# XiandaGuo/OpenStereo

Measured on NVIDIA H100. Metric: stereo_pairs_per_sec_gwcnet_256x512_d192, higher is better.
Workload: dtype f32

## Files before the change

include/openstereo_b200.h:

```cpp
#ifndef OPENSTEREO_B200_H_
#define OPENSTEREO_B200_H_

#include <stddef.h>
#include <stdint.h>

#ifdef __cplusplus
extern "C" {
#endif

#define OSB_OK 0
#define OSB_EINVAL 1
#define OSB_ECUDA 2
#define OSB_EUNSUPPORTED 3

#define OSB_ACT_NONE 0
#define OSB_ACT_RELU 1
#define OSB_ACT_LEAKY 2
#define OSB_ACT_RELU6 3

typedef void* osb_stream_t;

int osb_abi_version(void);
const char* osb_last_error(void);
uint64_t osb_launch_count(void);
int osb_tc_overflow_count(osb_stream_t stream, int reset, unsigned int* count);
int osb_tc_overflow_poll(osb_stream_t stream, unsigned int* host_pinned);
const unsigned int* osb_tc_overflow_flag(void);
float osb_set_rz_kappa(float kappa);
int osb_set_persistent_grid_cap(int cap);
const char* osb_tc_last_variant(void);
const char* osb_volume_last_variant(void);


int osb_gwc_volume_fwd(const float* ref, const float* tgt, float* out, int B, int C, int H, int W,
                       int D, int G, osb_stream_t stream);

int osb_concat_volume_fwd(const float* ref, const float* tgt, float* out, int B, int C, int H,
                          int W, int D, int mask_left, osb_stream_t stream);

int osb_gwc_concat_volume_fwd(const float* ref_gwc, const float* tgt_gwc, const float* ref_cat,
                              const float* tgt_cat, float* out, int B, int Cg, int Cc, int H, int W,
                              int D, int G, osb_stream_t stream);

int osb_corr_volume_fwd(const float* left, const float* right, float* out, int B, int C, int H,
                        int W, int D, osb_stream_t stream);


int osb_softargmin_fwd(const float* cost, float* out, int B, int D, int H, int W, float alpha,
                       float start, float step, int normalize, osb_stream_t stream);

int osb_upsample_softargmin_fwd(const float* cost, float* out, int B, int Dl, int Hl, int Wl, int D,
                                int H, int W, int align_corners, osb_stream_t stream);

int osb_upsample_softargmin_values_fwd(const float* cost, const float* values, float* out, int B, int Dl, int Hl, int Wl,
                                       int D, int H, int W, int align_corners, osb_stream_t stream);

int osb_epe_partial_fwd(const float* pred, const float* gt, float* out, int B, int HW, float maxdisp,
                        osb_stream_t stream);


int osb_conv3d_k3_bn_act_fwd(const float* x, const float* w_packed, const float* scale,
                             const float* shift, const float* residual, const float* gate, float* y,
                             int B, int Cin, int Cout, int D, int H, int W, int stride, int act,
                             osb_stream_t stream);

int osb_deconv3d_bn_act_fwd(const float* x, const float* w_packed, const float* scale,
                            const float* shift, const float* residual, float* y, int B, int Cin,
                            int Cout, int D, int H, int W, int kernel, int act, osb_stream_t stream);

int osb_conv3d_1x1_bn_act_fwd(const float* x0, const float* x1, int Cin0, const float* w_packed,
                              const float* scale, const float* shift, const float* residual,
                              const float* gate, float* y, int B, int Cin, int Cout, int D, int H,
                              int W, int act, int sigmoid_out, osb_stream_t stream);


int osb_conv3d_tc_supported(int Cin, int Cout, int W, int stride);
#define OSB_TC_MIN_WIDTH 24
int osb_tc_general_width(int W);
int osb_conv3d_tc_kc(int Cin, int Cout, int W, int stride);
int osb_conv3d_k3_tc_fwd(const float* x_ndhwc, const void* w_split, const float* scale, const float* shift,
                         const float* residual, float* y, int B, int Cin, int Cout, int D, int H, int W, int act,
                         int out_ndhwc, int res_ndhwc, osb_stream_t stream);
int osb_conv3d_k3_tc_gate_fwd(const float* x_ndhwc, const void* w_split, const float* scale, const float* shift,
                              const float* residual, const float* gate_nhwc, float* y, int B, int Cin, int Cout, int D, int H, int W,
                              int act, osb_stream_t stream);
int osb_conv3d_k3_tc_ncdhw_fwd(const float* x_ncdhw, const void* w_split, const float* scale, const float* shift,
                               const float* residual, float* y, int B, int Cin, int Cout, int D, int H, int W, int act,
                               int out_ndhwc, int res_ndhwc, osb_stream_t stream);
int osb_conv3d_s2_tc_supported(int Cin, int Cout, int D, int H, int W);
int osb_conv3d_k3_s2_tc_fwd(const float* x_ndhwc, const void* w_split, const float* scale, const float* shift,
                            const float* residual, float* y, int B, int Cin, int Cout, int D, int H, int W, int act,
                            int out_ndhwc, int res_ndhwc, osb_stream_t stream);
int osb_deconv3d_tc_supported(int Cin, int Cout, int W);
int osb_deconv3d_k3_tc_fwd(const float* x_ndhwc, const void* w_split, const float* scale, const float* shift,
                           const float* residual, float* y, int B, int Cin, int Cout, int D, int H, int W, int act,
                           int out_ndhwc, int res_ndhwc, osb_stream_t stream);
int osb_deconv3d_k4_tc_supported(int Cin, int Cout, int W);
int osb_deconv3d_k4_tc_fwd(const float* x_ndhwc, const void* w_split, const float* scale, const float* shift,
                           const float* residual, float* y, int B, int Cin, int Cout, int cout_real, int D, int H, int W, int act,
                           int out_ndhwc, int res_ndhwc, osb_stream_t stream);
int osb_conv3d_k3_tc_cs_fwd(const float* x_ndhwc, const void* w_split, const float* scale, const float* shift, const float* residual,
                            const float* gate_nhwc, float* y, int B, int Cin, int Cout, int D, int H, int W, int act, int ystride,
                            osb_stream_t stream);
int osb_conv3d_k3_s2_tc_cs_fwd(const float* x_ndhwc, const void* w_split, const float* scale, const float* shift, float* y, int B,
                               int Cin, int Cout, int D, int H, int W, int act, int ystride, osb_stream_t stream);
int osb_deconv3d_k4_tc_cs_fwd(const float* x_ndhwc, const void* w_split, const float* scale, const float* shift, float* y, int B,
                              int Cin, int Cout, int D, int H, int W, int act, int ystride, osb_stream_t stream);
int osb_conv1x1_ndhwc_cat_fwd(const float* x0, const float* x1, int C0, int C1, const float* w_packed, const float* scale,
                              const float* shift, float* y, long long voxels, int Cout, int act, osb_stream_t stream);
int osb_conv1x1_ndhwc_fwd(const float* x, const float* w_packed, const float* scale, const float* shift, float* y,
                          long long voxels, int Cin, int Cout, int act, osb_stream_t stream);
int osb_conv3d_k3_c1_ndhwc_fwd(const float* x_ndhwc, const float* w_taps, const float* scale, const float* shift, float* y, int B,
                               int Cin, int D, int H, int W, osb_stream_t stream);
int osb_conv2d_tc_kc(int Cin, int Cout, int W, int dilation);
int osb_conv2d_k3_tc_fwd(const float* x_nhwc, const void* w_split, const float* scale, const float* shift, const float* residual,
                         float* y, int B, int Cin, int Cout, int H, int W, int dilation, int act, int out_nhwc, int res_nhwc,
                         osb_stream_t stream);
int osb_gwc_volume_sum_fwd(const float* ref, const float* tgt, float* out, int B, int C, int H, int W, int D, int G,
                           osb_stream_t stream);
int osb_group_l2_normalize_fwd(const float* x, float* y, int B, int C, int H, int W, int G, float eps, osb_stream_t stream);
int osb_sub_volume_fwd(const float* left, const float* right, float* out, int B, int C, int H, int W, int D, osb_stream_t stream);
int osb_regression_values_fwd(const float* prob, const float* values, float* out, int B, int D, int H, int W, osb_stream_t stream);

int osb_warped_concat_volume_fwd(const float* x, const float* y, const float* disp, float* out, int B, int C, int D, int H, int W,
                                 int mask_left, osb_stream_t stream);
int osb_warped_gwc_concat_volume_fwd(const float* xg, const float* yg, const float* xc, const float* yc, const float* disp,
                                     float* out, int B, int Cg, int G, int Cc, int D, int H, int W, osb_stream_t stream);

int osb_coex_regression_fwd(const float* cost, const float* spx, float* out, int B, int D, int h, int w, int top_k, int spx_is_logits,
                            osb_stream_t stream);
int osb_nearest_resize3d_fwd(const float* x, float* y, int N, int Di, int Hi, int Wi, int Do, int Ho, int Wo, osb_stream_t stream);

int osb_mbv2_block3d_fwd(const float* x, const float* w_exp, const float* scale1, const float* shift1, const float* w_dw,
                         const float* scale2, const float* shift2, const float* w_proj, const float* scale3, const float* shift3,
                         const float* residual, float* y, int B, int Cin, int Chid, int Cout, int D, int H, int W, int stride,
                         int in_layout, int out_layout, osb_stream_t stream);

int osb_gwc_volume_bwd(const float* grad_vol, const float* ref, const float* tgt, float* grad_ref, float* grad_tgt, int B, int C,
                       int H, int W, int D, int G, int reduce_sum, osb_stream_t stream);
int osb_concat_volume_bwd(const float* grad_vol, float* grad_ref, float* grad_tgt, int B, int C, int H, int W, int D, int mask_left,
                          osb_stream_t stream);
int osb_softargmin_bwd(const float* cost, const float* grad_out, float* grad_cost, int B, int D, int H, int W, float alpha,
                       float start, float step, int normalize, osb_stream_t stream);

int osb_dwconv2d_fwd(const float* x, const float* w, const float* scale, const float* shift, const float* residual, float* y, int B,
                     int C, int H, int W, int KH, int KW, int stride, int act, osb_stream_t stream);
int osb_deconv2d_k3s2_fwd(const float* x, const float* w_packed, const float* scale, const float* shift, const float* residual,
                          float* y, int B, int Cin, int Cout, int H, int W, int act, osb_stream_t stream);

int osb_avgpool_pairs_fwd(const float* x, float* y, long long outer, int n, long long inner, osb_stream_t stream);
int osb_geo_lookup_fwd(const float* geo0, const float* geo1, const float* geo2, const float* geo3, const float* corr0,
                       const float* corr1, const float* corr2, const float* corr3, const float* disp, const float* coords,
                       float* out, int B, int C, int D, int H, int W, int W2, int num_levels, int radius, osb_stream_t stream);
int osb_context_upsample_fwd(const float* disp_low, const float* up_weights, float* out, int B, int h, int w, int scale,
                             osb_stream_t stream);
int osb_ncdhw_to_ndhwc(const float* x, float* y, int B, int C, int D, int H, int W, osb_stream_t stream);
int osb_ncdhw_to_ndhwc_pad(const float* x, float* y, int B, int C, int Cpad, int D, int H, int W, osb_stream_t stream);
int osb_feature_att_gate_fwd(const float* feat_nchw, const float* w1_packed, const float* scale1, const float* shift1,
                             const float* w2_packed, const float* scale2, const float* shift2, float* gate_nhwc, int B,
                             int Cf, int Ch, int Cv, int Cpad, int HW, int act1, osb_stream_t stream);

#ifdef __cplusplus
}
#endif
#endif
```

openstereo_b200/_lib.py:

```python
import ctypes
import os

_PKG = os.path.dirname(os.path.abspath(__file__))
LIB_PATH = os.path.join(_PKG, "lib", "libopenstereo_b200.so")

_f32p = ctypes.c_void_p
_i = ctypes.c_int
_f = ctypes.c_float
_s = ctypes.c_void_p

SIGNATURES = {
    "osb_gwc_volume_fwd": [_f32p, _f32p, _f32p, _i, _i, _i, _i, _i, _i, _s],
    "osb_concat_volume_fwd": [_f32p, _f32p, _f32p, _i, _i, _i, _i, _i, _i, _s],
    "osb_gwc_concat_volume_fwd": [_f32p, _f32p, _f32p, _f32p, _f32p, _i, _i, _i, _i, _i, _i, _i, _s],
    "osb_corr_volume_fwd": [_f32p, _f32p, _f32p, _i, _i, _i, _i, _i, _s],
    "osb_softargmin_fwd": [_f32p, _f32p, _i, _i, _i, _i, _f, _f, _f, _i, _s],
    "osb_upsample_softargmin_fwd": [_f32p, _f32p, _i, _i, _i, _i, _i, _i, _i, _i, _s],
    "osb_epe_partial_fwd": [_f32p, _f32p, _f32p, _i, _i, _f, _s],
    "osb_conv3d_k3_bn_act_fwd": [_f32p] * 7 + [_i] * 8 + [_s],
    "osb_deconv3d_bn_act_fwd": [_f32p] * 6 + [_i] * 8 + [_s],
    "osb_conv3d_1x1_bn_act_fwd": [_f32p, _f32p, _i] + [_f32p] * 6 + [_i] * 8 + [_s],
    "osb_conv3d_tc_supported": [_i, _i, _i, _i],
    "osb_conv3d_tc_kc": [_i, _i, _i, _i],
    "osb_tc_general_width": [_i],
    "osb_conv3d_s2_tc_supported": [_i, _i, _i, _i, _i],
    "osb_deconv3d_tc_supported": [_i, _i, _i],
    "osb_deconv3d_k3_tc_fwd": [_f32p] * 6 + [_i] * 9 + [_s],
    "osb_conv3d_k3_s2_tc_fwd": [_f32p] * 6 + [_i] * 9 + [_s],
    "osb_conv3d_k3_tc_fwd": [_f32p] * 6 + [_i] * 9 + [_s],
    "osb_conv3d_k3_tc_ncdhw_fwd": [_f32p] * 6 + [_i] * 9 + [_s],
    "osb_conv3d_k3_tc_gate_fwd": [_f32p] * 7 + [_i] * 7 + [_s],
    "osb_deconv3d_k4_tc_supported": [_i, _i, _i],
    "osb_conv3d_k3_tc_cs_fwd": [_f32p] * 7 + [_i] * 8 + [_s],
    "osb_conv3d_k3_s2_tc_cs_fwd": [_f32p] * 5 + [_i] * 8 + [_s],
    "osb_deconv3d_k4_tc_cs_fwd": [_f32p] * 5 + [_i] * 8 + [_s],
    "osb_deconv3d_k4_tc_fwd": [_f32p] * 6 + [_i] * 10 + [_s],
    "osb_conv1x1_ndhwc_cat_fwd": [_f32p, _f32p, _i, _i, _f32p, _f32p, _f32p, _f32p, ctypes.c_longlong, _i, _i, _s],
    "osb_feature_att_gate_fwd": [_f32p] * 8 + [_i] * 7 + [_s],
    "osb_ncdhw_to_ndhwc_pad": [_f32p, _f32p, _i, _i, _i, _i, _i, _i, _s],
    "osb_conv1x1_ndhwc_fwd": [_f32p] * 5 + [ctypes.c_longlong, _i, _i, _i, _s],
    "osb_conv3d_k3_c1_ndhwc_fwd": [_f32p] * 5 + [_i] * 5 + [_s],
    "osb_avgpool_pairs_fwd": [_f32p, _f32p, ctypes.c_longlong, _i, ctypes.c_longlong, _s],
    "osb_geo_lookup_fwd": [_f32p] * 11 + [_i] * 8 + [_s],
    "osb_context_upsample_fwd": [_f32p] * 3 + [_i] * 4 + [_s],
    "osb_conv2d_tc_kc": [_i] * 4,
    "osb_conv2d_k3_tc_fwd": [_f32p] * 6 + [_i] * 9 + [_s],
    "osb_ncdhw_to_ndhwc": [_f32p, _f32p, _i, _i, _i, _i, _i, _s],
    "osb_gwc_volume_sum_fwd": [_f32p, _f32p, _f32p, _i, _i, _i, _i, _i, _i, _s],
    "osb_group_l2_normalize_fwd": [_f32p, _f32p, _i, _i, _i, _i, _i, _f, _s],
    "osb_sub_volume_fwd": [_f32p, _f32p, _f32p, _i, _i, _i, _i, _i, _s],
    "osb_regression_values_fwd": [_f32p, _f32p, _f32p, _i, _i, _i, _i, _s],
    "osb_gwc_volume_bwd": [_f32p] * 5 + [_i] * 7 + [_s],
    "osb_concat_volume_bwd": [_f32p] * 3 + [_i] * 6 + [_s],
    "osb_softargmin_bwd": [_f32p] * 3 + [_i] * 4 + [_f, _f, _f, _i, _s],
    "osb_dwconv2d_fwd": [_f32p] * 6 + [_i] * 8 + [_s],
    "osb_deconv2d_k3s2_fwd": [_f32p] * 6 + [_i] * 6 + [_s],
    "osb_upsample_softargmin_values_fwd": [_f32p] * 3 + [_i] * 8 + [_s],
    "osb_warped_concat_volume_fwd": [_f32p] * 4 + [_i] * 6 + [_s],
    "osb_warped_gwc_concat_volume_fwd": [_f32p] * 6 + [_i] * 7 + [_s],
    "osb_coex_regression_fwd": [_f32p] * 3 + [_i] * 6 + [_s],
    "osb_nearest_resize3d_fwd": [_f32p] * 2 + [_i] * 7 + [_s],
    "osb_mbv2_block3d_fwd": [_f32p] * 12 + [_i] * 10 + [_s],
}


class NativeLibraryError(RuntimeError):
    pass


def _load():
    if not os.path.exists(LIB_PATH):
        raise NativeLibraryError(
            "%s not found: build it with `python -m openstereo_b200.build` (there is no CPU/PyTorch fallback)"
            % LIB_PATH)
    lib = ctypes.CDLL(LIB_PATH)
    lib.osb_abi_version.restype = ctypes.c_int
    lib.osb_last_error.restype = ctypes.c_char_p
    lib.osb_launch_count.restype = ctypes.c_uint64
    lib.osb_tc_overflow_count.argtypes = [ctypes.c_void_p, ctypes.c_int, ctypes.POINTER(ctypes.c_uint)]
    lib.osb_tc_overflow_count.restype = ctypes.c_int
    lib.osb_tc_overflow_poll.argtypes = [ctypes.c_void_p, ctypes.c_void_p]
    lib.osb_tc_overflow_poll.restype = ctypes.c_int
    lib.osb_tc_overflow_flag.argtypes = []
    lib.osb_tc_overflow_flag.restype = ctypes.c_void_p
    lib.osb_set_rz_kappa.argtypes = [ctypes.c_float]
    lib.osb_set_rz_kappa.restype = ctypes.c_float
    lib.osb_set_persistent_grid_cap.argtypes = [ctypes.c_int]
    lib.osb_set_persistent_grid_cap.restype = ctypes.c_int
    lib.osb_tc_last_variant.argtypes = []
    lib.osb_tc_last_variant.restype = ctypes.c_char_p
    lib.osb_volume_last_variant.argtypes = []
    lib.osb_volume_last_variant.restype = ctypes.c_char_p
    for name, argtypes in SIGNATURES.items():
        try:
            fn = getattr(lib, name)
        except AttributeError as exc:
            raise NativeLibraryError("%s does not export %s" % (LIB_PATH, name)) from exc
        fn.argtypes = argtypes
        fn.restype = ctypes.c_int
    return lib


lib = _load()

_ERRORS = {1: ValueError, 2: RuntimeError, 3: NotImplementedError}


def call(name, *args):
    if len(args) != len(SIGNATURES[name]):
        raise TypeError("%s takes %d arguments (%d given)" % (name, len(SIGNATURES[name]), len(args)))
    rc = getattr(lib, name)(*args)
    if rc != 0:
        msg = (lib.osb_last_error() or b"").decode("utf-8", "replace")
# ... 6 lines not shown
```

openstereo_b200/aggregation.py:

```python
import torch

from . import ops
from .ops import ACT_LEAKY, ACT_NONE, ACT_RELU, ACT_RELU6


class _Packed:
    __slots__ = ("w", "scale", "shift", "stride", "kernel", "transposed", "cin", "cout", "_w5", "_tc")

    def __init__(self, conv, bn=None):
        self._tc = {}
        self._w5 = conv.weight.detach() if conv.weight.dim() == 5 else None
        self.cin, self.cout = (conv.in_channels, conv.out_channels)
        self.transposed = isinstance(conv, (torch.nn.ConvTranspose3d, torch.nn.ConvTranspose2d))
        self.kernel = int(conv.kernel_size[0])
        self.stride = int(conv.stride[0])
        self._validate(conv)
        wt = conv.weight
        if wt.dim() == 4:
            wt = wt.unsqueeze(2)
        if self.transposed:
            self.w = ops.pack_deconv_weight(wt)
        else:
            self.w = ops.pack_conv_weight(wt)
        if self.kernel == 1:
            self.w = self.w.reshape(self.w.shape[0], self.w.shape[2]).contiguous()
        self.scale, self.shift = (None, None)
        if bn is not None:
            if bn.training:
                raise RuntimeError("BatchNorm folding is only valid in eval mode (call model.eval())")
            self.scale, self.shift = ops.fold_bn(bn)
        if getattr(conv, "bias", None) is not None:
            bias = conv.bias.detach().float()
            self.shift = bias.contiguous() if self.shift is None else (self.shift + bias * self.scale).contiguous()


def _packed_validate(self, conv):
    ks, st = tuple(conv.kernel_size), tuple(conv.stride)
    ok = len(set(ks)) == 1 and len(set(st)) == 1 and tuple(conv.dilation) == (1,) * len(ks) and conv.groups == 1
    if self.transposed:
        op = tuple(conv.output_padding)
        ok = ok and ((ks[0] == 3 and st[0] == 2 and tuple(conv.padding) == (1,) * len(ks) and op == (1,) * len(ks))
                     or (ks[0] == 4 and st[0] == 2 and tuple(conv.padding) == (1,) * len(ks) and op == (0,) * len(ks)))
    else:
        ok = ok and ks[0] in (1, 3) and st[0] in (1, 2) and tuple(conv.padding) == (ks[0] // 2,) * len(ks)
        ok = ok and getattr(conv, "padding_mode", "zeros") == "zeros"
    if not ok:
        raise NotImplementedError("openstereo_b200: no kernel for %r (supported: Conv k1/k3, stride 1/2, padding k//2, dilation 1, "
                                  "groups 1; ConvTranspose k3 s2 p1 op1 or k4 s2 p1)" % (conv,))


_Packed._validate = _packed_validate


def _conv(layer, x, act=ACT_NONE, residual=None, gate=None):
    if layer.kernel == 1:
        return ops.conv3d_1x1(x, layer.w, layer.scale, layer.shift, residual, gate, act)
    return ops.conv3d_k3(x, layer.w, layer.scale, layer.shift, residual, gate, layer.stride, act)


USE_TENSOR_CORES = True


def _tc_weight(layer, width):
    if not USE_TENSOR_CORES or layer.transposed or layer.kernel != 3 or layer.stride != 1 or layer._w5 is None:
        return None
    kc = ops.conv3d_tc_kc(layer.cin, layer.cout, width)
    if not kc:
        return None
    if kc not in layer._tc:
        layer._tc[kc] = ops.pack_tc_weight(layer._w5, kc, pad_cout_to=16 if layer.cout < 16 else None)
    return layer._tc[kc]


def _tc_ok(layer, width):
    return _tc_weight(layer, width) is not None


def _conv_tc(layer, x_ndhwc, act=ACT_NONE, residual=None, out_ndhwc=True, res_ndhwc=True, in_ncdhw=False):
    wt = _tc_weight(layer, x_ndhwc.shape[4] if in_ncdhw else x_ndhwc.shape[3])
    return ops.conv3d_k3_tc(x_ndhwc, wt, layer.scale, layer.shift, residual, act, out_ndhwc, res_ndhwc, in_ncdhw)


def _stem_in(layer, volume, act):
    if ops.conv3d_tc_kc(layer.cin, layer.cout, volume.shape[-1]) == 32:
        return _conv_tc(layer, volume, act, in_ncdhw=True)
    return _conv_tc(layer, ops.to_ndhwc(volume), act)


def _conv_auto(layer, x, act=ACT_NONE, residual=None):
    if layer.stride == 1 and _tc_ok(layer, x.shape[-1]):
        return _conv_tc(layer, ops.to_ndhwc(x), act, residual, out_ndhwc=False, res_ndhwc=False)
    if (USE_TENSOR_CORES and layer.stride == 2 and layer.kernel == 3 and not layer.transposed and layer._w5 is not None
            and ops.conv3d_s2_tc_supported(layer.cin, layer.cout, x.shape[2], x.shape[3], x.shape[4])):
        if "s2" not in layer._tc:
            layer._tc["s2"] = ops.pack_tc_weight(layer._w5, 16, kw_order=(1, 0, 2))
        return ops.conv3d_k3_s2_tc(ops.to_ndhwc(x), layer._tc["s2"], layer.scale, layer.shift, residual, act)
    return _conv(layer, x, act, residual)


def _deconv(layer, x, act=ACT_NONE, residual=None):
    if (USE_TENSOR_CORES and layer.transposed and layer.kernel == 3 and layer._w5 is not None
            and ops.deconv3d_tc_supported(layer.cin, layer.cout, x.shape[-1])):
        if "dc" not in layer._tc:
            layer._tc["dc"] = ops.pack_tc_deconv_weight(layer._w5)
        return ops.deconv3d_k3_tc(ops.to_ndhwc(x), layer._tc["dc"], layer.scale, layer.shift, residual, act)
    return ops.deconv3d(x, layer.w, layer.scale, layer.shift, residual, layer.kernel, act)


def _versions(module):
    return tuple(p._version for p in module.parameters()) + tuple(b._version for b in module.buffers())


class _Engine:

    def __init__(self, module):
        self.module = module
        self._stamp = None

    def _watch(self, device):
        if USE_TENSOR_CORES:
            mon = ops.TcOverflowMonitor.get(device)
            mon.check()
            return mon
        return None

    def _ensure(self, device):
        stamp = (str(device), _versions(self.module), tuple(p.data_ptr() for p in self.module.parameters()))
        if stamp != self._stamp:
            if self.module.training:
                raise RuntimeError("openstereo_b200 engines run inference only: call model.eval()")
            with torch.no_grad():
                self._pack()
            self._stamp = stamp

    @staticmethod
    def _check(x):
        if not x.is_cuda:
            raise RuntimeError("openstereo_b200: not implemented on the CPU (no fallback); move the model to CUDA")
        return x.detach().float().contiguous()


class _GwcHourglass:
    def __init__(self, m):
        self.conv1, self.conv2 = _Packed(m.conv1[0][0], m.conv1[0][1]), _Packed(m.conv2[0][0], m.conv2[0][1])
        self.conv3, self.conv4 = _Packed(m.conv3[0][0], m.conv3[0][1]), _Packed(m.conv4[0][0], m.conv4[0][1])
        self.conv5, self.conv6 = _Packed(m.conv5[0], m.conv5[1]), _Packed(m.conv6[0], m.conv6[1])
        self.redir1, self.redir2 = _Packed(m.redir1[0], m.redir1[1]), _Packed(m.redir2[0], m.redir2[1])

    def __call__(self, x):
        c1 = _conv_auto(self.conv1, x, ACT_RELU)
        c2 = _conv_auto(self.conv2, c1, ACT_RELU)
        c3 = _conv_auto(self.conv3, c2, ACT_RELU)
        c4 = _conv_auto(self.conv4, c3, ACT_RELU)
        c5 = _deconv(self.conv5, c4, ACT_RELU, residual=_conv(self.redir2, c2))
        return _deconv(self.conv6, c5, ACT_RELU, residual=_conv(self.redir1, x))


def _hg_channels_last_ok(hg, x_shape_ndhwc):
    if not USE_TENSOR_CORES:
        return False
    b, d, h, w, c = x_shape_ndhwc
    if d % 4 or h % 4 or w % 4:
        return False
    return (ops.conv3d_s2_tc_supported(hg.conv1.cin, hg.conv1.cout, d, h, w) and _tc_ok(hg.conv2, w // 2)
            and ops.conv3d_s2_tc_supported(hg.conv3.cin, hg.conv3.cout, d // 2, h // 2, w // 2) and _tc_ok(hg.conv4, w // 4)
            and ops.deconv3d_tc_supported(hg.conv5.cin, hg.conv5.cout, w // 4)
            and ops.deconv3d_tc_supported(hg.conv6.cin, hg.conv6.cout, w // 2)
            and (hg.redir1.cin, hg.redir1.cout) in ((32, 32), (64, 64)) and (hg.redir2.cin, hg.redir2.cout) in ((32, 32), (64, 64)))


def _s2_weight(layer):
    if "s2" not in layer._tc:
        layer._tc["s2"] = ops.pack_tc_weight(layer._w5, 16, kw_order=(1, 0, 2))
    return layer._tc["s2"]


def _dc_weight(layer):
    if "dc" not in layer._tc:
        layer._tc["dc"] = ops.pack_tc_deconv_weight(layer._w5)
    return layer._tc["dc"]


def _gwc_hourglass_channels_last(hg, x):
    c1 = ops.conv3d_k3_s2_tc(x, _s2_weight(hg.conv1), hg.conv1.scale, hg.conv1.shift, None, ACT_RELU, out_ndhwc=True)
    c2 = _conv_tc(hg.conv2, c1, ACT_RELU)
    c3 = ops.conv3d_k3_s2_tc(c2, _s2_weight(hg.conv3), hg.conv3.scale, hg.conv3.shift, None, ACT_RELU, out_ndhwc=True)
    c4 = _conv_tc(hg.conv4, c3, ACT_RELU)
    r2 = ops.conv1x1_ndhwc(c2, hg.redir2.w, hg.redir2.scale, hg.redir2.shift)
    c5 = ops.deconv3d_k3_tc(c4, _dc_weight(hg.conv5), hg.conv5.scale, hg.conv5.shift, r2, ACT_RELU, out_ndhwc=True, res_ndhwc=True)
    r1 = ops.conv1x1_ndhwc(x, hg.redir1.w, hg.redir1.scale, hg.redir1.shift)
    return ops.deconv3d_k3_tc(c5, _dc_weight(hg.conv6), hg.conv6.scale, hg.conv6.shift, r1, ACT_RELU, out_ndhwc=True, res_ndhwc=True)


def _classif3_channels_last(classif3, out):
    head0, cls = classif3
    width = out.shape[3]
    if _tc_ok(cls, width):
        return _conv_tc(cls, _conv_tc(head0, out, ACT_RELU), ACT_NONE, out_ndhwc=False, res_ndhwc=False)
    if cls.cin == 32 and cls.cout == 1 and cls._w5 is not None and cls.stride == 1:
        if "c1" not in cls._tc:
            cls._tc["c1"] = ops.pack_c1_weight(cls._w5)
        head = _conv_tc(head0, out, ACT_RELU)
        return ops.conv3d_k3_c1_ndhwc(head, cls._tc["c1"], cls.scale, cls.shift)
    head = _conv_tc(head0, out, ACT_RELU, out_ndhwc=False)
    return _conv(cls, head)


class GwcAggregation(_Engine):

    def _pack(self):
        m = self.module
        self.dres0 = [_Packed(m.dres0[0][0], m.dres0[0][1]), _Packed(m.dres0[2][0], m.dres0[2][1])]
        self.dres1 = [_Packed(m.dres1[0][0], m.dres1[0][1]), _Packed(m.dres1[2][0], m.dres1[2][1])]
        self.hg = [_GwcHourglass(m.dres2), _GwcHourglass(m.dres3), _GwcHourglass(m.dres4)]
        self.classif3 = [_Packed(m.classif3[0][0], m.classif3[0][1]), _Packed(m.classif3[2])]

    def logits(self, volume):
        volume = self._check(volume)
        self._ensure(volume.device)
        width = volume.shape[-1]
        stem_tc = all(_tc_ok(l, width) for l in (self.dres0[0], self.dres0[1], self.dres1[0], self.dres1[1]))
        b, _, dd, hh, ww = volume.shape
        if stem_tc and _tc_ok(self.classif3[0], width) and all(_hg_channels_last_ok(hg, (b, dd, hh, ww, 32)) for hg in self.hg):
            c = _conv_tc(self.dres0[1], _stem_in(self.dres0[0], volume, ACT_RELU), ACT_RELU)
            out = _conv_tc(self.dres1[1], _conv_tc(self.dres1[0], c, ACT_RELU), ACT_NONE, residual=c)
            for hg in self.hg:
                out = _gwc_hourglass_channels_last(hg, out)
            return _classif3_channels_last(self.classif3, out)
        if stem_tc:
            c = _conv_tc(self.dres0[1], _stem_in(self.dres0[0], volume, ACT_RELU), ACT_RELU)
            cost0 = _conv_tc(self.dres1[1], _conv_tc(self.dres1[0], c, ACT_RELU), ACT_NONE, residual=c, out_ndhwc=False)
        else:
            c = _conv(self.dres0[1], _conv(self.dres0[0], volume, ACT_RELU), ACT_RELU)
            cost0 = _conv(self.dres1[1], _conv(self.dres1[0], c, ACT_RELU), ACT_NONE, residual=c)
        out = cost0
        for hg in self.hg:
            out = hg(out)
        if _tc_ok(self.classif3[0], width):
            head = _conv_tc(self.classif3[0], ops.to_ndhwc(out), ACT_RELU, out_ndhwc=False)
        else:
            head = _conv(self.classif3[0], out, ACT_RELU)
        return _conv(self.classif3[1], head)

    def __call__(self, volume, h, w):
        mon = self._watch(volume.device)
        out = ops.upsample_softargmin(self.logits(volume), self.module.maxdisp, h, w, align_corners=False)
        if mon is not None:
            mon.poll()
        return out


class CascadeAggregation(GwcAggregation):

    def __call__(self, cost, fine_d, fine_h, fine_w, disp_range_samples):
        mon = self._watch(cost.device)
        assert tuple(disp_range_samples.shape[1:]) == (fine_d, fine_h, fine_w)
        out = ops.upsample_softargmin_values(self.logits(cost), disp_range_samples, align_corners=False)
        if mon is not None:
            mon.poll()
        return out


class _PSMHourglass:
    def __init__(self, m):
        self.conv1, self.conv2 = _Packed(m.conv1[0], m.conv1[1]), _Packed(m.conv2[0], m.conv2[1])
        self.conv3, self.conv4 = _Packed(m.conv3[0], m.conv3[1]), _Packed(m.conv4[0], m.conv4[1])
        self.conv5, self.conv6 = _Packed(m.conv5[0], m.conv5[1]), _Packed(m.conv6[0], m.conv6[1])

    def __call__(self, x, presqu, postsqu, skip):
        out = _conv_auto(self.conv1, x, ACT_RELU)
        pre = _conv_auto(self.conv2, out, ACT_RELU, residual=postsqu)
        out = _conv_auto(self.conv4, _conv_auto(self.conv3, pre, ACT_RELU), ACT_RELU)
        post = _deconv(self.conv5, out, ACT_RELU, residual=presqu if presqu is not None else pre)
        return _deconv(self.conv6, post, ACT_NONE, residual=skip), pre, post


def _psm_hg_channels_last_ok(hg, shape_ndhwc):
    if not USE_TENSOR_CORES:
        return False
    b, d, h, w, c = shape_ndhwc
    if d % 4 or h % 4 or w % 4 or any(l._w5 is None for l in (hg.conv1, hg.conv2, hg.conv3, hg.conv4, hg.conv5, hg.conv6)):
        return False
    return (ops.conv3d_s2_tc_supported(hg.conv1.cin, hg.conv1.cout, d, h, w) and _tc_ok(hg.conv2, w // 2)
            and ops.conv3d_s2_tc_supported(hg.conv3.cin, hg.conv3.cout, d // 2, h // 2, w // 2) and _tc_ok(hg.conv4, w // 4)
            and hg.conv5.kernel == 3 and hg.conv6.kernel == 3
            and ops.deconv3d_tc_supported(hg.conv5.cin, hg.conv5.cout, w // 4)
            and ops.deconv3d_tc_supported(hg.conv6.cin, hg.conv6.cout, w // 2))


def _psm_hourglass_channels_last(hg, x, presqu, postsqu, skip):
    out = ops.conv3d_k3_s2_tc(x, _s2_weight(hg.conv1), hg.conv1.scale, hg.conv1.shift, None, ACT_RELU, out_ndhwc=True)
    pre = _conv_tc(hg.conv2, out, ACT_RELU, residual=postsqu)
    out = ops.conv3d_k3_s2_tc(pre, _s2_weight(hg.conv3), hg.conv3.scale, hg.conv3.shift, None, ACT_RELU, out_ndhwc=True)
    out = _conv_tc(hg.conv4, out, ACT_RELU)
    post = ops.deconv3d_k3_tc(out, _dc_weight(hg.conv5), hg.conv5.scale, hg.conv5.shift, presqu if presqu is not None else pre, ACT_RELU,
                              out_ndhwc=True, res_ndhwc=True)
    out = ops.deconv3d_k3_tc(post, _dc_weight(hg.conv6), hg.conv6.scale, hg.conv6.shift, skip, ACT_NONE, out_ndhwc=True, res_ndhwc=True)
    return out, pre, post


class PSMAggregation(_Engine):

    def _pack(self):
        m = self.module
        self.dres0 = [_Packed(m.dres0[0][0], m.dres0[0][1]), _Packed(m.dres0[1][0], m.dres0[1][1])]
        self.dres1 = [_Packed(m.dres1[0][0], m.dres1[0][1]), _Packed(m.dres1[1][0], m.dres1[1][1])]
        self.hg = [_PSMHourglass(m.dres2), _PSMHourglass(m.dres3), _PSMHourglass(m.dres4)]
        self.heads = [[_Packed(c[0][0], c[0][1]), _Packed(c[1])] for c in (m.classif1, m.classif2, m.classif3)]
# ... 577 lines not shown
```

openstereo_b200/csrc/api.cu:

```cuda
#include <atomic>
#include <cstdarg>
#include <cstring>

#include "common.cuh"

namespace osb {

static thread_local char g_error[512] = "";
static std::atomic<uint64_t> g_launches{0};

void set_error(const char* fmt, ...) {
  va_list ap;
  va_start(ap, fmt);
  vsnprintf(g_error, sizeof(g_error), fmt, ap);
  va_end(ap);
}

static std::atomic<float> g_rz_kappa{1.57e-8f};
float rz_kappa() { return g_rz_kappa.load(std::memory_order_relaxed); }

static std::atomic<int> g_grid_cap{0};
long long cap_persistent_grid(long long grid) {
  const int cap = g_grid_cap.load(std::memory_order_relaxed);
  return (cap > 0 && grid > cap) ? cap : grid;
// ... 18 lines not shown
  unsigned int* fresh = nullptr;
  if (cudaMalloc(&fresh, sizeof(unsigned int)) != cudaSuccess || cudaMemset(fresh, 0, sizeof(unsigned int)) != cudaSuccess) {
    set_error("tc_overflow_flag: %s", cudaGetErrorString(cudaGetLastError()));
    return nullptr;
  }
  unsigned int* expected = nullptr;
  if (!g_overflow[dev].compare_exchange_strong(expected, fresh, std::memory_order_acq_rel)) {
    (void)cudaFree(fresh);
    return expected;
  }
  return fresh;
}

int device_index() {
  int dev = 0;
  if (cudaGetDevice(&dev) != cudaSuccess) {
    (void)cudaGetLastError();
    return 0;
  }
  return dev;
}

int sm_count() {
  static std::atomic<int> cache[64];
  const int dev = device_index();
  int n = cache[dev & 63].load(std::memory_order_relaxed);
  if (n > 0) return n;
  if (cudaDeviceGetAttribute(&n, cudaDevAttrMultiProcessorCount, dev) != cudaSuccess || n <= 0) {
    (void)cudaGetLastError();
    n = 132;
  }
  cache[dev & 63].store(n, std::memory_order_relaxed);
  return n;
}

void count_launch(int n) { g_launches.fetch_add((uint64_t)n, std::memory_order_relaxed); }

int check_launch(const char* what) {
  cudaError_t e = cudaGetLastError();
  if (e == cudaSuccess) return OSB_OK;
  set_error("%s: launch failed: %s", what, cudaGetErrorString(e));
  return OSB_ECUDA;
}

typedef CUresult (*EncodeTiledFn)(CUtensorMap*, CUtensorMapDataType, cuuint32_t, void*, const cuuint64_t*,
                                  const cuuint64_t*, const cuuint32_t*, const cuuint32_t*, CUtensorMapInterleave,
                                  CUtensorMapSwizzle, CUtensorMapL2promotion, CUtensorMapFloatOOBfill);

static EncodeTiledFn encode_fn() {
  static EncodeTiledFn fn = [] {
    void* p = nullptr;
    cudaDriverEntryPointQueryResult q;
    cudaError_t e = cudaGetDriverEntryPoint("cuTensorMapEncodeTiled", &p, cudaEnableDefault, &q);
    if (e != cudaSuccess || q != cudaDriverEntryPointSuccess) {
      (void)cudaGetLastError();
      return (EncodeTiledFn) nullptr;
    }
    return reinterpret_cast<EncodeTiledFn>(p);
  }();
  return fn;
}

bool make_tensor_map_3d(CUtensorMap* out, const void* base, uint64_t d0, uint64_t d1, uint64_t d2, uint64_t stride1_bytes,
                        uint64_t stride2_bytes, uint32_t box0, uint32_t box1, uint32_t box2) {
  EncodeTiledFn fn = encode_fn();
  if (!fn) {
    set_error("cuTensorMapEncodeTiled not available from the driver");
    return false;
  }
  const cuuint64_t dims[3] = {d0, d1, d2};
  const cuuint64_t strides[2] = {stride1_bytes, stride2_bytes};
  const cuuint32_t box[3] = {box0, box1, box2};
  const cuuint32_t elem[3] = {1, 1, 1};
  CUresult r = fn(out, CU_TENSOR_MAP_DATA_TYPE_FLOAT32, 3, const_cast<void*>(base), dims, strides, box, elem,
                  CU_TENSOR_MAP_INTERLEAVE_NONE, CU_TENSOR_MAP_SWIZZLE_NONE, CU_TENSOR_MAP_L2_PROMOTION_L2_128B,
                  CU_TENSOR_MAP_FLOAT_OOB_FILL_NONE);
  if (r != CUDA_SUCCESS) {
    set_error("cuTensorMapEncodeTiled failed with CUresult %d", (int)r);
    return false;
  }
  return true;
}

}

extern "C" {
int osb_abi_version(void) { return 1; }
const char* osb_last_error(void) { return osb::g_error; }
uint64_t osb_launch_count(void) { return osb::g_launches.load(std::memory_order_relaxed); }
float osb_set_rz_kappa(float kappa) {
  const float old = osb::g_rz_kappa.load(std::memory_order_relaxed);
  if (kappa >= 0.f && kappa < 1e-6f) osb::g_rz_kappa.store(kappa, std::memory_order_relaxed);
  return old;
}
int osb_set_persistent_grid_cap(int cap) { return osb::g_grid_cap.exchange(cap > 0 ? cap : 0, std::memory_order_relaxed); }
const char* osb_tc_last_variant(void) { return osb::g_tc_variant; }
int osb_tc_overflow_count(osb_stream_t stream, int reset, unsigned int* count) {
  using namespace osb;
  OSB_REQUIRE(count, "tc_overflow_count: null pointer");
  unsigned int* flag = tc_overflow_flag();
  if (!flag) return OSB_ECUDA;
  cudaStream_t st = (cudaStream_t)stream;
  cudaError_t e = cudaMemcpyAsync(count, flag, sizeof(unsigned int), cudaMemcpyDeviceToHost, st);
  if (e == cudaSuccess && reset) e = cudaMemsetAsync(flag, 0, sizeof(unsigned int), st);
  if (e == cudaSuccess) e = cudaStreamSynchronize(st);
  if (e != cudaSuccess) {
    set_error("tc_overflow_count: %s", cudaGetErrorString(e));
    return OSB_ECUDA;
  }
  return OSB_OK;
}
const unsigned int* osb_tc_overflow_flag(void) { return osb::tc_overflow_flag(); }
int osb_tc_overflow_poll(osb_stream_t stream, unsigned int* host_pinned) {
  using namespace osb;
  OSB_REQUIRE(host_pinned, "tc_overflow_poll: null pointer");
  unsigned int* flag = tc_overflow_flag();
  if (!flag) return OSB_ECUDA;
  cudaError_t e = cudaMemcpyAsync(host_pinned, flag, sizeof(unsigned int), cudaMemcpyDeviceToHost, (cudaStream_t)stream);
  if (e != cudaSuccess) {
    set_error("tc_overflow_poll: %s", cudaGetErrorString(e));
    return OSB_ECUDA;
  }
  return OSB_OK;
}
}
```

openstereo_b200/csrc/common.cuh:

```cuda
#pragma once
#include <cuda.h>
#include <cuda_runtime.h>
#include <stdint.h>
#include <stdio.h>

#include <string>

#include "../../include/openstereo_b200.h"

namespace osb {

void set_error(const char* fmt, ...);
void count_launch(int n = 1);
int check_launch(const char* what);
int device_index();
int sm_count();
long long cap_persistent_grid(long long grid);
std::string tc_variant_name(const char* fmt, ...);
void set_tc_variant(const char* name);
struct PerDeviceFlag {
  bool done[64] = {};
  bool& here() { return done[device_index() & 63]; }
};

#define OSB_REQUIRE(cond, ...)          \
  do {                                  \
    if (!(cond)) {                      \
      ::osb::set_error(__VA_ARGS__);    \
      return OSB_EINVAL;                \
    }                                   \
  } while (0)

__device__ __forceinline__ uint32_t smem_u32(const void* p) {
  return static_cast<uint32_t>(__cvta_generic_to_shared(p));
}

__device__ __forceinline__ void mbar_init(uint64_t* bar, uint32_t count) {
  asm volatile("mbarrier.init.shared::cta.b64 [%0], %1;" ::"r"(smem_u32(bar)), "r"(count));
}
__device__ __forceinline__ void fence_mbar_init() {
  asm volatile("fence.mbarrier_init.release.cluster;" ::: "memory");
}
__device__ __forceinline__ void fence_proxy_async() {
  asm volatile("fence.proxy.async.shared::cta;" ::: "memory");
}
__device__ __forceinline__ void mbar_arrive_expect_tx(uint64_t* bar, uint32_t bytes) {
  asm volatile("mbarrier.arrive.expect_tx.shared::cta.b64 _, [%0], %1;" ::"r"(smem_u32(bar)), "r"(bytes)
               : "memory");
}
__device__ __forceinline__ void mbar_wait(uint64_t* bar, uint32_t parity) {
  asm volatile(
      "{\n"
      ".reg .pred p;\n"
      "WAIT_LOOP:\n"
      "mbarrier.try_wait.parity.shared::cta.b64 p, [%0], %1;\n"
      "@p bra DONE;\n"
      "bra WAIT_LOOP;\n"
      "DONE:\n"
      "}\n" ::"r"(smem_u32(bar)),
      "r"(parity)
      : "memory");
}
__device__ __forceinline__ void tma_load_3d(void* smem_dst, const CUtensorMap* map, uint64_t* bar, int c0,
                                            int c1, int c2) {
  asm volatile(
      "cp.async.bulk.tensor.3d.shared::cluster.global.mbarrier::complete_tx::bytes [%0], [%1, {%3, %4, %5}], [%2];"
      ::"r"(smem_u32(smem_dst)),
      "l"(reinterpret_cast<uint64_t>(map)), "r"(smem_u32(bar)), "r"(c0), "r"(c1), "r"(c2)
      : "memory");
}
__device__ __forceinline__ void tma_prefetch_desc(const CUtensorMap* map) {
  asm volatile("prefetch.tensormap [%0];" ::"l"(reinterpret_cast<uint64_t>(map)) : "memory");
}

__device__ __forceinline__ void st_cs_f4(float* p, float4 v) { __stcs(reinterpret_cast<float4*>(p), v); }

bool make_tensor_map_3d(CUtensorMap* out, const void* base, uint64_t d0, uint64_t d1, uint64_t d2, uint64_t stride1_bytes,
                        uint64_t stride2_bytes, uint32_t box0, uint32_t box1, uint32_t box2);

}
```

openstereo_b200/csrc/conv3d_tc.cu:

```cuda
#include <type_traits>

#include "tc_common.cuh"

namespace osb {

constexpr int TC_W = 128;
constexpr int TC_KC = 32;
constexpr int TC_TILES = TC_WGS;
constexpr int TC_ROWS = TC_TILES + 2;
constexpr int TC_STAGES = 4;
constexpr int TC_RAW = 2;
constexpr int TC_ROW_BYTES = TC_W * TC_KC * 4;

struct TcParams {
  const float* x;
  const void* w;
  const float* scale;
  const float* shift;
  const float* residual;
  float* y;
  int B, D, H, Cin, Cout;
  int act;
  float kappa;
  unsigned int* overflow;
  int out_ndhwc, res_ndhwc;
  int bulk_rows;
  int in_ncdhw;
  int items, hblocks;
};

template <int COUT>
struct TcCfg {
  static constexpr int N3 = 3 * COUT;
  static constexpr int B_SLICE = N3 * TC_KC * 4;
  static constexpr int XCHG_FLOATS = 2 * frag_xchg_floats<COUT, 1>();
  static constexpr int A_OFF = 0;
  static constexpr int B_OFF = A_OFF + TC_STAGES * TC_ROW_BYTES;
  static constexpr int RAW_OFF = B_OFF + TC_BSLOTS * 3 * B_SLICE;
  static constexpr int BAR_OFF = RAW_OFF + TC_RAW * TC_ROW_BYTES;
  static constexpr size_t SMEM = 1024 + (size_t)BAR_OFF + 256 + TC_WGS * XCHG_FLOATS * 4 + 4 * TC_WGS * FRAG_TP_FLOATS * 4 + 2 * COUT * 4;
  static_assert(B_SLICE % 1024 == 0, "weight slices must stay 1024-byte aligned");
  static_assert(SMEM <= 232448, "shared memory budget of one CTA exceeded");
};

template <int COUT>
__global__ void __launch_bounds__(TC_WG_THREADS, 1) conv3d_tc_kernel(const TcParams p) {
  using C = TcCfg<COUT>;
  constexpr int N3 = C::N3;
  constexpr int B_SLICE = C::B_SLICE;
  extern __shared__ __align__(1024) uint8_t smem_raw[];
  uint8_t* smem = smem_raw + ((1024u - (smem_u32(smem_raw) & 1023u)) & 1023u);
  uint8_t* a_buf = smem + C::A_OFF;
  uint8_t* b_buf = smem + C::B_OFF;
  uint8_t* raw_buf = smem + C::RAW_OFF;
  uint64_t* bars = reinterpret_cast<uint64_t*>(smem + C::BAR_OFF);
  uint64_t* a_ready = bars;
  uint64_t* a_empty = a_ready + TC_STAGES;
  uint64_t* b_full = a_empty + TC_STAGES;
  uint64_t* b_empty = b_full + TC_BSLOTS * 3;
  uint64_t* raw_full = b_empty + TC_BSLOTS * 3;
  uint64_t* raw_empty = raw_full + TC_RAW;
  float* xchg = reinterpret_cast<float*>(smem + C::BAR_OFF + 256);
  float* tiles = xchg + TC_WGS * C::XCHG_FLOATS;
  float* s_scale = tiles + 4 * TC_WGS * FRAG_TP_FLOATS;
  float* s_shift = s_scale + COUT;

  const int warp = threadIdx.x >> 5, lane = threadIdx.x & 31;
  const int nchunk = p.Cin / TC_KC;

  if (threadIdx.x == 0) {
    for (int s = 0; s < TC_STAGES; ++s) {
      mbar_init(&a_ready[s], 128);
      mbar_init(&a_empty[s], 4 * TC_WGS);
    }
    for (int k = 0; k < TC_BSLOTS * 3; ++k) {
      mbar_init(&b_full[k], 1);
      mbar_init(&b_empty[k], 4 * TC_WGS);
    }
    for (int k = 0; k < TC_RAW; ++k) {
      mbar_init(&raw_full[k], 1);
      mbar_init(&raw_empty[k], 128);
    }
    fence_mbar_init();
  }
  for (int c = threadIdx.x; c < COUT; c += blockDim.x) {
    s_scale[c] = p.scale ? p.scale[c] : 1.f;
    s_shift[c] = p.shift ? p.shift[c] : 0.f;
  }
  __syncthreads();
  struct RowIter {
    int it, kd, ch, r;
  };
  auto advance = [&](RowIter& s) {
    for (;;) {
      if (s.it >= p.items) return false;
      if (++s.r < TC_ROWS) return true;
      s.r = -1;
      if (++s.ch < nchunk) continue;
      s.ch = 0;
      const int d = (s.it / p.hblocks) % p.D;
      for (++s.kd; s.kd < 3; ++s.kd) {
        const int din = d + s.kd - 1;
        if (din >= 0 && din < p.D) break;
      }
      if (s.kd < 3) continue;
      s.it += gridDim.x;
      if (s.it >= p.items) return false;
      const int d2 = (s.it / p.hblocks) % p.D;
      s.kd = (d2 == 0) ? 1 : 0;
    }
  };
  if (warp < 4 * TC_WGS) {
    setmaxnreg_inc<TC_CONSUMER_REGS>();
    const int wg = warp >> 2;
    xchg += wg * C::XCHG_FLOATS;
    const int bar_xchg = 1 + wg;
    constexpr uint32_t LO = TcK<TC_KC>::LO_OFF;
    constexpr uint32_t A_HALF = 64 * TC_KC * 4 / 16;
    const uint64_t dbase = desc_sw128_base();
    const uint32_t b16 = (smem_u32(b_buf) & 0x3FFFF) >> 4;
    const int q = warp & 3;
    uint32_t rowc = 0, phc = 0, exc = 0;
    for (int it = blockIdx.x; it < p.items; it += gridDim.x) {
      const int d = (it / p.hblocks) % p.D;
      const int b = it / (p.hblocks * p.D);
      const int h = (it % p.hblocks) * TC_TILES + wg;
      if (h < p.H && p.residual && p.res_ndhwc)
        asm volatile("prefetch.global.L2 [%0];" ::"l"(p.residual + ((((size_t)b * p.D + d) * p.H + h) * TC_W + q * 32 + lane) * COUT));
      float acc[2][N3 / 2];
      uint32_t accum = 0;
      for (int kd = 0; kd < 3; ++kd) {
        const int din = d + kd - 1;
        if (din < 0 || din >= p.D) continue;
        for (int ch = 0; ch < nchunk; ++ch, ++phc) {
          const uint32_t bslot = (phc & 1) * 3;
#pragma unroll
          for (int r = 0; r < TC_ROWS; ++r) {
            const uint32_t s = rowc % TC_STAGES, par = (rowc / TC_STAGES) & 1;
            mbar_wait(&a_ready[s], par);
            const int kh = r - wg;
            if (kh >= 0 && kh < 3) {
              mbar_wait(&b_full[bslot + kh], (phc >> 1) & 1);
              const uint64_t da0 = dbase | (uint64_t)((smem_u32(a_buf + s * TC_ROW_BYTES) & 0x3FFFF) >> 4);
              const uint64_t db0 = dbase | (uint64_t)(b16 + (bslot + kh) * (B_SLICE / 16));
              wg_fence();
#pragma unroll
              for (int ks = 0; ks < TcK<TC_KC>::KSTEPS; ++ks)
                wg_mma_split<N3>(acc, da0 + 2 * ks, A_HALF, db0 + 2 * ks, LO, ks > 0 ? 1u : accum);
              wg_commit();
              wg_wait_all();
              accum = 1;
              wg_release(&b_empty[bslot + kh], lane);
            }
            wg_release(&a_empty[s], lane);
            ++rowc;
          }
        }
      }
      if (h >= p.H) continue;
      const float corr = 1.f + p.kappa * (float)(((d > 0) + 1 + (d + 1 < p.D)) * nchunk * 3 * TcK<TC_KC>::KSTEPS * 3);
      frag_unshift<COUT, 1, TC_W>(acc, xchg + (exc & 1) * (C::XCHG_FLOATS / 2), q, lane, corr, bar_xchg);
      ++exc;
      const size_t row0 = (((size_t)b * p.D + d) * p.H + h) * TC_W;
      const size_t plane = (size_t)p.D * p.H * TC_W;
      const size_t ncdhw0 = (size_t)b * p.Cout * plane + ((size_t)d * p.H + h) * TC_W;
      auto rows = [&](int m, ptrdiff_t& yo, ptrdiff_t& ro, ptrdiff_t& go) {
        yo = p.out_ndhwc ? (ptrdiff_t)(row0 + m) * COUT : (ptrdiff_t)(ncdhw0 + m);
        ro = p.res_ndhwc ? (ptrdiff_t)(row0 + m) * COUT : (ptrdiff_t)(ncdhw0 + m);
        go = 0;
        return true;
      };
      frag_epilogue<COUT>(acc, lane, q, tiles + warp * FRAG_TP_FLOATS, s_scale, s_shift, p.act, p.y, p.out_ndhwc ? 1 : plane, p.residual, p.res_ndhwc ? 1 : plane,
                          nullptr, rows, COUT == 32 ? 32 : p.Cout);
    }
  }
  else if (warp < 4 * TC_WGS + 4) {
    setmaxnreg_dec<TC_LOADER_REGS>();
    const int lt = threadIdx.x - 4 * TC_WGS * 32;
    const int vsel = lt >> 3, c16 = lt & 7;
    const int vcol = ((vsel & 1) << 2) | ((vsel >> 1) & 3) | (vsel & 8);
    float amax = 0.f;
    auto run = [&](auto in_ncdhw) {
      constexpr bool NCDHW = decltype(in_ncdhw)::value;
      const size_t row_stride = (size_t)TC_W * p.Cin;
      auto load_row = [&](const RowIter& s, float4 (&v)[8]) {
        const int hb = s.it % p.hblocks;
        const int d = (s.it / p.hblocks) % p.D;
        const int b = s.it / (p.hblocks * p.D);
        const int hin = hb * TC_TILES - 1 + s.r, din = d + s.kd - 1;
        if (hin >= 0 && hin < p.H && NCDHW) {
          const size_t plane = (size_t)p.D * p.H * TC_W;
          const float* src = p.x + (((size_t)b * p.Cin + s.ch * TC_KC) * p.D + din) * p.H * TC_W + (size_t)hin * TC_W + lt;
#pragma unroll
          for (int j = 0; j < 8; ++j, src += 4 * plane)
            v[j] = make_float4(__ldg(src), __ldg(src + plane), __ldg(src + 2 * plane), __ldg(src + 3 * plane));
          const bool swap = (lt >> 3) & 1;
#pragma unroll
          for (int j = 0; j < 8; j += 2) {
            const float4 e = v[j], o = v[j + 1];
            v[j] = swap ? o : e;
            v[j + 1] = swap ? e : o;
          }
        } else if (hin >= 0 && hin < p.H) {
          const float* src = p.x + (((size_t)b * p.D + din) * p.H + hin) * row_stride + s.ch * TC_KC + c16 * 4 + vcol * p.Cin;
#pragma unroll
          for (int j = 0; j < 8; ++j) v[j] = __ldg(reinterpret_cast<const float4*>(src + 16 * j * p.Cin));
        } else {
#pragma unroll
          for (int j = 0; j < 8; ++j) v[j] = make_float4(0.f, 0.f, 0.f, 0.f);
        }
      };
      uint32_t rowc = 0;
      auto store_row = [&](const float4 (&v)[8]) {
        const uint32_t s = rowc % TC_STAGES, par = (rowc / TC_STAGES) & 1;
        mbar_wait_relaxed(&a_empty[s], par ^ 1);
        uint8_t* tile = a_buf + s * TC_ROW_BYTES;
        if (NCDHW) {
#pragma unroll
          for (int j = 0; j < 8; ++j) stage_f16_split<TC_KC>(tile, lt, j ^ ((lt >> 3) & 1), v[j], amax);
        } else {
#pragma unroll
          for (int j = 0; j < 8; ++j) stage_f16_split<TC_KC>(tile, vcol + 16 * j, c16, v[j], amax);
        }
        fence_proxy_async();
        mbar_arrive(&a_ready[s]);
        ++rowc;
      };
      RowIter ld{(int)blockIdx.x, 0, 0, -1};
      if (ld.it < p.items) ld.kd = (((ld.it / p.hblocks) % p.D) == 0) ? 1 : 0;
      if (p.bulk_rows) {
        uint32_t rawc = 0;
        while (advance(ld)) {
          const int hb = ld.it % p.hblocks;
          const int hin = hb * TC_TILES - 1 + ld.r;
          const uint32_t slot = rawc % TC_RAW, par = (rawc / TC_RAW) & 1;
          mbar_wait_relaxed(&raw_full[slot], par);
          float4 v[8];
          if (hin >= 0 && hin < p.H && NCDHW) {
            const float* src = reinterpret_cast<const float*>(raw_buf + slot * TC_ROW_BYTES) + lt;
#pragma unroll
            for (int j = 0; j < 8; ++j) {
              const float* q = src + 4 * (j ^ ((lt >> 3) & 1)) * TC_W;
              v[j] = make_float4(q[0], q[TC_W], q[2 * TC_W], q[3 * TC_W]);
            }
          } else if (hin >= 0 && hin < p.H) {
            const float* src = reinterpret_cast<const float*>(raw_buf + slot * TC_ROW_BYTES) + c16 * 4;
#pragma unroll
            for (int j = 0; j < 8; ++j) v[j] = *reinterpret_cast<const float4*>(src + (vcol + 16 * j) * TC_KC);
          } else {
#pragma unroll
            for (int j = 0; j < 8; ++j) v[j] = make_float4(0.f, 0.f, 0.f, 0.f);
          }
          store_row(v);
          mbar_arrive(&raw_empty[slot]);
          ++rawc;
        }
        tc_report_overflow(p.overflow, amax);
        amax = 0.f;
      }
      float4 va[8], vb[8];
      bool has_a = !p.bulk_rows && advance(ld);
      if (has_a) load_row(ld, va);
      bool has_b = has_a && advance(ld);
      if (has_b) load_row(ld, vb);
      while (has_a) {
        store_row(va);
        has_a = has_b && advance(ld);
        if (has_a) load_row(ld, va);
        if (!has_b) break;
        store_row(vb);
        has_b = has_a && advance(ld);
        if (has_b) load_row(ld, vb);
      }
      tc_report_overflow(p.overflow, amax);
    };
    if (p.in_ncdhw) run(std::true_type{});
    else run(std::false_type{});
  }
  else {
    setmaxnreg_dec<TC_PRODUCER_REGS>();
    if (warp == 4 * TC_WGS + 4 && elect_one()) {
      const uint8_t* wsrc = reinterpret_cast<const uint8_t*>(p.w);
      uint32_t phc = 0;
      for (int it = blockIdx.x; it < p.items; it += gridDim.x) {
        const int d = (it / p.hblocks) % p.D;
        for (int kd = 0; kd < 3; ++kd) {
          const int din = d + kd - 1;
          if (din < 0 || din >= p.D) continue;
          for (int ch = 0; ch < nchunk; ++ch, ++phc) {
            for (int kh = 0; kh < 3; ++kh) {
              const uint32_t slot = (phc & 1) * 3 + kh;
              const size_t slice = ((size_t)kd * nchunk + ch) * 3 + kh;
              mbar_wait_relaxed(&b_empty[slot], ((phc >> 1) & 1) ^ 1);
              mbar_arrive_expect_tx(&b_full[slot], B_SLICE);
              bulk_g2s(b_buf + slot * B_SLICE, wsrc + slice * B_SLICE, B_SLICE, &b_full[slot]);
            }
          }
        }
      }
    }
    else if (warp == 4 * TC_WGS + 5 && p.bulk_rows && elect_one()) {
      RowIter ld{(int)blockIdx.x, 0, 0, -1};
      if (ld.it < p.items) ld.kd = (((ld.it / p.hblocks) % p.D) == 0) ? 1 : 0;
      uint32_t rawc = 0;
      while (advance(ld)) {
        const int hb = ld.it % p.hblocks;
        const int d = (ld.it / p.hblocks) % p.D;
        const int b = ld.it / (p.hblocks * p.D);
        const int hin = hb * TC_TILES - 1 + ld.r, din = d + ld.kd - 1;
        const uint32_t slot = rawc % TC_RAW, par = (rawc / TC_RAW) & 1;
        mbar_wait_relaxed(&raw_empty[slot], par ^ 1);
        if (hin >= 0 && hin < p.H && p.in_ncdhw) {
          const size_t plane = (size_t)p.D * p.H * TC_W;
          const float* src = p.x + (((size_t)b * p.Cin + ld.ch * TC_KC) * p.D + din) * p.H * TC_W + (size_t)hin * TC_W;
          mbar_arrive_expect_tx(&raw_full[slot], TC_ROW_BYTES);
          for (int c = 0; c < TC_KC; ++c)
            bulk_g2s(raw_buf + slot * TC_ROW_BYTES + c * (TC_W * 4), src + c * plane, TC_W * 4, &raw_full[slot]);
        } else if (hin >= 0 && hin < p.H) {
          const float* src = p.x + (((size_t)b * p.D + din) * p.H + hin) * (size_t)(TC_W * TC_KC);
          mbar_arrive_expect_tx(&raw_full[slot], TC_ROW_BYTES);
          bulk_g2s(raw_buf + slot * TC_ROW_BYTES, src, TC_ROW_BYTES, &raw_full[slot]);
        } else {
          mbar_arrive(&raw_full[slot]);
        }
        ++rawc;
      }
    }
    __syncwarp();
  }
}

__global__ void __launch_bounds__(256) ncdhw_to_ndhwc_kernel(const float* __restrict__ x, float* __restrict__ y, int C, int Cp,
                                                             size_t vol) {
  __shared__ float tile[32][33];
  const int b = blockIdx.z;
  const size_t v0 = (size_t)blockIdx.x * 32;
  const int c0 = blockIdx.y * 32;
  const int tx = threadIdx.x & 31, ty = threadIdx.x >> 5;
  for (int i = ty; i < 32; i += 8) {
    const int c = c0 + i;
    const size_t v = v0 + tx;
    tile[i][tx] = (c < C && v < vol) ? __ldg(x + ((size_t)b * C + c) * vol + v) : 0.f;
  }
  __syncthreads();
  for (int i = ty; i < 32; i += 8) {
    const size_t v = v0 + i;
    const int c = c0 + tx;
    if (c < Cp && v < vol) y[((size_t)b * vol + v) * Cp + c] = tile[tx][i];
  }
}

template <int COUT>
int launch_tc(const TcArgs& a, cudaStream_t stream) {
  TcParams p{};
  p.Cout = a.Cout, p.in_ncdhw = a.in_ncdhw;
  p.bulk_rows = a.in_ncdhw || a.Cin == TC_KC;
  p.hblocks = (a.H + TC_TILES - 1) / TC_TILES;
  static const std::string variant = tc_variant_name("tc<%d>", COUT);
  return launch_persistent<conv3d_tc_kernel<COUT>>(a, p, (long long)a.B * a.D * p.hblocks, TcCfg<COUT>::SMEM, variant.c_str(), stream);
}
template int launch_tc<32>(const TcArgs&, cudaStream_t);
template int launch_tc<16>(const TcArgs&, cudaStream_t);

}

extern "C" {

int osb_tc_general_width(int W) { return W >= OSB_TC_MIN_WIDTH ? 1 : 0; }

int osb_conv3d_tc_kc(int Cin, int Cout, int W, int stride) {
  return stride == 1 ? osb::select_conv3d_tc(Cin, Cout, W, 1, false, false).kc : 0;
}

int osb_conv3d_tc_supported(int Cin, int Cout, int W, int stride) { return osb_conv3d_tc_kc(Cin, Cout, W, stride) != 0; }

int osb_ncdhw_to_ndhwc_pad(const float* x, float* y, int B, int C, int Cpad, int D, int H, int W, osb_stream_t stream) {
  using namespace osb;
  OSB_REQUIRE(x && y, "ncdhw_to_ndhwc: null pointer");
  OSB_REQUIRE(B > 0 && C > 0 && Cpad >= C && D > 0 && H > 0 && W > 0 && B <= 65535, "ncdhw_to_ndhwc: bad shape");
  const size_t vol = (size_t)D * H * W;
  dim3 grid((unsigned)((vol + 31) / 32), (Cpad + 31) / 32, B);
  ncdhw_to_ndhwc_kernel<<<grid, 256, 0, (cudaStream_t)stream>>>(x, y, C, Cpad, vol);
  count_launch();
  return check_launch("ncdhw_to_ndhwc_kernel");
}

int osb_ncdhw_to_ndhwc(const float* x, float* y, int B, int C, int D, int H, int W, osb_stream_t stream) {
  return osb_ncdhw_to_ndhwc_pad(x, y, B, C, C, D, H, W, stream);
}

static int conv3d_k3_tc_impl(osb::TcArgs a, int dilation, osb_stream_t stream) {
  using namespace osb;
  const int kc = select_conv3d_tc(a.Cin, a.Cout, a.W, dilation, false, false).kc;
  OSB_REQUIRE(kc, "conv3d_k3_tc: unsupported shape Cin=%d Cout=%d W=%d dilation=%d", a.Cin, a.Cout, a.W, dilation);
  OSB_REQUIRE(!a.in_ncdhw || kc == 32, "conv3d_k3_tc: NCDHW input is served by the W = 128 kernel only");
  OSB_REQUIRE((!a.ystride && !a.gate) || kc == 16, "conv3d_k3_tc: a channel slice or gate needs the 16-channel-chunk kernels");
  OSB_REQUIRE(a.Cout > 16 || (!a.out_ndhwc && (!a.residual || !a.res_ndhwc)), "conv3d_k3_tc: Cout <= 16 writes (and adds) NCDHW tensors only");
  const TcLaunch launch = select_conv3d_tc(a.Cin, a.Cout, a.W, dilation, a.gate != nullptr, a.slice()).launch;
  const int rc = check_tc_args("conv3d_k3_tc", a, launch);
  return rc != OSB_OK ? rc : launch(a, (cudaStream_t)stream);
}

int osb_conv3d_k3_tc_fwd(const float* x_ndhwc, const void* w_split, const float* scale, const float* shift,
                         const float* residual, float* y, int B, int Cin, int Cout, int D, int H, int W, int act,
                         int out_ndhwc, int res_ndhwc, osb_stream_t stream) {
  return conv3d_k3_tc_impl({x_ndhwc, w_split, scale, shift, residual, nullptr, y, B, Cin, Cout, D, H, W, act, out_ndhwc, res_ndhwc, 0, 0,
                            Cout}, 1, stream);
}

int osb_conv3d_k3_tc_gate_fwd(const float* x_ndhwc, const void* w_split, const float* scale, const float* shift,
                              const float* residual, const float* gate_nhwc, float* y, int B, int Cin, int Cout, int D, int H, int W,
                              int act, osb_stream_t stream) {
  OSB_REQUIRE(gate_nhwc, "conv3d_k3_tc_gate: null gate");
  return conv3d_k3_tc_impl({x_ndhwc, w_split, scale, shift, residual, gate_nhwc, y, B, Cin, Cout, D, H, W, act, 1, 1, 0, 0, Cout}, 1,
                           stream);
}

int osb_conv3d_k3_tc_cs_fwd(const float* x_ndhwc, const void* w_split, const float* scale, const float* shift, const float* residual,
                            const float* gate_nhwc, float* y, int B, int Cin, int Cout, int D, int H, int W, int act, int ystride,
                            osb_stream_t stream) {
  return conv3d_k3_tc_impl({x_ndhwc, w_split, scale, shift, residual, gate_nhwc, y, B, Cin, Cout, D, H, W, act, 1, 1, 0, ystride, Cout},
                           1, stream);
}

int osb_conv3d_k3_tc_ncdhw_fwd(const float* x_ncdhw, const void* w_split, const float* scale, const float* shift,
                               const float* residual, float* y, int B, int Cin, int Cout, int D, int H, int W, int act,
                               int out_ndhwc, int res_ndhwc, osb_stream_t stream) {
  return conv3d_k3_tc_impl({x_ncdhw, w_split, scale, shift, residual, nullptr, y, B, Cin, Cout, D, H, W, act, out_ndhwc, res_ndhwc, 1, 0,
                            Cout}, 1, stream);
}

int osb_conv2d_tc_kc(int Cin, int Cout, int W, int dilation) { return osb::select_conv3d_tc(Cin, Cout, W, dilation, false, false).kc; }

int osb_conv2d_k3_tc_fwd(const float* x_nhwc, const void* w_split, const float* scale, const float* shift, const float* residual,
                         float* y, int B, int Cin, int Cout, int H, int W, int dilation, int act, int out_nhwc, int res_nhwc,
                         osb_stream_t stream) {
  return conv3d_k3_tc_impl({x_nhwc, w_split, scale, shift, residual, nullptr, y, B, Cin, Cout, 1, H, W, act, out_nhwc, res_nhwc, 0, 0,
                            Cout}, dilation, stream);
}
}
```

openstereo_b200/csrc/conv3d_tcdc.cu:

```cuda
#include "tc_common.cuh"

namespace osb {

struct TcdcParams {
  const float* x;
  const void* w;
  const float* scale;
  const float* shift;
  const float* residual;
  float* y;
  int B, D, H, Cin;
  int act;
  float kappa;
  unsigned int* overflow;
  int out_ndhwc, res_ndhwc;
  int items, hblocks;
  int Wr, ctiles;
  int ystride;
  int cout_real;
};

template <int COUT, int KC, int W, int TILES, bool GW = false, int KS_ = 3>
struct TcdcCfg {
  static_assert(!GW || W == 128, "general-width tiles are 128-column segments of one input row");
  static_assert(KS_ == 3 || (KS_ == 4 && !GW), "kernel size 3 (any width) or 4 (whole-row tiles)");
  static constexpr int KS = KS_;
  static constexpr int HALO = GW ? 1 : 0;
  static constexpr int CSTEP = 128 - HALO;
  static constexpr int R = 128 / W;
  static constexpr int ROWB = KC * 4;
  static constexpr int UNIT_BYTES = 128 * ROWB;
  static constexpr int N3 = KS_ * COUT;
  static constexpr int G = 32;
  static constexpr int NG = COUT / G;
  static constexpr int NGK = KS_ * G;
  static constexpr int B_SLICE = N3 * ROWB;
  static constexpr int B_SUB = NGK * ROWB;
  static constexpr int SCOLS = KS_ == 3 ? NGK : 2 * G;
  static constexpr int LD = SCOLS + 4;
  static constexpr int NU = KS_ - 1;
  static constexpr int NLW = 4;
  static constexpr int XCHG_FLOATS = 2 * 4 * 2 * 32;
  static constexpr int FIXED_SMEM = 1024 + TC_BSLOTS * KS_ * B_SUB + TC_WGS * 128 * LD * 4 + 1024 + TC_WGS * XCHG_FLOATS * 4 + 3 * COUT * 4;
  static constexpr int STAGES = (232448 - FIXED_SMEM) / UNIT_BYTES < 10 ? (232448 - FIXED_SMEM) / UNIT_BYTES : 10;
  static_assert(STAGES >= NLW, "the ring must hold at least one unit per loader warp");
  static constexpr int HBLK = TILES * R;
  static constexpr int KSTEPS = KC / 16;
  static constexpr int LO = KC / 8;
  static constexpr int A_OFF = 0;
  static constexpr int B_OFF = A_OFF + STAGES * UNIT_BYTES;
  static constexpr int STAGE_OFF = B_OFF + TC_BSLOTS * KS_ * B_SUB;
  static constexpr int BAR_OFF = STAGE_OFF + TC_WGS * 128 * LD * 4;
  static constexpr int THREADS = TC_WG_THREADS;
  static constexpr size_t SMEM = 1024 + (size_t)BAR_OFF + 1024 + TC_WGS * XCHG_FLOATS * 4 + 3 * COUT * 4;
  static_assert(SMEM <= 232448, "shared memory budget of one CTA exceeded");
  static_assert(TILES == 1, "a consumer warpgroup holds one accumulator tile");
  static_assert(COUT % G == 0, "output channels come in groups of 32");
  static_assert(32 * LD >= TP_WARP_FLOATS, "store_ndhwc_chunk32 transposes through the warp's own rows of the staging tile");
  static_assert(B_SUB % 1024 == 0 && UNIT_BYTES % 1024 == 0, "operand tiles must stay 1024-byte aligned");
  static constexpr int kh_of(int u, int t) { return (t - 1 + 2 * u >= 0 && t - 1 + 2 * u < KS_) ? t - 1 + 2 * u : -1; }
};

struct ItemDc {
  int b, od, j0, ct, nkd;
};
__device__ __forceinline__ bool kd_valid(int od, int kd, int D) {
  const int num = od + 1 - kd;
  return !(num & 1) && num >= 0 && (num >> 1) < D;
}
__device__ __forceinline__ bool kh_valid(int ph, int kh) { return ((ph + 1 - kh) & 1) == 0; }
template <class C>
__device__ __forceinline__ ItemDc decode_dc(const TcdcParams& p, int it) {
  ItemDc w;
  w.ct = 0;
  if (C::HALO) {
    w.ct = it % p.ctiles;
    it /= p.ctiles;
  }
  const int Do = 2 * p.D;
  w.od = it % Do;
  it /= Do;
  w.j0 = (it % p.hblocks) * C::HBLK;
  w.b = it / p.hblocks;
  w.nkd = 0;
#pragma unroll
  for (int k = 0; k < C::KS; ++k) w.nkd += kd_valid(w.od, k, p.D) ? 1 : 0;
  return w;
}

template <int N, int GA, int GB, bool ADD>
__device__ __forceinline__ void dc_stage_pair(float* stage, int ld, const float (&acc)[2][N / 2], int wq, int lane) {
#pragma unroll
  for (int h = 0; h < 2; ++h) {
    float* r0 = stage + (64 * h + 16 * wq + (lane >> 2)) * ld + 2 * (lane & 3);
#pragma unroll
    for (int g = 0; g < 2; ++g)
#pragma unroll
      for (int jj = 0; jj < 4; ++jj) {
        const int j = (g ? GB : GA) * 4 + jj;
#pragma unroll
        for (int r = 0; r < 2; ++r) {
          float2* d = reinterpret_cast<float2*>(r0 + 8 * r * ld + 32 * g + 8 * jj);
          float2 v = make_float2(acc[h][4 * j + 2 * r], acc[h][4 * j + 2 * r + 1]);
          if (ADD) {
            const float2 s = *d;
            v = make_float2(s.x + v.x, s.y + v.y);
          }
          *d = v;
        }
      }
  }
}

template <int COUT, int KC, int W, int TILES, bool GW = false, int KS = 3>
__global__ void __launch_bounds__(TcdcCfg<COUT, KC, W, TILES, GW, KS>::THREADS, 1) conv3d_tcdc_kernel(const TcdcParams p) {
  using C = TcdcCfg<COUT, KC, W, TILES, GW, KS>;
  extern __shared__ __align__(1024) uint8_t smem_raw[];
  uint8_t* smem = smem_raw + ((1024u - (smem_u32(smem_raw) & 1023u)) & 1023u);
  uint8_t* a_buf = smem + C::A_OFF;
  uint8_t* b_buf = smem + C::B_OFF;
  float* stage = reinterpret_cast<float*>(smem + C::STAGE_OFF);
  uint64_t* bars = reinterpret_cast<uint64_t*>(smem + C::BAR_OFF);
  uint64_t* a_ready = bars;
  uint64_t* a_empty = a_ready + C::STAGES;
  uint64_t* b_full = a_empty + C::STAGES;
  uint64_t* b_empty = b_full + TC_BSLOTS * KS;
  float* xchg = reinterpret_cast<float*>(smem + C::BAR_OFF + 1024);
  float* s_scale = xchg + TC_WGS * C::XCHG_FLOATS;
  float* s_shift = s_scale + COUT;
  float* zeros = s_shift + COUT;

  const int warp = threadIdx.x >> 5, lane = threadIdx.x & 31;
  const int nchunk = p.Cin / KC;
  const int Wp = GW ? p.Wr : W;
  const int YS = (W < 32 && p.ystride) ? p.ystride : COUT;

  if (threadIdx.x == 0) {
    for (int s = 0; s < C::STAGES; ++s) {
      mbar_init(&a_ready[s], 32);
      mbar_init(&a_empty[s], 4 * TC_WGS);
    }
    for (int k = 0; k < TC_BSLOTS * KS; ++k) {
      mbar_init(&b_full[k], 1);
      mbar_init(&b_empty[k], 4 * TC_WGS);
    }
    fence_mbar_init();
  }
  for (int c = threadIdx.x; c < COUT; c += blockDim.x) {
    s_scale[c] = p.scale ? p.scale[c] : 1.f;
    s_shift[c] = p.shift ? p.shift[c] : 0.f;
    zeros[c] = 0.f;
  }
  __syncthreads();

  if (warp < 4 * TC_WGS) {
    setmaxnreg_inc<TC_CONSUMER_REGS>();
    const int wg = warp >> 2;
    stage += wg * 128 * C::LD;
    xchg += wg * C::XCHG_FLOATS;
    const int bar_stage = 1 + 2 * wg, bar_xchg = 2 + 2 * wg;
    const uint64_t dbase = (KC == 32) ? desc_sw128_base() : desc_sw64_base();
    constexpr uint32_t A_HALF = 64 * C::ROWB / 16;
    const uint32_t b16 = (smem_u32(b_buf) & 0x3FFFF) >> 4;
    const int q = warp & 3;
    const int m = q * 32 + lane;
    const int rr = m / W, wcol = m % W;
    const bool has_right_q = (((q + 1) * 32) % W) != 0;
    const bool has_left_q = ((q * 32) % W) != 0;
    const int Do = 2 * p.D, Ho = 2 * p.H;
    const int Wo = 2 * Wp;
    uint32_t unitc = 0, phc = 0, exc = 0;
    for (int it = blockIdx.x; it < p.items; it += gridDim.x) {
      const int cg = (it % C::NG) * C::G;
      const ItemDc w = decode_dc<C>(p, it / C::NG);
      float ev[32], od_[32];
      float acc[2][C::NGK / 2];
      uint32_t accum = 0;
      for (int kd = 0; kd < KS; ++kd) {
        if (!kd_valid(w.od, kd, p.D)) continue;
        for (int ch = 0; ch < nchunk; ++ch, ++phc) {
          const uint32_t bset = (phc & 1) * KS, bpar = (phc >> 1) & 1;
#pragma unroll
          for (int kh = 0; kh < KS; ++kh) {
            if (kh_valid(wg, kh)) continue;
            mbar_wait(&b_full[bset + kh], bpar);
            wg_release(&b_empty[bset + kh], lane);
          }
#pragma unroll
          for (int u = 0; u < C::NU; ++u) {
            const uint32_t slot = unitc % C::STAGES, par = (unitc / C::STAGES) & 1;
            mbar_wait(&a_ready[slot], par);
            const int kh = C::kh_of(u, wg);
            if (kh >= 0) {
              mbar_wait(&b_full[bset + kh], bpar);
              const uint64_t da0 = dbase | (uint64_t)((smem_u32(a_buf + slot * C::UNIT_BYTES) & 0x3FFFF) >> 4);
              const uint64_t db0 = dbase | (uint64_t)(b16 + ((bset + kh) * C::B_SUB) / 16);
              wg_fence();
#pragma unroll
              for (int ks = 0; ks < C::KSTEPS; ++ks)
                wg_mma_split<C::NGK>(acc, da0 + 2 * ks, A_HALF, db0 + 2 * ks, C::LO, ks > 0 ? 1u : accum);
              wg_commit();
              wg_wait_all();
              accum = 1;
              wg_release(&b_empty[bset + kh], lane);
            }
            wg_release(&a_empty[slot], lane);
            ++unitc;
          }
        }
      }
      const int j = w.j0 + rr;
      const bool live = j < p.H;
      const int oh = 2 * j + wg;
      const int col = GW ? w.ct * C::CSTEP + m : wcol;
      const bool cvalid = !GW || (m < C::CSTEP && col < Wp);
      const uint32_t vmask = GW ? __ballot_sync(0xffffffffu, cvalid) : 0xffffffffu;
      const size_t vox = (((size_t)w.b * Do + w.od) * Ho + oh) * Wo + 2 * col;
      if (live && cvalid && p.residual && p.res_ndhwc) {
        const float* rp = p.residual + vox * YS;
#pragma unroll
        for (int k = 0; k < 2 * COUT; k += 32) asm volatile("prefetch.global.L2 [%0];" ::"l"(rp + k));
      }
      const float corr = 1.f + p.kappa * (float)(w.nkd * (KS == 4 ? 2 : wg + 1) * nchunk * C::KSTEPS * 3);
      float* srow = stage + m * C::LD;
      float* xb = xchg + (exc & 1) * (4 * 2 * 32);
      ++exc;
      named_bar_sync(bar_stage, 128);
      if constexpr (KS == 3) {
        wg_stage<C::NGK>(stage, C::LD, acc, q, lane);
        named_bar_sync(bar_stage, 128);
        if (lane == 0) {
#pragma unroll
          for (int i = 0; i < 32; i += 4)
            *reinterpret_cast<float4*>(xb + (q * 2) * 32 + i) = *reinterpret_cast<const float4*>(srow + 2 * C::G + i);
        }
        named_bar_sync(bar_xchg, 128);
        const float* xr = has_right_q ? xb + ((q + 1) * 2) * 32 : zeros;
#pragma unroll
        for (int i0 = 0; i0 < 32; i0 += 4) {
          const float4 r4 = *reinterpret_cast<const float4*>(xr + i0);
          const float4 e4 = *reinterpret_cast<const float4*>(srow + i0);
          const float4 p24 = *reinterpret_cast<const float4*>(srow + C::G + i0);
          const float4 p04 = *reinterpret_cast<const float4*>(srow + 2 * C::G + i0);
          const float re[4] = {r4.x, r4.y, r4.z, r4.w};
          const float e[4] = {e4.x, e4.y, e4.z, e4.w}, p2[4] = {p24.x, p24.y, p24.z, p24.w}, p0[4] = {p04.x, p04.y, p04.z, p04.w};
#pragma unroll
          for (int k = 0; k < 4; ++k) {
            const int i = i0 + k;
            float right = __shfl_down_sync(0xffffffffu, p0[k], 1);
            right = (lane == 31) ? re[k] : right;
            if (W < 32) right = (wcol == W - 1) ? 0.f : right;
            ev[i] = e[k] * corr;
            od_[i] = (p2[k] + right) * corr;
          }
        }
      } else {
        dc_stage_pair<C::NGK, 1, 3, false>(stage, C::LD, acc, q, lane);
        named_bar_sync(bar_stage, 128);
        if (lane == 31) {
#pragma unroll
          for (int i = 0; i < 32; i += 4)
            *reinterpret_cast<float4*>(xb + (q * 2 + 1) * 32 + i) = *reinterpret_cast<const float4*>(srow + i);
        }
        if (lane == 0) {
#pragma unroll
          for (int i = 0; i < 32; i += 4)
            *reinterpret_cast<float4*>(xb + (q * 2) * 32 + i) = *reinterpret_cast<const float4*>(srow + C::G + i);
        }
        named_bar_sync(bar_xchg, 128);
        const float* xl = has_left_q ? xb + ((q - 1) * 2 + 1) * 32 : zeros;
        const float* xr = has_right_q ? xb + ((q + 1) * 2) * 32 : zeros;
#pragma unroll
        for (int i0 = 0; i0 < 32; i0 += 4) {
          const float4 l4 = *reinterpret_cast<const float4*>(xl + i0);
          const float4 r4 = *reinterpret_cast<const float4*>(xr + i0);
          const float4 p34 = *reinterpret_cast<const float4*>(srow + i0);
          const float4 p04 = *reinterpret_cast<const float4*>(srow + C::G + i0);
          const float le[4] = {l4.x, l4.y, l4.z, l4.w}, re[4] = {r4.x, r4.y, r4.z, r4.w};
          const float p3[4] = {p34.x, p34.y, p34.z, p34.w}, p0[4] = {p04.x, p04.y, p04.z, p04.w};
          float e[4], o[4];
#pragma unroll
          for (int k = 0; k < 4; ++k) {
            const float left = __shfl_up_sync(0xffffffffu, p3[k], 1);
// ... 231 lines not shown
```

openstereo_b200/csrc/conv3d_tcg.cu:

```cuda
#include "tc_common.cuh"

namespace osb {

struct TcgParams {
  const float* x;
  const void* w;
  const float* scale;
  const float* shift;
  const float* residual;
  const float* gate;
  float* y;
  int B, D, H, Cin;
  int act;
  float kappa;
  unsigned int* overflow;
  int out_ndhwc, res_ndhwc;
  int items, hblocks;
  int Wr, ctiles;
  int ystride;
};

template <int COUT, int KC, int W, int TILES, int DIL = 1, bool GW = false>
struct TcgCfg {
  static_assert(!GW || W == 128, "general-width tiles are 128-column segments of one image row");
  static constexpr int HALO = GW ? DIL : 0;
  static constexpr int CSTEP = 128 - 2 * HALO;
  static_assert(DIL == 1 || (W == 128 && DIL == 2 && COUT >= 64), "dilation 2 is instantiated for full-width rows only");
  static constexpr int R = 128 / W;
  static constexpr int ROWB = KC * 4;
  static constexpr int UNIT_BYTES = 128 * ROWB;
  static constexpr int N3 = 3 * COUT;
  static constexpr int G = 32;
  static constexpr int NG = COUT / G;
  static constexpr int NG3 = 3 * G;
  static constexpr int B_SLICE = N3 * ROWB;
  static constexpr int B_SUB = NG3 * ROWB;
  static constexpr int NT = TC_WGS * TILES;
  static constexpr int TS = R * DIL;
  static constexpr int HSPAN = NT * TS;
  __host__ __device__ static constexpr int row0(int hb) { return (hb / DIL) * HSPAN + (hb % DIL) * R; }
  __host__ static int hblocks(int H) { return DIL * ((H + HSPAN - 1) / HSPAN); }
  static constexpr int NLW = 4;
  static constexpr int XCHG_FLOATS = 2 * frag_xchg_floats<G, DIL>();
  static constexpr int FIXED_SMEM = 1024 + TC_BSLOTS * 3 * B_SUB + 1024 + TC_WGS * XCHG_FLOATS * 4 + 4 * TC_WGS * FRAG_TP_FLOATS * 4 +
                                    2 * COUT * 4;
  static constexpr int STAGES = (232448 - FIXED_SMEM) / UNIT_BYTES < 10 ? (232448 - FIXED_SMEM) / UNIT_BYTES : 10;
  static_assert(STAGES >= NLW, "the ring must hold at least one unit per loader warp");
  static constexpr int S_FIRST = -DIL;
  static constexpr int S_LAST = (NT - 1) * TS + DIL;
  static constexpr int KSTEPS = KC / 16;
  static constexpr int LO = KC / 8;
  static constexpr int A_OFF = 0;
  static constexpr int B_OFF = A_OFF + STAGES * UNIT_BYTES;
  static constexpr int BAR_OFF = B_OFF + TC_BSLOTS * 3 * B_SUB;
  static constexpr int THREADS = TC_WG_THREADS;
  static constexpr size_t SMEM = 1024 + (size_t)BAR_OFF + 1024 + TC_WGS * XCHG_FLOATS * 4 + 4 * TC_WGS * FRAG_TP_FLOATS * 4 + 2 * COUT * 4;
  static_assert(SMEM <= 232448, "shared memory budget of one CTA exceeded");
  static_assert(TILES == 1, "a consumer warpgroup holds one accumulator tile");
  static_assert(DIL == 1 || R == 1, "interleaved row blocks assume one image row per tile");
  static_assert(COUT % G == 0, "output channels come in groups of 32");
  static_assert(B_SUB % 1024 == 0 && UNIT_BYTES % 1024 == 0, "operand tiles must stay 1024-byte aligned");
  static constexpr int tile_of(int s, int kh) {
    const int num = s - (kh - 1) * DIL;
    return (num >= 0 && num % TS == 0 && num / TS < NT) ? num / TS : -1;
  }
  static constexpr bool used(int s) { return tile_of(s, 0) >= 0 || tile_of(s, 1) >= 0 || tile_of(s, 2) >= 0; }
  static constexpr int units_per_phase() {
    int n = 0;
    for (int s = S_FIRST; s <= S_LAST; ++s) n += used(s) ? 1 : 0;
    return n;
  }
  static constexpr int NU = units_per_phase();
  static constexpr int unit_s(int j) {
    int k = 0;
    for (int s = S_FIRST; s <= S_LAST; ++s)
      if (used(s)) {
        if (k == j) return s;
        ++k;
      }
    return S_LAST;
  }
};

template <int COUT, int KC, int W, int TILES, int DIL = 1, bool GW = false, bool GATE = false>
__global__ void __launch_bounds__(TcgCfg<COUT, KC, W, TILES, DIL, GW>::THREADS, 1) conv3d_tcg_kernel(const TcgParams p) {
  using C = TcgCfg<COUT, KC, W, TILES, DIL, GW>;
  extern __shared__ __align__(1024) uint8_t smem_raw[];
  uint8_t* smem = reinterpret_cast<uint8_t*>((reinterpret_cast<uintptr_t>(smem_raw) + 1023) & ~static_cast<uintptr_t>(1023));
  uint8_t* a_buf = smem + C::A_OFF;
  uint8_t* b_buf = smem + C::B_OFF;
  uint64_t* bars = reinterpret_cast<uint64_t*>(smem + C::BAR_OFF);
  uint64_t* a_ready = bars;
  uint64_t* a_empty = a_ready + C::STAGES;
  uint64_t* b_full = a_empty + C::STAGES;
  uint64_t* b_empty = b_full + TC_BSLOTS * 3;
  float* xchg = reinterpret_cast<float*>(smem + C::BAR_OFF + 1024);
  float* tiles = xchg + TC_WGS * C::XCHG_FLOATS;
  float* s_scale = tiles + 4 * TC_WGS * FRAG_TP_FLOATS;
  float* s_shift = s_scale + COUT;

  const int warp = threadIdx.x >> 5, lane = threadIdx.x & 31;
  const int nchunk = p.Cin / KC;
  const int Wp = GW ? p.Wr : W;
  const int YS = (W < 32 && p.ystride) ? p.ystride : COUT;
  const int ctiles = GW ? p.ctiles : 1;

  if (threadIdx.x == 0) {
    for (int s = 0; s < C::STAGES; ++s) {
      mbar_init(&a_ready[s], 32);
      mbar_init(&a_empty[s], 4 * TC_WGS);
    }
    for (int k = 0; k < TC_BSLOTS * 3; ++k) {
      mbar_init(&b_full[k], 1);
      mbar_init(&b_empty[k], 4 * TC_WGS);
    }
    fence_mbar_init();
  }
  for (int c = threadIdx.x; c < COUT; c += blockDim.x) {
    s_scale[c] = p.scale ? p.scale[c] : 1.f;
    s_shift[c] = p.shift ? p.shift[c] : 0.f;
  }
  __syncthreads();

  if (warp < 4 * TC_WGS) {
    setmaxnreg_inc<TC_CONSUMER_REGS>();
    const int wg = warp >> 2;
    xchg += wg * C::XCHG_FLOATS;
    const int bar_xchg = 1 + wg;
    const uint64_t dbase = (KC == 32) ? desc_sw128_base() : desc_sw64_base();
    constexpr uint32_t A_HALF = 64 * C::ROWB / 16;
    const uint32_t b16 = (smem_u32(b_buf) & 0x3FFFF) >> 4;
    const int q = warp & 3;
    uint32_t unitc = 0, phc = 0, exc = 0;
    for (int it = blockIdx.x; it < p.items; it += gridDim.x) {
      const int cg = (it % C::NG) * C::G;
      const int it0 = it / C::NG;
      const int ct = it0 % ctiles;
      const int hb = (it0 / ctiles) % p.hblocks;
      const int d = (it0 / (ctiles * p.hblocks)) % p.D;
      const int b = it0 / (ctiles * p.hblocks * p.D);
      auto tile_row = [&](int m, int& h, int& col) {
        h = C::row0(hb) + wg * C::TS + m / W;
        col = GW ? ct * C::CSTEP - C::HALO + m : m % W;
        return h < p.H && (!GW || (m >= C::HALO && m < 128 - C::HALO && col < Wp));
      };
      {
        int h, col;
        if (tile_row(q * 32 + lane, h, col)) {
          const ptrdiff_t vox = (((ptrdiff_t)b * p.D + d) * p.H + h) * Wp + col;
          if (p.residual && p.res_ndhwc) asm volatile("prefetch.global.L2 [%0];" ::"l"(p.residual + vox * YS + cg));
          if (GATE && p.gate) asm volatile("prefetch.global.L2 [%0];" ::"l"(p.gate + (((ptrdiff_t)b * p.H + h) * Wp + col) * YS + cg));
        }
      }
      float acc[2][C::NG3 / 2];
      uint32_t accum = 0;
      for (int kd = 0; kd < 3; ++kd) {
        const int din = d + kd - 1;
        if (din < 0 || din >= p.D) continue;
        for (int ch = 0; ch < nchunk; ++ch, ++phc) {
#pragma unroll
          for (int s = C::S_FIRST; s <= C::S_LAST; ++s) {
            if (!C::used(s)) continue;
            const uint32_t slot = unitc % C::STAGES, par = (unitc / C::STAGES) & 1;
            mbar_wait(&a_ready[slot], par);
            const uint64_t da0 = dbase | (uint64_t)((smem_u32(a_buf + slot * C::UNIT_BYTES) & 0x3FFFF) >> 4);
#pragma unroll
            for (int kh = 0; kh < 3; ++kh) {
              if (C::tile_of(s, kh) != wg) continue;
              const uint32_t bslot = (phc & 1) * 3 + kh;
              mbar_wait(&b_full[bslot], (phc >> 1) & 1);
              const uint64_t db0 = dbase | (uint64_t)(b16 + (bslot * C::B_SUB) / 16);
              wg_fence();
#pragma unroll
              for (int ks = 0; ks < C::KSTEPS; ++ks)
                wg_mma_split<C::NG3>(acc, da0 + 2 * ks, A_HALF, db0 + 2 * ks, C::LO, ks > 0 ? 1u : accum);
              wg_commit();
              wg_wait_all();
              accum = 1;
              wg_release(&b_empty[bslot], lane);
            }
            wg_release(&a_empty[slot], lane);
            ++unitc;
          }
        }
      }
      const float corr = 1.f + p.kappa * (float)(((d > 0) + 1 + (d + 1 < p.D)) * nchunk * 3 * C::KSTEPS * 3);
      frag_unshift<C::G, DIL, W>(acc, xchg + (exc & 1) * (C::XCHG_FLOATS / 2), q, lane, corr, bar_xchg);
      ++exc;
      const size_t plane = (size_t)p.D * p.H * Wp;
      auto rows = [&](int m, ptrdiff_t& yo, ptrdiff_t& ro, ptrdiff_t& go) {
        int h, col;
        const bool ok = tile_row(m, h, col);
        const ptrdiff_t vox = (((ptrdiff_t)b * p.D + d) * p.H + h) * Wp + col;
        const ptrdiff_t ncdhw = (ptrdiff_t)b * COUT * plane + ((ptrdiff_t)d * p.H + h) * Wp + col;
        yo = p.out_ndhwc ? vox * YS : ncdhw;
        ro = p.res_ndhwc ? vox * YS : ncdhw;
        go = (((ptrdiff_t)b * p.H + h) * Wp + col) * YS;
        return ok;
      };
      frag_epilogue<C::G>(acc, lane, q, tiles + warp * FRAG_TP_FLOATS, s_scale + cg, s_shift + cg, p.act, p.y + (p.out_ndhwc ? (size_t)cg : cg * plane),
                          p.out_ndhwc ? 1 : plane, p.residual ? p.residual + (p.res_ndhwc ? (size_t)cg : cg * plane) : nullptr,
                          p.res_ndhwc ? 1 : plane, (GATE && p.gate) ? p.gate + cg : nullptr, rows, C::G);
    }
  }
  else if (warp < 4 * TC_WGS + C::NLW) {
    setmaxnreg_dec<TC_LOADER_REGS>();
    const int lw = warp - 4 * TC_WGS;
    static_assert(KC == 16, "lane_voxel / unit-row mapping below is written for 64-byte operand rows");
    constexpr int CPR = KC / 4;
    constexpr int VPL = 32 / CPR;
    constexpr int NLD = 128 / VPL;
    static_assert(W % VPL == 0, "a load instruction must not straddle image rows");
    const int v0 = lane_voxel<KC>(lane), c = lane % CPR;
    float amax = 0.f;
    uint32_t ubase = 0;
    int first = lw;
    auto fill = [&](const float* base, size_t rstride, size_t cstride, int h_first, int h_step, uint32_t u, int col0) {
      float4 v[NLD];
#pragma unroll
      for (int j = 0; j < NLD; ++j) {
        const int hin = h_first + h_step * ((VPL * j) / W);
        const size_t off = (size_t)((VPL * j) / W) * rstride + (size_t)((VPL * j) % W) * cstride;
        bool ok = hin >= 0 && hin < p.H;
        if (GW) ok = ok && (unsigned)(col0 + VPL * j) < (unsigned)Wp;
        v[j] = ok ? __ldg(reinterpret_cast<const float4*>(base + (ptrdiff_t)off)) : make_float4(0.f, 0.f, 0.f, 0.f);
      }
      const uint32_t slot = u % C::STAGES, ph = (u / C::STAGES) & 1;
      mbar_wait_relaxed(&a_empty[slot], ph ^ 1);
      uint8_t* tile = a_buf + slot * C::UNIT_BYTES;
#pragma unroll
      for (int j = 0; j < NLD; ++j) stage_f16_split<KC>(tile, v0 + VPL * j, c, v[j], amax);
      fence_proxy_async();
      mbar_arrive(&a_ready[slot]);
    };
    for (int it = blockIdx.x; it < p.items; it += gridDim.x) {
      const int it0 = it / C::NG;
      const int ct = it0 % ctiles;
      const int hb = (it0 / ctiles) % p.hblocks;
      const int d = (it0 / (ctiles * p.hblocks)) % p.D;
      const int b = it0 / (ctiles * p.hblocks * p.D);
      const int h0 = C::row0(hb);
      const int col0 = ct * C::CSTEP - C::HALO + v0;
      for (int kd = 0; kd < 3; ++kd) {
        const int din = d + kd - 1;
        if (din < 0 || din >= p.D) continue;
        const float* plane = p.x + ((size_t)b * p.D + din) * p.H * (size_t)Wp * p.Cin;
        for (int ch = 0; ch < nchunk; ++ch) {
#pragma unroll 1
          for (int j = first; j < C::NU; j += C::NLW) {
            const int s = C::unit_s(j);
            const float* base = plane + ((ptrdiff_t)(h0 + s) * Wp + col0) * p.Cin + ch * KC + c * 4;
            fill(base, (size_t)Wp * p.Cin, (size_t)p.Cin, h0 + s, 1, ubase + j, col0);
          }
          ubase += C::NU;
          first = (first + C::NLW - C::NU % C::NLW) % C::NLW;
        }
      }
    }
// ... 80 lines not shown
```

openstereo_b200/csrc/conv3d_tcs2.cu:

```cuda
#include "tc_common.cuh"

namespace osb {

struct Tcs2Params {
  const float* x;
  const void* w;
  const float* scale;
  const float* shift;
  const float* residual;
  float* y;
  int B, D, H, Cin;
  int act;
  float kappa;
  unsigned int* overflow;
  int out_ndhwc, res_ndhwc;
  int items, hblocks;
  int Wr, ctiles;
  int ystride;
};

template <int COUT, int KC, int W, int TILES, bool GW = false>
struct Tcs2Cfg {
  static_assert(!GW || W == 128, "general-width tiles are 128-column segments of one output row");
  static constexpr int HALO = GW ? 1 : 0;
  static constexpr int CSTEP = 128 - HALO;
  static constexpr int R = 128 / W;
  static constexpr int ROWB = KC * 4;
  static constexpr int UNIT_BYTES = 128 * ROWB;
  static constexpr int N3 = 3 * COUT;
  static constexpr int G = 32;
  static constexpr int NG = COUT / G;
  static constexpr int NP = (NG + TC_WGS - 1) / TC_WGS;
  static constexpr int B_SLICE = N3 * ROWB;
  static constexpr int B_SUB = 3 * G * ROWB;
  static constexpr int B_SLOT = TC_WGS * B_SUB;
  static constexpr int PC = 16;
  static constexpr int NPASS = G / PC;
  static constexpr int LD = 3 * PC + 4;
  static constexpr int XCHG_FLOATS = 2 * 4 * PC;
  static constexpr int NLW = 4;
  static constexpr int FIXED_SMEM = 1024 + TC_BSLOTS * 3 * B_SLOT + TC_WGS * 128 * LD * 4 + 1024 + TC_WGS * XCHG_FLOATS * 4 + 3 * COUT * 4;
  static constexpr int STAGES = (232448 - FIXED_SMEM) / UNIT_BYTES < 10 ? (232448 - FIXED_SMEM) / UNIT_BYTES : 10;
  static_assert(STAGES >= NLW, "the ring must hold at least one unit per loader warp");
  static constexpr int NU = TILES * 3 * 2;
  static constexpr int HBLK = TILES * R;
  static constexpr int KSTEPS = KC / 16;
  static constexpr int LO = KC / 8;
  static constexpr int A_OFF = 0;
  static constexpr int B_OFF = A_OFF + STAGES * UNIT_BYTES;
  static constexpr int STAGE_OFF = B_OFF + TC_BSLOTS * 3 * B_SLOT;
  static constexpr int BAR_OFF = STAGE_OFF + TC_WGS * 128 * LD * 4;
  static constexpr int THREADS = TC_WG_THREADS;
  static constexpr size_t SMEM = 1024 + (size_t)BAR_OFF + 1024 + TC_WGS * XCHG_FLOATS * 4 + 3 * COUT * 4;
  static_assert(SMEM <= 232448, "shared memory budget of one CTA exceeded");
  static_assert(TILES == 1, "a consumer warpgroup holds one accumulator tile");
  static_assert(COUT % G == 0, "output channels come in groups of 32");
  static_assert(32 * LD >= TP_WARP_FLOATS, "store_ndhwc_chunk32 transposes through the warp's own rows of the staging tile");
  static_assert(B_SUB % 1024 == 0 && UNIT_BYTES % 1024 == 0, "operand tiles must stay 1024-byte aligned");
};

template <int N>
__device__ __forceinline__ void s2_stage16(float* stage, int ld, const float (&acc)[2][N / 2], int c0, int dst, int wq, int lane) {
#pragma unroll
  for (int h = 0; h < 2; ++h) {
    float* r0 = stage + (64 * h + 16 * wq + (lane >> 2)) * ld + 2 * (lane & 3) + dst;
#pragma unroll
    for (int jj = 0; jj < 2; ++jj) {
      const int j = c0 / 8 + jj;
      *reinterpret_cast<float2*>(r0 + 8 * jj) = make_float2(acc[h][4 * j], acc[h][4 * j + 1]);
      *reinterpret_cast<float2*>(r0 + 8 * ld + 8 * jj) = make_float2(acc[h][4 * j + 2], acc[h][4 * j + 3]);
    }
  }
}

template <int COUT, int KC, int W, int TILES, bool GW = false>
__global__ void __launch_bounds__(Tcs2Cfg<COUT, KC, W, TILES, GW>::THREADS, 1) conv3d_tcs2_kernel(const Tcs2Params p) {
  using C = Tcs2Cfg<COUT, KC, W, TILES, GW>;
  extern __shared__ __align__(1024) uint8_t smem_raw[];
  uint8_t* smem = smem_raw + ((1024u - (smem_u32(smem_raw) & 1023u)) & 1023u);
  uint8_t* a_buf = smem + C::A_OFF;
  uint8_t* b_buf = smem + C::B_OFF;
  float* stage = reinterpret_cast<float*>(smem + C::STAGE_OFF);
  uint64_t* bars = reinterpret_cast<uint64_t*>(smem + C::BAR_OFF);
  uint64_t* a_ready = bars;
  uint64_t* a_empty = a_ready + C::STAGES;
  uint64_t* b_full = a_empty + C::STAGES;
  uint64_t* b_empty = b_full + TC_BSLOTS * 3;
  float* xchg = reinterpret_cast<float*>(smem + C::BAR_OFF + 1024);
  float* s_scale = xchg + TC_WGS * C::XCHG_FLOATS;
  float* s_shift = s_scale + COUT;
  float* zeros = s_shift + COUT;

  const int warp = threadIdx.x >> 5, lane = threadIdx.x & 31;
  const int nchunk = p.Cin / KC;
  const int Wp = GW ? p.Wr : W;
  const int YS = (W < 32 && p.ystride) ? p.ystride : COUT;
  const int ctiles = GW ? p.ctiles : 1;

  if (threadIdx.x == 0) {
    for (int s = 0; s < C::STAGES; ++s) {
      mbar_init(&a_ready[s], 32);
      mbar_init(&a_empty[s], 4 * TC_WGS);
    }
    for (int k = 0; k < TC_BSLOTS * 3; ++k) {
      mbar_init(&b_full[k], 1);
      mbar_init(&b_empty[k], 4 * TC_WGS);
    }
    fence_mbar_init();
  }
  for (int c = threadIdx.x; c < COUT; c += blockDim.x) {
    s_scale[c] = p.scale ? p.scale[c] : 1.f;
    s_shift[c] = p.shift ? p.shift[c] : 0.f;
    zeros[c] = 0.f;
  }
  __syncthreads();

  if (warp < 4 * TC_WGS) {
    setmaxnreg_inc<TC_CONSUMER_REGS>();
    const int wg = warp >> 2;
    stage += wg * 128 * C::LD;
    xchg += wg * C::XCHG_FLOATS;
    const int bar_stage = 1 + 2 * wg, bar_xchg = 2 + 2 * wg;
    const uint64_t dbase = (KC == 32) ? desc_sw128_base() : desc_sw64_base();
    constexpr uint32_t A_HALF = 64 * C::ROWB / 16;
    const uint32_t b16 = (smem_u32(b_buf) & 0x3FFFF) >> 4;
    const int Do = p.D / 2, Ho = p.H / 2;
    const int q = warp & 3;
    const int m = q * 32 + lane;
    const int rr = m / W, wcol = m % W;
    const bool has_left_q = ((q * 32) % W) != 0;
    uint32_t unitc = 0, phc = 0, exc = 0;
    for (int it = blockIdx.x; it < p.items; it += gridDim.x) {
      const int g = (it % C::NP) * TC_WGS + wg;
      const bool has_group = g < C::NG;
      const int cg = g * C::G;
      const int it0 = it / C::NP;
      const int ct = it0 % ctiles;
      const int hb = (it0 / ctiles) % p.hblocks;
      const int d = (it0 / (ctiles * p.hblocks)) % Do;
      const int b = it0 / (ctiles * p.hblocks * Do);
      float acc_e[2][C::G / 2], acc_o[2][C::G];
      uint32_t accum_e = 0, accum_o = 0;
      for (int kd = 0; kd < 3; ++kd) {
        const int din = 2 * d + kd - 1;
        if (din < 0 || din >= p.D) continue;
        for (int ch = 0; ch < nchunk; ++ch, ++phc) {
#pragma unroll
          for (int kh = 0; kh < 3; ++kh) {
            const uint32_t bslot = (phc & 1) * 3 + kh;
#pragma unroll
            for (int par = 0; par < 2; ++par) {
              const uint32_t slot = unitc % C::STAGES, ph = (unitc / C::STAGES) & 1;
              mbar_wait(&a_ready[slot], ph);
              if (par == 0) mbar_wait(&b_full[bslot], (phc >> 1) & 1);
              if (has_group) {
                const uint64_t da0 = dbase | (uint64_t)((smem_u32(a_buf + slot * C::UNIT_BYTES) & 0x3FFFF) >> 4);
                const uint64_t db0 = dbase | (uint64_t)(b16 + (bslot * C::B_SLOT + wg * C::B_SUB + (par ? C::G * C::ROWB : 0)) / 16);
                wg_fence();
#pragma unroll
                for (int ks = 0; ks < C::KSTEPS; ++ks) {
                  if (par == 0) wg_mma_split<C::G>(acc_e, da0 + 2 * ks, A_HALF, db0 + 2 * ks, C::LO, ks > 0 ? 1u : accum_e);
                  else wg_mma_split<2 * C::G>(acc_o, da0 + 2 * ks, A_HALF, db0 + 2 * ks, C::LO, ks > 0 ? 1u : accum_o);
                }
                wg_commit();
                wg_wait_all();
                if (par == 0) accum_e = 1;
                else accum_o = 1;
              }
              wg_release(&a_empty[slot], lane);
              if (par == 1) wg_release(&b_empty[bslot], lane);
              ++unitc;
            }
          }
        }
      }
      if (!has_group) continue;
      const int h = hb * C::HBLK + rr;
      const bool live = h < Ho;
      const int col = GW ? ct * C::CSTEP - C::HALO + m : wcol;
      const bool cvalid = !GW || (m >= C::HALO && col < Wp);
      const uint32_t vmask = GW ? __ballot_sync(0xffffffffu, cvalid) : 0xffffffffu;
      const float corr = 1.f + p.kappa * (float)(((d > 0) + 1 + (2 * d + 1 < p.D)) * nchunk * 3 * C::KSTEPS * 3);
      const ptrdiff_t vox = (((ptrdiff_t)b * Do + d) * Ho + h) * Wp + col;
      const size_t plane = (size_t)Do * Ho * Wp;
      const ptrdiff_t ncdhw0 = (ptrdiff_t)b * COUT * plane + ((ptrdiff_t)d * Ho + h) * Wp + col;
      float out[32];
#pragma unroll
      for (int pass = 0; pass < C::NPASS; ++pass) {
        named_bar_sync(bar_stage, 128);
        s2_stage16<C::G>(stage, C::LD, acc_e, pass * C::PC, 0, q, lane);
        s2_stage16<2 * C::G>(stage, C::LD, acc_o, pass * C::PC, C::PC, q, lane);
        s2_stage16<2 * C::G>(stage, C::LD, acc_o, C::G + pass * C::PC, 2 * C::PC, q, lane);
        named_bar_sync(bar_stage, 128);
        const float* srow = stage + m * C::LD;
        float* xb = xchg + (exc & 1) * (4 * C::PC);
        ++exc;
        if (lane == 31) {
#pragma unroll
          for (int i = 0; i < C::PC; i += 4)
            *reinterpret_cast<float4*>(xb + q * C::PC + i) = *reinterpret_cast<const float4*>(srow + C::PC + i);
        }
        named_bar_sync(bar_xchg, 128);
        const float* xl = has_left_q ? xb + (q - 1) * C::PC : zeros;
#pragma unroll
        for (int i0 = 0; i0 < C::PC; i0 += 4) {
          const float4 l4 = *reinterpret_cast<const float4*>(xl + i0);
          const float4 p14 = *reinterpret_cast<const float4*>(srow + i0);
          const float4 p04 = *reinterpret_cast<const float4*>(srow + C::PC + i0);
          const float4 p24 = *reinterpret_cast<const float4*>(srow + 2 * C::PC + i0);
          const float le[4] = {l4.x, l4.y, l4.z, l4.w};
          const float p0[4] = {p04.x, p04.y, p04.z, p04.w}, p1[4] = {p14.x, p14.y, p14.z, p14.w}, p2[4] = {p24.x, p24.y, p24.z, p24.w};
#pragma unroll
          for (int k = 0; k < 4; ++k) {
            float left = __shfl_up_sync(0xffffffffu, p0[k], 1);
            left = (lane == 0) ? le[k] : left;
            if (W < 32) left = (wcol == 0) ? 0.f : left;
            out[pass * C::PC + i0 + k] = ((left + p1[k]) + p2[k]) * corr;
          }
        }
      }
      const uint32_t vm = (W < 32) ? __ballot_sync(0xffffffffu, live) : (live ? vmask : 0u);
      if (vm && p.out_ndhwc && (!p.residual || p.res_ndhwc)) {
        store_ndhwc_chunk32(stage + q * 32 * C::LD, lane, out, p.y + (vox - lane) * YS + cg,
                            p.residual ? p.residual + (vox - lane) * YS + cg : nullptr, YS, s_scale + cg, s_shift + cg, p.act, vm);
      } else if (live && cvalid) {
#pragma unroll
        for (int i = 0; i < 32; ++i) out[i] = fmaf(out[i], s_scale[cg + i], s_shift[cg + i]);
        if (p.residual) {
          if (p.res_ndhwc) {
            const float4* rp = reinterpret_cast<const float4*>(p.residual + vox * YS + cg);
#pragma unroll
            for (int i = 0; i < 8; ++i) {
              const float4 rv = __ldg(rp + i);
              out[4 * i] += rv.x, out[4 * i + 1] += rv.y, out[4 * i + 2] += rv.z, out[4 * i + 3] += rv.w;
            }
          } else {
#pragma unroll
            for (int i = 0; i < 32; ++i) out[i] += __ldg(p.residual + ncdhw0 + (size_t)(cg + i) * plane);
          }
        }
        if (p.act == OSB_ACT_RELU) {
#pragma unroll
          for (int i = 0; i < 32; ++i) out[i] = fmaxf(out[i], 0.f);
        } else if (p.act == OSB_ACT_LEAKY) {
#pragma unroll
// ... 162 lines not shown
```

openstereo_b200/csrc/tc_common.cuh:

```cuda
#pragma once
#include "common.cuh"

namespace osb {

__device__ __forceinline__ void mbar_wait_relaxed(uint64_t* bar, uint32_t parity) {
  uint32_t done;
  for (;;) {
    asm volatile(
        "{\n.reg .pred p;\nmbarrier.try_wait.parity.shared::cta.b64 p, [%1], %2;\nselp.u32 %0, 1, 0, p;\n}\n"
        : "=r"(done)
        : "r"(smem_u32(bar)), "r"(parity)
        : "memory");
    if (done) return;
    __nanosleep(64);
  }
}
__device__ __forceinline__ void mbar_arrive(uint64_t* bar) {
  asm volatile("mbarrier.arrive.shared::cta.b64 _, [%0];" ::"r"(smem_u32(bar)) : "memory");
}
__device__ __forceinline__ uint64_t desc_sw128_base() {
  uint64_t d = 0;
  d |= (uint64_t)1 << 16;
  d |= (uint64_t)(1024 >> 4) << 32;
  d |= (uint64_t)1 << 62;
  return d;
}
__device__ __forceinline__ uint64_t desc_sw64_base() {
  uint64_t d = 0;
  d |= (uint64_t)1 << 16;
  d |= (uint64_t)(512 >> 4) << 32;
  d |= (uint64_t)2 << 62;
  return d;
}

template <int N>
__device__ __forceinline__ void wgmma_f16(float (&d)[N / 2], uint64_t da, uint64_t db, uint32_t accumulate);
template <>
__device__ __forceinline__ void wgmma_f16<32>(float (&d)[16], uint64_t da, uint64_t db, uint32_t accumulate) {
  asm volatile(
      "{\n.reg .pred p;\nsetp.ne.b32 p, %18, 0;\n"
      "wgmma.mma_async.sync.aligned.m64n32k16.f32.f16.f16 {%0, %1, %2, %3, %4, %5, %6, %7, %8, %9, %10, %11, %12, %13, %14, %15}, %16, %17, p, 1, 1, 0, 0;\n}\n"
      : "+f"(d[0]), "+f"(d[1]), "+f"(d[2]), "+f"(d[3]), "+f"(d[4]), "+f"(d[5]), "+f"(d[6]), "+f"(d[7]), "+f"(d[8]), "+f"(d[9]), "+f"(d[10]), "+f"(d[11]), "+f"(d[12]), "+f"(d[13]), "+f"(d[14]), "+f"(d[15])
      : "l"(da), "l"(db), "r"(accumulate)
      : "memory");
}

template <>
__device__ __forceinline__ void wgmma_f16<48>(float (&d)[24], uint64_t da, uint64_t db, uint32_t accumulate) {
  asm volatile(
      "{\n.reg .pred p;\nsetp.ne.b32 p, %26, 0;\n"
      "wgmma.mma_async.sync.aligned.m64n48k16.f32.f16.f16 {%0, %1, %2, %3, %4, %5, %6, %7, %8, %9, %10, %11, %12, %13, %14, %15, %16, %17, %18, %19, %20, %21, %22, %23}, %24, %25, p, 1, 1, 0, 0;\n}\n"
      : "+f"(d[0]), "+f"(d[1]), "+f"(d[2]), "+f"(d[3]), "+f"(d[4]), "+f"(d[5]), "+f"(d[6]), "+f"(d[7]), "+f"(d[8]), "+f"(d[9]), "+f"(d[10]), "+f"(d[11]), "+f"(d[12]), "+f"(d[13]), "+f"(d[14]), "+f"(d[15]), "+f"(d[16]), "+f"(d[17]), "+f"(d[18]), "+f"(d[19]), "+f"(d[20]), "+f"(d[21]), "+f"(d[22]), "+f"(d[23])
      : "l"(da), "l"(db), "r"(accumulate)
      : "memory");
}

template <>
__device__ __forceinline__ void wgmma_f16<64>(float (&d)[32], uint64_t da, uint64_t db, uint32_t accumulate) {
  asm volatile(
      "{\n.reg .pred p;\nsetp.ne.b32 p, %34, 0;\n"
      "wgmma.mma_async.sync.aligned.m64n64k16.f32.f16.f16 {%0, %1, %2, %3, %4, %5, %6, %7, %8, %9, %10, %11, %12, %13, %14, %15, %16, %17, %18, %19, %20, %21, %22, %23, %24, %25, %26, %27, %28, %29, %30, %31}, %32, %33, p, 1, 1, 0, 0;\n}\n"
      : "+f"(d[0]), "+f"(d[1]), "+f"(d[2]), "+f"(d[3]), "+f"(d[4]), "+f"(d[5]), "+f"(d[6]), "+f"(d[7]), "+f"(d[8]), "+f"(d[9]), "+f"(d[10]), "+f"(d[11]), "+f"(d[12]), "+f"(d[13]), "+f"(d[14]), "+f"(d[15]), "+f"(d[16]), "+f"(d[17]), "+f"(d[18]), "+f"(d[19]), "+f"(d[20]), "+f"(d[21]), "+f"(d[22]), "+f"(d[23]), "+f"(d[24]), "+f"(d[25]), "+f"(d[26]), "+f"(d[27]), "+f"(d[28]), "+f"(d[29]), "+f"(d[30]), "+f"(d[31])
      : "l"(da), "l"(db), "r"(accumulate)
      : "memory");
}

template <>
__device__ __forceinline__ void wgmma_f16<96>(float (&d)[48], uint64_t da, uint64_t db, uint32_t accumulate) {
  asm volatile(
      "{\n.reg .pred p;\nsetp.ne.b32 p, %50, 0;\n"
      "wgmma.mma_async.sync.aligned.m64n96k16.f32.f16.f16 {%0, %1, %2, %3, %4, %5, %6, %7, %8, %9, %10, %11, %12, %13, %14, %15, %16, %17, %18, %19, %20, %21, %22, %23, %24, %25, %26, %27, %28, %29, %30, %31, %32, %33, %34, %35, %36, %37, %38, %39, %40, %41, %42, %43, %44, %45, %46, %47}, %48, %49, p, 1, 1, 0, 0;\n}\n"
      : "+f"(d[0]), "+f"(d[1]), "+f"(d[2]), "+f"(d[3]), "+f"(d[4]), "+f"(d[5]), "+f"(d[6]), "+f"(d[7]), "+f"(d[8]), "+f"(d[9]), "+f"(d[10]), "+f"(d[11]), "+f"(d[12]), "+f"(d[13]), "+f"(d[14]), "+f"(d[15]), "+f"(d[16]), "+f"(d[17]), "+f"(d[18]), "+f"(d[19]), "+f"(d[20]), "+f"(d[21]), "+f"(d[22]), "+f"(d[23]), "+f"(d[24]), "+f"(d[25]), "+f"(d[26]), "+f"(d[27]), "+f"(d[28]), "+f"(d[29]), "+f"(d[30]), "+f"(d[31]), "+f"(d[32]), "+f"(d[33]), "+f"(d[34]), "+f"(d[35]), "+f"(d[36]), "+f"(d[37]), "+f"(d[38]), "+f"(d[39]), "+f"(d[40]), "+f"(d[41]), "+f"(d[42]), "+f"(d[43]), "+f"(d[44]), "+f"(d[45]), "+f"(d[46]), "+f"(d[47])
      : "l"(da), "l"(db), "r"(accumulate)
      : "memory");
}

template <>
__device__ __forceinline__ void wgmma_f16<128>(float (&d)[64], uint64_t da, uint64_t db, uint32_t accumulate) {
  asm volatile(
      "{\n.reg .pred p;\nsetp.ne.b32 p, %66, 0;\n"
      "wgmma.mma_async.sync.aligned.m64n128k16.f32.f16.f16 {%0, %1, %2, %3, %4, %5, %6, %7, %8, %9, %10, %11, %12, %13, %14, %15, %16, %17, %18, %19, %20, %21, %22, %23, %24, %25, %26, %27, %28, %29, %30, %31, %32, %33, %34, %35, %36, %37, %38, %39, %40, %41, %42, %43, %44, %45, %46, %47, %48, %49, %50, %51, %52, %53, %54, %55, %56, %57, %58, %59, %60, %61, %62, %63}, %64, %65, p, 1, 1, 0, 0;\n}\n"
      : "+f"(d[0]), "+f"(d[1]), "+f"(d[2]), "+f"(d[3]), "+f"(d[4]), "+f"(d[5]), "+f"(d[6]), "+f"(d[7]), "+f"(d[8]), "+f"(d[9]), "+f"(d[10]), "+f"(d[11]), "+f"(d[12]), "+f"(d[13]), "+f"(d[14]), "+f"(d[15]), "+f"(d[16]), "+f"(d[17]), "+f"(d[18]), "+f"(d[19]), "+f"(d[20]), "+f"(d[21]), "+f"(d[22]), "+f"(d[23]), "+f"(d[24]), "+f"(d[25]), "+f"(d[26]), "+f"(d[27]), "+f"(d[28]), "+f"(d[29]), "+f"(d[30]), "+f"(d[31]), "+f"(d[32]), "+f"(d[33]), "+f"(d[34]), "+f"(d[35]), "+f"(d[36]), "+f"(d[37]), "+f"(d[38]), "+f"(d[39]), "+f"(d[40]), "+f"(d[41]), "+f"(d[42]), "+f"(d[43]), "+f"(d[44]), "+f"(d[45]), "+f"(d[46]), "+f"(d[47]), "+f"(d[48]), "+f"(d[49]), "+f"(d[50]), "+f"(d[51]), "+f"(d[52]), "+f"(d[53]), "+f"(d[54]), "+f"(d[55]), "+f"(d[56]), "+f"(d[57]), "+f"(d[58]), "+f"(d[59]), "+f"(d[60]), "+f"(d[61]), "+f"(d[62]), "+f"(d[63])
      : "l"(da), "l"(db), "r"(accumulate)
      : "memory");
}

__device__ __forceinline__ void wg_fence() { asm volatile("wgmma.fence.sync.aligned;" ::: "memory"); }
__device__ __forceinline__ void wg_commit() { asm volatile("wgmma.commit_group.sync.aligned;" ::: "memory"); }
__device__ __forceinline__ void wg_wait_all() { asm volatile("wgmma.wait_group.sync.aligned 0;" ::: "memory"); }

template <int N>
__device__ __forceinline__ void wg_mma_split(float (&acc)[2][N / 2], uint64_t da, uint32_t a_half, uint64_t db, uint32_t lo,
                                             uint32_t accumulate) {
#pragma unroll
  for (int h = 0; h < 2; ++h) {
    wgmma_f16<N>(acc[h], da + h * a_half + lo, db, accumulate);
    wgmma_f16<N>(acc[h], da + h * a_half, db + lo, 1);
    wgmma_f16<N>(acc[h], da + h * a_half, db, 1);
  }
}
__device__ __forceinline__ void wg_release(uint64_t* bar, int lane) {
  if (lane == 0) mbar_arrive(bar);
}
template <int N>
__device__ __forceinline__ void wg_stage(float* stage, int ld, const float (&acc)[2][N / 2], int wq, int lane) {
#pragma unroll
  for (int h = 0; h < 2; ++h) {
    float* r0 = stage + (64 * h + 16 * wq + (lane >> 2)) * ld + 2 * (lane & 3);
#pragma unroll
    for (int j = 0; j < N / 8; ++j) {
      *reinterpret_cast<float2*>(r0 + 8 * j) = make_float2(acc[h][4 * j], acc[h][4 * j + 1]);
      *reinterpret_cast<float2*>(r0 + 8 * ld + 8 * j) = make_float2(acc[h][4 * j + 2], acc[h][4 * j + 3]);
    }
  }
}
__device__ __forceinline__ void stage_ld16(const float* row, uint32_t* r) {
#pragma unroll
  for (int i = 0; i < 4; ++i) {
    const float4 v = reinterpret_cast<const float4*>(row)[i];
    r[4 * i] = __float_as_uint(v.x), r[4 * i + 1] = __float_as_uint(v.y), r[4 * i + 2] = __float_as_uint(v.z), r[4 * i + 3] = __float_as_uint(v.w);
  }
}

__device__ __forceinline__ void bulk_g2s(void* smem_dst, const void* gsrc, uint32_t bytes, uint64_t* bar) {
  asm volatile("cp.async.bulk.shared::cluster.global.mbarrier::complete_tx::bytes [%0], [%1], %2, [%3];" ::"r"(smem_u32(smem_dst)),
               "l"(gsrc), "r"(bytes), "r"(smem_u32(bar))
               : "memory");
}
__device__ __forceinline__ void cp_async16(void* smem_dst, const void* gsrc, bool valid) {
  const uint32_t n = valid ? 16u : 0u;
  asm volatile("cp.async.ca.shared.global [%0], [%1], 16, %2;" ::"r"(smem_u32(smem_dst)), "l"(gsrc), "r"(n) : "memory");
}
__device__ __forceinline__ void cp_async_commit() { asm volatile("cp.async.commit_group;" ::: "memory"); }
template <int N>
__device__ __forceinline__ void cp_async_wait() {
  asm volatile("cp.async.wait_group %0;" ::"n"(N) : "memory");
}
constexpr int TC_BSLOTS = 2;
__device__ __forceinline__ void named_bar_sync(int id, int threads) {
  asm volatile("bar.sync %0, %1;" ::"r"(id), "r"(threads) : "memory");
}
__device__ __forceinline__ void named_bar_arrive(int id, int threads) {
  asm volatile("bar.arrive %0, %1;" ::"r"(id), "r"(threads) : "memory");
}
constexpr int TC_WGS = 2;
constexpr int TC_CONSUMER_REGS = 184;
constexpr int TC_LOADER_REGS = 112;
constexpr int TC_PRODUCER_REGS = 32;
constexpr int TC_WG_THREADS = 512;
template <int N>
__device__ __forceinline__ void setmaxnreg_inc() {
  asm volatile("setmaxnreg.inc.sync.aligned.u32 %0;" ::"n"(N));
}
template <int N>
__device__ __forceinline__ void setmaxnreg_dec() {
  asm volatile("setmaxnreg.dec.sync.aligned.u32 %0;" ::"n"(N));
}
__device__ __forceinline__ bool elect_one() {
  uint32_t pred;
  asm volatile("{\n.reg .pred p;\nelect.sync _|p, 0xffffffff;\nselp.u32 %0, 1, 0, p;\n}\n" : "=r"(pred));
  return pred != 0;
}
constexpr float TC_ACT_SCALE = 16.f;
constexpr float TC_F16_MAX = 65504.f;
__device__ __forceinline__ uint32_t cvt_f16x2_sat(float a, float b) {
  uint32_t r;
  asm("cvt.rn.satfinite.f16x2.f32 %0, %1, %2;" : "=r"(r) : "f"(b), "f"(a));
  return r;
}
__device__ __forceinline__ float2 f16x2_to_float2(uint32_t h) {
  float2 f;
  asm("{\n.reg .b16 l, u;\nmov.b32 {l, u}, %2;\ncvt.f32.f16 %0, l;\ncvt.f32.f16 %1, u;\n}\n" : "=f"(f.x), "=f"(f.y) : "r"(h));
  return f;
}
__device__ __forceinline__ void f16_split4(const float4 v, uint2& hi, uint2& lo, float& amax) {
  const float x0 = v.x * TC_ACT_SCALE, x1 = v.y * TC_ACT_SCALE, x2 = v.z * TC_ACT_SCALE, x3 = v.w * TC_ACT_SCALE;
  amax = fmaxf(amax, fmaxf(fmaxf(fabsf(x0), fabsf(x1)), fmaxf(fabsf(x2), fabsf(x3))));
  hi.x = cvt_f16x2_sat(x0, x1);
  hi.y = cvt_f16x2_sat(x2, x3);
  const float2 h01 = f16x2_to_float2(hi.x), h23 = f16x2_to_float2(hi.y);
  lo.x = cvt_f16x2_sat(x0 - h01.x, x1 - h01.y);
  lo.y = cvt_f16x2_sat(x2 - h23.x, x3 - h23.y);
}
unsigned int* tc_overflow_flag();
__device__ __forceinline__ void tc_report_overflow(unsigned int* flag, float amax) {
  if (amax > TC_F16_MAX) atomicAdd(flag, 1u);
}

float rz_kappa();


template <int KC>
__device__ __forceinline__ int swz_offset(int row, int c) {
  if constexpr (KC == 32) return row * 128 + ((c ^ (row & 7)) << 4);
  else return row * 64 + ((c ^ ((row >> 1) & 3)) << 4);
}


template <int KC>
__device__ __forceinline__ void stage_f16_split(uint8_t* tile, int row, int q, const float4 v, float& amax) {
  uint2 hi, lo;
  f16_split4(v, hi, lo, amax);
  const int sub = (q & 1) << 3;
  *reinterpret_cast<uint2*>(tile + swz_offset<KC>(row, q >> 1) + sub) = hi;
  *reinterpret_cast<uint2*>(tile + swz_offset<KC>(row, KC / 8 + (q >> 1)) + sub) = lo;
}
template <int KC>
__device__ __forceinline__ int lane_voxel(int lane) {
  if constexpr (KC == 32) return (((lane >> 3) & 1) << 2) | (lane >> 4);
  else return ((lane >> 2) & 1) | (((lane >> 3) & 1) << 2) | ((lane >> 4) << 1);
}
template <int KC>
struct TcK {
  static constexpr int KSTEPS = KC / 16;
  static constexpr int LO_OFF = KC / 8;
};

template <int G, int DIL>
constexpr int frag_xchg_floats() { return 8 * 2 * DIL * G; }
template <int G, int DIL, int W>
__device__ __forceinline__ void frag_unshift(float (&acc)[2][3 * G / 2], float* xb, int wq, int lane, float corr, int bar) {
  constexpr int SIDE = DIL * G;
  const int l4 = lane >> 2, c0 = 2 * (lane & 3);
#pragma unroll
  for (int h = 0; h < 2; ++h) {
    float* grp = xb + (4 * h + wq) * 2 * SIDE;
    if (l4 >= 8 - DIL) {
#pragma unroll
      for (int j = 0; j < G / 8; ++j)
        *reinterpret_cast<float2*>(grp + (l4 - 8 + DIL) * G + 8 * j + c0) = make_float2(acc[h][4 * j + 2], acc[h][4 * j + 3]);
    }
    if (l4 < DIL) {
#pragma unroll
      for (int j = 0; j < G / 8; ++j)
        *reinterpret_cast<float2*>(grp + SIDE + l4 * G + 8 * j + c0) =
            make_float2(acc[h][4 * (j + G / 4)], acc[h][4 * (j + G / 4) + 1]);
    }
  }
  named_bar_sync(bar, 128);
  const int src_l = (lane - 4 * DIL) & 31, src_r = (lane + 4 * DIL) & 31;
  const bool wrap_l = l4 >= 8 - DIL, wrap_r = l4 < DIL;
#pragma unroll
  for (int h = 0; h < 2; ++h) {
    const int g = 4 * h + wq;
    const float* xl = xb + (g > 0 ? g - 1 : 0) * 2 * SIDE + (l4 < DIL ? l4 : 0) * G + c0;
    const float* xr = xb + (g < 7 ? g + 1 : 7) * 2 * SIDE + SIDE + (l4 >= 8 - DIL ? l4 - 8 + DIL : 0) * G + c0;
    const int mlo = (64 * h + 16 * wq + l4) % W, mhi = (64 * h + 16 * wq + 8 + l4) % W;
#pragma unroll
    for (int j = 0; j < G / 8; ++j) {
      const float2 sl = *reinterpret_cast<const float2*>(xl + 8 * j);
      const float2 sr = *reinterpret_cast<const float2*>(xr + 8 * j);
#pragma unroll
      for (int c2 = 0; c2 < 2; ++c2) {
        const float p0lo = acc[h][4 * j + c2], p0hi = acc[h][4 * j + 2 + c2];
        const float p2lo = acc[h][4 * (j + G / 4) + c2], p2hi = acc[h][4 * (j + G / 4) + 2 + c2];
        float llo = __shfl_sync(0xffffffffu, p0lo, src_l);
        float lhi = __shfl_sync(0xffffffffu, wrap_l ? p0lo : p0hi, src_l);
        float rlo = __shfl_sync(0xffffffffu, wrap_r ? p2hi : p2lo, src_r);
        float rhi = __shfl_sync(0xffffffffu, p2hi, src_r);
        llo = (l4 < DIL) ? (c2 ? sl.y : sl.x) : llo;
        rhi = (l4 >= 8 - DIL) ? (c2 ? sr.y : sr.x) : rhi;
        llo = (mlo < DIL) ? 0.f : llo;
        lhi = (mhi < DIL) ? 0.f : lhi;
        rlo = (mlo >= W - DIL) ? 0.f : rlo;
        rhi = (mhi >= W - DIL) ? 0.f : rhi;
        float& olo = acc[h][4 * (j + G / 8) + c2];
        float& ohi = acc[h][4 * (j + G / 8) + 2 + c2];
        olo = ((llo + olo) + rlo) * corr;
        ohi = ((lhi + ohi) + rhi) * corr;
      }
    }
  }
}
constexpr int FRAG_TP_STRIDE = 40;
constexpr int FRAG_TP_FLOATS = 16 * FRAG_TP_STRIDE;
template <int G, class Rows>
__device__ __forceinline__ void frag_epilogue(const float (&acc)[2][3 * G / 2], int lane, int wq, float* tbuf, const float* sc,
                                              const float* sh, int act, float* y, size_t ycs, const float* res, size_t rcs,
                                              const float* gate, Rows rows, int nch) {
  const int c0 = 2 * (lane & 3), l4 = lane >> 2;
  if constexpr (G == 32) {
    if (ycs == 1 && (!res || rcs == 1)) {
      const int c4 = 4 * (lane & 7), sub = lane >> 3;
      const float4 a = *reinterpret_cast<const float4*>(sc + c4);
      const float4 b = *reinterpret_cast<const float4*>(sh + c4);
#pragma unroll
      for (int h = 0; h < 2; ++h) {
        __syncwarp();
#pragma unroll
        for (int j = 0; j < 4; ++j)
#pragma unroll
          for (int rh = 0; rh < 2; ++rh)
            *reinterpret_cast<float2*>(tbuf + (8 * rh + l4) * FRAG_TP_STRIDE + 8 * j + c0) =
                make_float2(acc[h][4 * (j + 4) + 2 * rh], acc[h][4 * (j + 4) + 2 * rh + 1]);
        __syncwarp();
        float4 o[4];
        ptrdiff_t yo[4], ro[4], go[4];
        bool ok[4];
#pragma unroll
        for (int i = 0; i < 4; ++i) {
          ok[i] = rows(64 * h + 16 * wq + 4 * i + sub, yo[i], ro[i], go[i]);
          o[i] = *reinterpret_cast<const float4*>(tbuf + (4 * i + sub) * FRAG_TP_STRIDE + c4);
          o[i].x = fmaf(o[i].x, a.x, b.x), o[i].y = fmaf(o[i].y, a.y, b.y), o[i].z = fmaf(o[i].z, a.z, b.z), o[i].w = fmaf(o[i].w, a.w, b.w);
        }
        if (res) {
          float4 r[4];
#pragma unroll
          for (int i = 0; i < 4; ++i) r[i] = ok[i] ? __ldg(reinterpret_cast<const float4*>(res + ro[i] + c4)) : make_float4(0.f, 0.f, 0.f, 0.f);
#pragma unroll
          for (int i = 0; i < 4; ++i) o[i].x += r[i].x, o[i].y += r[i].y, o[i].z += r[i].z, o[i].w += r[i].w;
        }
        if (act == OSB_ACT_RELU) {
#pragma unroll
          for (int i = 0; i < 4; ++i) o[i].x = fmaxf(o[i].x, 0.f), o[i].y = fmaxf(o[i].y, 0.f), o[i].z = fmaxf(o[i].z, 0.f), o[i].w = fmaxf(o[i].w, 0.f);
        } else if (act == OSB_ACT_LEAKY) {
#pragma unroll
          for (int i = 0; i < 4; ++i) {
            o[i].x = o[i].x > 0.f ? o[i].x : 0.01f * o[i].x, o[i].y = o[i].y > 0.f ? o[i].y : 0.01f * o[i].y;
            o[i].z = o[i].z > 0.f ? o[i].z : 0.01f * o[i].z, o[i].w = o[i].w > 0.f ? o[i].w : 0.01f * o[i].w;
          }
        }
        if (gate) {
          float4 g[4];
#pragma unroll
          for (int i = 0; i < 4; ++i) g[i] = ok[i] ? __ldg(reinterpret_cast<const float4*>(gate + go[i] + c4)) : make_float4(1.f, 1.f, 1.f, 1.f);
#pragma unroll
          for (int i = 0; i < 4; ++i) o[i].x *= g[i].x, o[i].y *= g[i].y, o[i].z *= g[i].z, o[i].w *= g[i].w;
        }
#pragma unroll
        for (int i = 0; i < 4; ++i)
          if (ok[i]) *reinterpret_cast<float4*>(y + yo[i] + c4) = o[i];
      }
      return;
    }
  }
#pragma unroll
  for (int h = 0; h < 2; ++h) {
    float2 rv[G / 8][2], gv[G / 8][2];
#pragma unroll
    for (int j = 0; j < G / 8; ++j)
#pragma unroll
      for (int rh = 0; rh < 2; ++rh) {
        const int c = 8 * j + c0;
        ptrdiff_t yo, ro, go;
        const bool live = rows(64 * h + 16 * wq + l4 + 8 * rh, yo, ro, go);
        rv[j][rh] = make_float2(0.f, 0.f);
        gv[j][rh] = make_float2(1.f, 1.f);
        if (res) {
          if (rcs == 1) {
            if (live) rv[j][rh] = __ldg(reinterpret_cast<const float2*>(res + ro + c));
          } else {
            if (live && c < nch) rv[j][rh].x = __ldg(res + ro + (size_t)c * rcs);
            if (live && c + 1 < nch) rv[j][rh].y = __ldg(res + ro + (size_t)(c + 1) * rcs);
          }
        }
        if (gate && live) gv[j][rh] = __ldg(reinterpret_cast<const float2*>(gate + go + c));
      }
#pragma unroll
    for (int j = 0; j < G / 8; ++j) {
      const int c = 8 * j + c0;
      const float2 a = *reinterpret_cast<const float2*>(sc + c);
      const float2 b = *reinterpret_cast<const float2*>(sh + c);
#pragma unroll
      for (int rh = 0; rh < 2; ++rh) {
        ptrdiff_t yo, ro, go;
        const bool live = rows(64 * h + 16 * wq + l4 + 8 * rh, yo, ro, go);
        float v0 = fmaf(acc[h][4 * (j + G / 8) + 2 * rh], a.x, b.x);
        float v1 = fmaf(acc[h][4 * (j + G / 8) + 2 * rh + 1], a.y, b.y);
        if (res) v0 += rv[j][rh].x, v1 += rv[j][rh].y;
        if (act == OSB_ACT_RELU) {
          v0 = fmaxf(v0, 0.f), v1 = fmaxf(v1, 0.f);
        } else if (act == OSB_ACT_LEAKY) {
          v0 = v0 > 0.f ? v0 : 0.01f * v0, v1 = v1 > 0.f ? v1 : 0.01f * v1;
        }
        if (gate) v0 *= gv[j][rh].x, v1 *= gv[j][rh].y;
        if (!live) continue;
        if (ycs == 1) {
          *reinterpret_cast<float2*>(y + yo + c) = make_float2(v0, v1);
        } else {
          if (c < nch) y[yo + (size_t)c * ycs] = v0;
          if (c + 1 < nch) y[yo + (size_t)(c + 1) * ycs] = v1;
        }
      }
    }
  }
}

constexpr int TP_STRIDE = 36;
constexpr int TP_WARP_FLOATS = 32 * TP_STRIDE;

__device__ __forceinline__ void store_ndhwc_chunk32(float* tbuf, int lane, const float (&sum)[32], float* y0, const float* res0,
                                                    size_t vstride, const float* sc, const float* sh, int act,
                                                    uint32_t vmask = 0xffffffffu, const float* gate0 = nullptr) {
  const int c4 = 4 * (lane & 7), sub = lane >> 3;
  __syncwarp();
  float4* row = reinterpret_cast<float4*>(tbuf + lane * TP_STRIDE);
#pragma unroll
  for (int i = 0; i < 8; ++i) row[i] = make_float4(sum[4 * i], sum[4 * i + 1], sum[4 * i + 2], sum[4 * i + 3]);
  __syncwarp();
  const float4 a = *reinterpret_cast<const float4*>(sc + c4);
  const float4 b = *reinterpret_cast<const float4*>(sh + c4);
  float4 o[8];
#pragma unroll
  for (int j = 0; j < 8; ++j) {
    o[j] = *reinterpret_cast<const float4*>(tbuf + (4 * j + sub) * TP_STRIDE + c4);
    o[j].x = fmaf(o[j].x, a.x, b.x), o[j].y = fmaf(o[j].y, a.y, b.y), o[j].z = fmaf(o[j].z, a.z, b.z), o[j].w = fmaf(o[j].w, a.w, b.w);
  }
  if (res0) {
    float4 r[8];
#pragma unroll
    for (int j = 0; j < 8; ++j)
      r[j] = ((vmask >> (4 * j + sub)) & 1u) ? __ldg(reinterpret_cast<const float4*>(res0 + (size_t)(4 * j + sub) * vstride + c4))
                                             : make_float4(0.f, 0.f, 0.f, 0.f);
#pragma unroll
    for (int j = 0; j < 8; ++j) o[j].x += r[j].x, o[j].y += r[j].y, o[j].z += r[j].z, o[j].w += r[j].w;
  }
  if (act == OSB_ACT_RELU) {
#pragma unroll
    for (int j = 0; j < 8; ++j) o[j].x = fmaxf(o[j].x, 0.f), o[j].y = fmaxf(o[j].y, 0.f), o[j].z = fmaxf(o[j].z, 0.f), o[j].w = fmaxf(o[j].w, 0.f);
  } else if (act == OSB_ACT_LEAKY) {
#pragma unroll
    for (int j = 0; j < 8; ++j) {
      o[j].x = o[j].x > 0.f ? o[j].x : 0.01f * o[j].x, o[j].y = o[j].y > 0.f ? o[j].y : 0.01f * o[j].y;
      o[j].z = o[j].z > 0.f ? o[j].z : 0.01f * o[j].z, o[j].w = o[j].w > 0.f ? o[j].w : 0.01f * o[j].w;
    }
  }
  if (gate0) {
#pragma unroll
    for (int j = 0; j < 8; ++j) {
      if (!((vmask >> (4 * j + sub)) & 1u)) continue;
      const float4 g = __ldg(reinterpret_cast<const float4*>(gate0 + (size_t)(4 * j + sub) * vstride + c4));
      o[j].x *= g.x, o[j].y *= g.y, o[j].z *= g.z, o[j].w *= g.w;
    }
  }
#pragma unroll
  for (int j = 0; j < 8; ++j)
    if ((vmask >> (4 * j + sub)) & 1u) *reinterpret_cast<float4*>(y0 + (size_t)(4 * j + sub) * vstride + c4) = o[j];
}

struct TcArgs {
  const float* x;
  const void* w;
  const float* scale;
  const float* shift;
  const float* residual;
  const float* gate;
  float* y;
  int B, Cin, Cout, D, H, W;
  int act, out_ndhwc, res_ndhwc;
  int in_ncdhw;
  int ystride;
  int cout_real;
  float kappa;
  unsigned int* overflow;
  bool slice() const { return ystride != 0 && ystride != Cout; }
};
using TcLaunch = int (*)(const TcArgs&, cudaStream_t);

inline int check_tc_args(const char* what, TcArgs& a, TcLaunch launch) {
  auto aligned = [](const void* p) { return (reinterpret_cast<uintptr_t>(p) & 15) == 0; };
  OSB_REQUIRE(a.x && a.w && a.y, "%s: null pointer", what);
  OSB_REQUIRE(a.B > 0 && a.D > 0 && a.H > 0, "%s: empty shape", what);
  OSB_REQUIRE(a.act >= 0 && a.act <= 2, "%s: unknown activation %d", what, a.act);
  OSB_REQUIRE(aligned(a.x) && aligned(a.w) && aligned(a.y) && aligned(a.residual) && aligned(a.gate),
              "%s: pointers must be 16-byte aligned", what);
  const bool channels_last = a.out_ndhwc && (!a.residual || a.res_ndhwc);
  OSB_REQUIRE(a.ystride == 0 || (a.ystride >= a.Cout && a.ystride % 4 == 0 && channels_last),
              "%s: a channel slice (ystride %d) needs channels-last tensors", what, a.ystride);
  OSB_REQUIRE(!a.gate || channels_last, "%s: the gate operand needs a channels-last output (and residual)", what);
  OSB_REQUIRE(a.cout_real == a.Cout || (a.cout_real >= 1 && a.cout_real < a.Cout && !a.out_ndhwc && (!a.residual || !a.res_ndhwc)),
              "%s: only NCDHW tensors may hold fewer (%d) channels than the packed %d", what, a.cout_real, a.Cout);
  if (!launch) {
    set_error("%s: no instantiation serves Cout=%d W=%d with gate=%d ystride=%d", what, a.Cout, a.W, a.gate != nullptr, a.ystride);
    return OSB_EUNSUPPORTED;
  }
  a.kappa = rz_kappa();
  a.overflow = tc_overflow_flag();
  return a.overflow ? OSB_OK : OSB_ECUDA;
}

template <auto KERNEL, class P>
int launch_persistent(const TcArgs& a, P p, long long items, size_t smem, const char* variant, cudaStream_t stream) {
  OSB_REQUIRE(items < (1ll << 31), "%s: too many work items", variant);
  static PerDeviceFlag configured;
  if (!configured.here()) {
    const cudaError_t e = cudaFuncSetAttribute(KERNEL, cudaFuncAttributeMaxDynamicSharedMemorySize, (int)smem);
    if (e != cudaSuccess) {
      set_error("%s: cannot reserve %zu bytes of shared memory: %s", variant, smem, cudaGetErrorString(e));
      return OSB_ECUDA;
    }
    configured.here() = true;
  }
  p.x = a.x, p.w = a.w, p.scale = a.scale, p.shift = a.shift, p.residual = a.residual, p.y = a.y;
  p.B = a.B, p.D = a.D, p.H = a.H, p.Cin = a.Cin, p.act = a.act, p.out_ndhwc = a.out_ndhwc, p.res_ndhwc = a.res_ndhwc;
  p.kappa = a.kappa, p.overflow = a.overflow;
  p.items = (int)items;
  const int sms = sm_count();
  set_tc_variant(variant);
  KERNEL<<<(int)cap_persistent_grid(p.items < sms ? p.items : sms), TC_WG_THREADS, smem, stream>>>(p);
  count_launch();
  const cudaError_t e = cudaGetLastError();
  if (e != cudaSuccess) {
    cudaFuncAttributes fa{};
    (void)cudaFuncGetAttributes(&fa, KERNEL);
    set_error("%s: launch failed: %s (threads %d, kernel maxThreadsPerBlock %d, regs %d, static smem %zu, dynamic smem %zu, "
              "max dynamic %d)", variant, cudaGetErrorString(e), TC_WG_THREADS, fa.maxThreadsPerBlock, fa.numRegs,
              fa.sharedSizeBytes, smem, fa.maxDynamicSharedSizeBytes);
    return OSB_ECUDA;
  }
  return OSB_OK;
}

struct TcRoute {
  TcLaunch launch;
  int kc;
};
TcRoute select_conv3d_tc(int Cin, int Cout, int W, int dilation, bool gate, bool slice);
template <int COUT>
int launch_tc(const TcArgs& a, cudaStream_t stream);

}
```

openstereo_b200/ops.py:

```python
import math

import torch

from . import _lib

ACT_NONE, ACT_RELU, ACT_LEAKY, ACT_RELU6 = 0, 1, 2, 3
TC_WIDTH = 128
TC_KC = 32


_LAUNCH_DEVICE = [None]


def _stream(t):
    _LAUNCH_DEVICE[0] = t.device.index
    return torch.cuda.current_stream(t.device).cuda_stream


def _same_device(*tensors):
    devs = {t.device for t in tensors if t is not None}
    if len(devs) > 1:
        raise RuntimeError("openstereo_b200: operands live on different devices: %s" % sorted(str(d) for d in devs))


_PROFILE = None


def profile_start():
    global _PROFILE
    _PROFILE = {}


def profile_stop():
    global _PROFILE
    out, _PROFILE = _PROFILE, None
    return out or {}


def _call(name, *args):
    dev = _LAUNCH_DEVICE[0]
    if dev is not None and dev != torch.cuda.current_device():
        with torch.cuda.device(dev):
            return _call_on_current(name, *args)
    return _call_on_current(name, *args)


def _call_on_current(name, *args):
    if _PROFILE is None:
        return _lib.call(name, *args)
    start, stop = torch.cuda.Event(enable_timing=True), torch.cuda.Event(enable_timing=True)
    start.record()
    _lib.call(name, *args)
    stop.record()
    _PROFILE.setdefault(name, []).append((start, stop))


def _prep(t, name):
    if not isinstance(t, torch.Tensor):
        raise TypeError("%s must be a torch.Tensor" % name)
    if not t.is_cuda:
        raise RuntimeError("%s: not implemented on the CPU (openstereo_b200 has no CPU fallback)" % name)
    if t.dtype not in (torch.float32, torch.float16, torch.bfloat16):
        raise TypeError("%s: unsupported dtype %s" % (name, t.dtype))
    return t.detach().float().contiguous(), t.dtype


def _ptr(t):
    return None if t is None else t.data_ptr()


def _recording(*tensors):
    return torch.is_grad_enabled() and any(isinstance(t, torch.Tensor) and t.requires_grad for t in tensors)


def _grad_operands(*tensors):
    for t in tensors:
        if not t.is_cuda:
            raise RuntimeError("openstereo_b200: not implemented on the CPU (openstereo_b200 has no CPU fallback)")
    return [t.float() for t in tensors]


def build_gwc_volume(refimg_fea, targetimg_fea, maxdisp, num_groups):
    if _recording(refimg_fea, targetimg_fea):
        from .autograd import GwcVolumeFn
        assert refimg_fea.dim() == 4 and refimg_fea.shape == targetimg_fea.shape and refimg_fea.shape[1] % num_groups == 0
        r, t = _grad_operands(refimg_fea, targetimg_fea)
        return GwcVolumeFn.apply(r, t, int(maxdisp), int(num_groups), False).to(refimg_fea.dtype)
    ref, dt = _prep(refimg_fea, "refimg_fea")
    tgt, _ = _prep(targetimg_fea, "targetimg_fea")
    assert ref.dim() == 4 and ref.shape == tgt.shape
    _same_device(ref, tgt)
    b, c, h, w = ref.shape
    assert c % num_groups == 0
    out = torch.empty((b, num_groups, maxdisp, h, w), dtype=torch.float32, device=ref.device)
    if out.numel():
        _call("osb_gwc_volume_fwd", ref.data_ptr(), tgt.data_ptr(), out.data_ptr(), b, c, h, w, maxdisp,
                  num_groups, _stream(out))
    return out.to(dt)


def build_concat_volume(refimg_fea, targetimg_fea, maxdisp, mask_left=True):
    if _recording(refimg_fea, targetimg_fea):
        from .autograd import ConcatVolumeFn
        assert refimg_fea.dim() == 4 and refimg_fea.shape == targetimg_fea.shape
        r, t = _grad_operands(refimg_fea, targetimg_fea)
        return ConcatVolumeFn.apply(r, t, int(maxdisp), bool(mask_left)).to(refimg_fea.dtype)
    ref, dt = _prep(refimg_fea, "refimg_fea")
    tgt, _ = _prep(targetimg_fea, "targetimg_fea")
    assert ref.dim() == 4 and ref.shape == tgt.shape
    _same_device(ref, tgt)
    b, c, h, w = ref.shape
    out = torch.empty((b, 2 * c, maxdisp, h, w), dtype=torch.float32, device=ref.device)
    if out.numel():
        _call("osb_concat_volume_fwd", ref.data_ptr(), tgt.data_ptr(), out.data_ptr(), b, c, h, w, maxdisp,
                  1 if mask_left else 0, _stream(out))
    return out.to(dt)


def cat_fms(reference_fm, target_fm, max_disp=192, start_disp=0, dilation=1):
    if start_disp != 0 or dilation != 1:
        raise NotImplementedError("cat_fms: only start_disp=0, dilation=1 (the PSMNet configuration) is accelerated")
    return build_concat_volume(reference_fm, target_fm, max_disp)


def correlation_volume(left_feature, right_feature, max_disp):
    if _recording(left_feature, right_feature):
        from .autograd import GwcVolumeFn
        assert left_feature.dim() == 4 and left_feature.shape == right_feature.shape
        l, r = _grad_operands(left_feature, right_feature)
        return GwcVolumeFn.apply(l, r, int(max_disp), 1, False).squeeze(1).to(left_feature.dtype)
    l, dt = _prep(left_feature, "left_feature")
    r, _ = _prep(right_feature, "right_feature")
    assert l.dim() == 4 and l.shape == r.shape
    _same_device(l, r)
    b, c, h, w = l.shape
    out = torch.empty((b, max_disp, h, w), dtype=torch.float32, device=l.device)
    if out.numel():
# ... 412 lines not shown
            if n:
                tc_overflow_count(self.device, reset=True)
                raise RuntimeError("openstereo_b200: %d loader threads met activations outside the fp16 range of the tensor-core "
                                   "convolutions (|x| >= 4094); the previous result is invalid.  Run those layers with "
                                   "aggregation.USE_TENSOR_CORES = False" % n)


def f16_split(w):
    w = w.contiguous()
    hi = w.to(torch.float16)
    lo = (w - hi.float()).to(torch.float16)
    return hi, lo


class TcWeight:
    __slots__ = ("data", "inv", "kc", "cout", "cout_real", "ksize", "_eff")

    def __init__(self, data, inv, kc, cout, cout_real=None, ksize=3):
        self.data, self.inv, self.kc, self.cout, self._eff = data, inv, kc, cout, None
        self.cout_real = cout if cout_real is None else cout_real
        self.ksize = ksize

    def eff_scale(self, scale):
        key = None if scale is None else (scale.data_ptr(), scale._version)
        if self._eff is None or self._eff[0] != key:
            if scale is not None and scale.numel() < self.inv.numel():
                scale = torch.cat((scale.float(), scale.new_ones(self.inv.numel() - scale.numel()).float()))
            eff = self.inv if scale is None else scale.float() * self.inv
            self._eff = (key, eff.contiguous())
        return self._eff[1]


def pack_tc_weight(weight, kc=None, kw_order=(0, 1, 2), pad_cout_to=None):
    w = weight.detach().float()
    cout_real, cin = w.shape[:2]
    k = int(w.shape[2])
    if pad_cout_to is not None and cout_real < pad_cout_to:
        w = torch.cat((w, w.new_zeros((pad_cout_to - cout_real,) + tuple(w.shape[1:]))), 0)
    cout = w.shape[0]
    kc = TC_KC if kc is None else kc
    assert kc in (16, 32) and cin % kc == 0 and k in (3, 4) and tuple(w.shape[2:]) == (k, k, k) and len(kw_order) == k
    amax = w.abs().amax(dim=(1, 2, 3, 4))
    _, ex = torch.frexp(amax)
    e = torch.where(amax > 0, TC_WEIGHT_TOP_LOG2 - ex, torch.zeros_like(ex)).clamp(-40, 40)
    ws = torch.ldexp(w, e.view(-1, 1, 1, 1, 1))
    hi, lo = f16_split(ws)
    both = torch.stack((hi, lo), 0)
    both = both[..., list(kw_order)]
    both = both.contiguous().view(2, cout, cin // kc, kc, k, k, k)
    both = both.permute(4, 2, 5, 6, 1, 0, 3)
    data = both.reshape(k, cin // kc, k, k * cout, 2 * kc).contiguous()
    cpr = (2 * kc) // 8
    rows = torch.arange(k * cout, device=data.device)
    key = (rows & 7) if kc == 32 else ((rows >> 1) & 3)
    src = torch.arange(cpr, device=data.device).view(1, cpr) ^ key.view(-1, 1)
    data = data.view(k, cin // kc, k, k * cout, cpr, 8)
    data = torch.gather(data, 4, src.view(1, 1, 1, k * cout, cpr, 1).expand(k, cin // kc, k, k * cout, cpr, 8).contiguous())
    data = data.reshape(k, cin // kc, k, k * cout, 2 * kc).contiguous()
    inv = torch.ldexp(torch.ones_like(amax), -(e + TC_ACT_SCALE_LOG2))
    return TcWeight(data, inv.contiguous(), kc, cout, cout_real, ksize=k)


def _tc_args(w_split, cin, kc, scale):
    assert isinstance(w_split, TcWeight) and w_split.kc == kc
    k = w_split.ksize
    assert tuple(w_split.data.shape) == (k, cin // kc, k, k * w_split.cout, 2 * kc) and w_split.data.dtype == torch.float16
    assert w_split.data.is_contiguous() and w_split.data.is_cuda
    return w_split.data.data_ptr(), w_split.eff_scale(scale)


def to_ndhwc(x, pad_to=None):
    assert x.is_cuda and x.dtype == torch.float32 and x.is_contiguous() and x.dim() == 5
    b, c, d, h, w = x.shape
    cp = c if pad_to is None else int(pad_to)
    assert cp >= c
    y = torch.empty((b, d, h, w, cp), dtype=torch.float32, device=x.device)
    if cp == c:
        _call("osb_ncdhw_to_ndhwc", x.data_ptr(), y.data_ptr(), b, c, d, h, w, _stream(y))
    else:
        _call("osb_ncdhw_to_ndhwc_pad", x.data_ptr(), y.data_ptr(), b, c, cp, d, h, w, _stream(y))
    return y


def conv3d_k3_tc(x_ndhwc, w_split, scale=None, shift=None, residual=None, act=ACT_NONE, out_ndhwc=True, res_ndhwc=True,
                 in_ncdhw=False, gate=None):
    assert x_ndhwc.is_cuda and x_ndhwc.dtype == torch.float32 and x_ndhwc.is_contiguous() and x_ndhwc.dim() == 5
    if in_ncdhw:
        b, cin, d, h, w = x_ndhwc.shape
    else:
        b, d, h, w, cin = x_ndhwc.shape
    cout = w_split.cout_real
    kc = conv3d_tc_kc(cin, cout, w)
    assert kc
    wptr, scale = _tc_args(w_split, cin, kc, scale)
    if shift is not None and shift.numel() < w_split.cout:
        shift = torch.cat((shift.float(), shift.new_zeros(w_split.cout - shift.numel()).float()))
    shape = (b, d, h, w, cout) if out_ndhwc else (b, cout, d, h, w)
    y = torch.empty(shape, dtype=torch.float32, device=x_ndhwc.device)
    if residual is not None:
        want = (b, d, h, w, cout) if res_ndhwc else (b, cout, d, h, w)
        assert tuple(residual.shape) == want and residual.is_contiguous()
    assert not in_ncdhw or kc == 32
    if gate is not None:
        assert kc == 16 and out_ndhwc and res_ndhwc and not in_ncdhw
        assert tuple(gate.shape) == (b, h, w, cout) and gate.is_contiguous() and gate.dtype == torch.float32 and gate.is_cuda
        _call("osb_conv3d_k3_tc_gate_fwd", x_ndhwc.data_ptr(), wptr, _ptr(scale), _ptr(shift), _ptr(residual), gate.data_ptr(),
              y.data_ptr(), b, cin, cout, d, h, w, act, _stream(y))
        return y
    _call("osb_conv3d_k3_tc_ncdhw_fwd" if in_ncdhw else "osb_conv3d_k3_tc_fwd", x_ndhwc.data_ptr(), wptr, _ptr(scale), _ptr(shift), _ptr(residual),
          y.data_ptr(), b, cin, cout, d, h, w, act, 1 if out_ndhwc else 0, 1 if res_ndhwc else 0, _stream(y))
    return y


def conv3d_s2_tc_supported(cin, cout, d, h, w):
    return bool(_lib.lib.osb_conv3d_s2_tc_supported(int(cin), int(cout), int(d), int(h), int(w)))


def conv3d_k3_s2_tc(x_ndhwc, w_split, scale=None, shift=None, residual=None, act=ACT_NONE, out_ndhwc=False, res_ndhwc=False):
    assert x_ndhwc.is_cuda and x_ndhwc.dtype == torch.float32 and x_ndhwc.is_contiguous() and x_ndhwc.dim() == 5
    b, d, h, w, cin = x_ndhwc.shape
    cout = w_split.cout
    wptr, scale = _tc_args(w_split, cin, 16, scale)
    do, ho, wo = d // 2, h // 2, w // 2
    shape = (b, do, ho, wo, cout) if out_ndhwc else (b, cout, do, ho, wo)
    y = torch.empty(shape, dtype=torch.float32, device=x_ndhwc.device)
    if residual is not None:
        want = (b, do, ho, wo, cout) if res_ndhwc else (b, cout, do, ho, wo)
        assert tuple(residual.shape) == want and residual.is_contiguous()
    _call("osb_conv3d_k3_s2_tc_fwd", x_ndhwc.data_ptr(), wptr, _ptr(scale), _ptr(shift), _ptr(residual),
          y.data_ptr(), b, cin, cout, d, h, w, act, 1 if out_ndhwc else 0, 1 if res_ndhwc else 0, _stream(y))
    return y


def deconv3d_tc_supported(cin, cout, w):
    return bool(_lib.lib.osb_deconv3d_tc_supported(int(cin), int(cout), int(w)))


def pack_tc_deconv_weight(weight):
    w = weight.detach().float().permute(1, 0, 2, 3, 4).contiguous()
    return pack_tc_weight(w, 16, kw_order=(1, 2, 0) if w.shape[2] == 3 else (1, 3, 2, 0))


def deconv3d_k4_tc_supported(cin, cout, w):
    return bool(_lib.lib.osb_deconv3d_k4_tc_supported(int(cin), int(cout), int(w)))


def deconv3d_k4_tc(x_ndhwc, w_split, scale=None, shift=None, residual=None, act=ACT_NONE, out_ndhwc=True, res_ndhwc=True,
                   cout_real=None):
    assert x_ndhwc.is_cuda and x_ndhwc.dtype == torch.float32 and x_ndhwc.is_contiguous() and x_ndhwc.dim() == 5
    b, d, h, w, cin = x_ndhwc.shape
    cout = w_split.cout
    creal = cout if cout_real is None else int(cout_real)
    assert w_split.ksize == 4 and (out_ndhwc is False or creal == cout)
    wptr, scale = _tc_args(w_split, cin, 16, scale)
    shape = (b, 2 * d, 2 * h, 2 * w, cout) if out_ndhwc else (b, creal, 2 * d, 2 * h, 2 * w)
    y = torch.empty(shape, dtype=torch.float32, device=x_ndhwc.device)
    if residual is not None:
        want = (b, 2 * d, 2 * h, 2 * w, cout) if res_ndhwc else (b, creal, 2 * d, 2 * h, 2 * w)
        assert tuple(residual.shape) == want and residual.is_contiguous()
    _call("osb_deconv3d_k4_tc_fwd", x_ndhwc.data_ptr(), wptr, _ptr(scale), _ptr(shift), _ptr(residual),
          y.data_ptr(), b, cin, cout, creal, d, h, w, act, 1 if out_ndhwc else 0, 1 if res_ndhwc else 0, _stream(y))
    return y


def tc_slice(kind, x_ndhwc, w_split, scale, shift, y, coff, act=ACT_NONE, gate=None):
    assert x_ndhwc.is_cuda and x_ndhwc.dtype == torch.float32 and x_ndhwc.is_contiguous() and x_ndhwc.dim() == 5
    assert y.is_contiguous() and y.dtype == torch.float32 and y.dim() == 5
    b, d, h, w, cin = x_ndhwc.shape
    cout, ctot = w_split.cout, y.shape[-1]
    assert 0 <= coff and coff + cout <= ctot and coff % 4 == 0
    wptr, scale = _tc_args(w_split, cin, 16, scale)
    yp = y.data_ptr() + 4 * coff
    if kind == "s1":
        assert tuple(y.shape[:4]) == (b, d, h, w)
        gp = None
        if gate is not None:
            assert tuple(gate.shape) == (b, h, w, ctot) and gate.is_contiguous()
            gp = gate.data_ptr() + 4 * coff
        _call("osb_conv3d_k3_tc_cs_fwd", x_ndhwc.data_ptr(), wptr, _ptr(scale), _ptr(shift), None, gp, yp, b, cin, cout, d, h, w, act,
              ctot, _stream(y))
    elif kind == "s2":
        assert tuple(y.shape[:4]) == (b, d // 2, h // 2, w // 2) and gate is None
        _call("osb_conv3d_k3_s2_tc_cs_fwd", x_ndhwc.data_ptr(), wptr, _ptr(scale), _ptr(shift), yp, b, cin, cout, d, h, w, act, ctot,
              _stream(y))
# ... 161 lines not shown
```

Before: 284.3.

## Pass pre-split fp16 hi/lo activations between stem convs, loaded via TMA

Adds a split fp16 hi/lo activation layout that the W=128 tensor-core conv kernel can write in its epilogue and read back with a 4D TMA load, replacing the 128-thread loader that converts fp32 to split fp16 for every row. The GwcNet stem and classifier head chains now keep intermediates in this layout. The goal is to avoid the loader-warp conversion work and to move the same number of bytes per voxel without extra conversion passes. In exchange it adds a new tensor map, changes the smem channel chunk ordering and swizzle indexing (vcol, lane_voxel, TcK), and adds overflow reporting on stores, so correctness depends on the reordered layout matching everywhere.

```diff
diff --git a/include/openstereo_b200.h b/include/openstereo_b200.h
--- a/include/openstereo_b200.h
+++ b/include/openstereo_b200.h
@@ -87,6 +87,13 @@
 int osb_conv3d_k3_tc_ncdhw_fwd(const float* x_ncdhw, const void* w_split, const float* scale, const float* shift,
                                const float* residual, float* y, int B, int Cin, int Cout, int D, int H, int W, int act,
                                int out_ndhwc, int res_ndhwc, osb_stream_t stream);
+#define OSB_LAYOUT_NCDHW 0
+#define OSB_LAYOUT_NDHWC 1
+#define OSB_LAYOUT_SPLIT 2
+int osb_ncdhw_to_split(const float* x, float* y_split, int B, int C, int D, int H, int W, osb_stream_t stream);
+int osb_conv3d_k3_tc_split_fwd(const float* x, const void* w_split, const float* scale, const float* shift, const float* residual,
+                               float* y, int B, int Cin, int Cout, int D, int H, int W, int act, int in_layout, int out_layout,
+                               int res_layout, osb_stream_t stream);
 int osb_conv3d_s2_tc_supported(int Cin, int Cout, int D, int H, int W);
 int osb_conv3d_k3_s2_tc_fwd(const float* x_ndhwc, const void* w_split, const float* scale, const float* shift,
                             const float* residual, float* y, int B, int Cin, int Cout, int D, int H, int W, int act,
diff --git a/openstereo_b200/_lib.py b/openstereo_b200/_lib.py
--- a/openstereo_b200/_lib.py
+++ b/openstereo_b200/_lib.py
@@ -29,6 +29,8 @@
     "osb_conv3d_k3_s2_tc_fwd": [_f32p] * 6 + [_i] * 9 + [_s],
     "osb_conv3d_k3_tc_fwd": [_f32p] * 6 + [_i] * 9 + [_s],
     "osb_conv3d_k3_tc_ncdhw_fwd": [_f32p] * 6 + [_i] * 9 + [_s],
+    "osb_conv3d_k3_tc_split_fwd": [_f32p] * 6 + [_i] * 10 + [_s],
+    "osb_ncdhw_to_split": [_f32p, _f32p] + [_i] * 5 + [_s],
     "osb_conv3d_k3_tc_gate_fwd": [_f32p] * 7 + [_i] * 7 + [_s],
     "osb_deconv3d_k4_tc_supported": [_i, _i, _i],
     "osb_conv3d_k3_tc_cs_fwd": [_f32p] * 7 + [_i] * 8 + [_s],
diff --git a/openstereo_b200/aggregation.py b/openstereo_b200/aggregation.py
--- a/openstereo_b200/aggregation.py
+++ b/openstereo_b200/aggregation.py
@@ -76,14 +76,19 @@
     return _tc_weight(layer, width) is not None
 
 
-def _conv_tc(layer, x_ndhwc, act=ACT_NONE, residual=None, out_ndhwc=True, res_ndhwc=True, in_ncdhw=False):
+def _conv_tc(layer, x_ndhwc, act=ACT_NONE, residual=None, out_ndhwc=True, res_ndhwc=True, in_ncdhw=False, out_split=False):
     wt = _tc_weight(layer, x_ndhwc.shape[4] if in_ncdhw else x_ndhwc.shape[3])
-    return ops.conv3d_k3_tc(x_ndhwc, wt, layer.scale, layer.shift, residual, act, out_ndhwc, res_ndhwc, in_ncdhw)
-
-
-def _stem_in(layer, volume, act):
+    return ops.conv3d_k3_tc(x_ndhwc, wt, layer.scale, layer.shift, residual, act, out_ndhwc, res_ndhwc, in_ncdhw,
+                            out_split=out_split)
+
+
+def _split_chain_ok(width, *layers):
+    return USE_TENSOR_CORES and all(ops.conv3d_tc_kc(l.cin, l.cout, width) == 32 for l in layers)
+
+
+def _stem_in(layer, volume, act, out_split=False):
     if ops.conv3d_tc_kc(layer.cin, layer.cout, volume.shape[-1]) == 32:
-        return _conv_tc(layer, volume, act, in_ncdhw=True)
+        return _conv_tc(layer, volume, act, in_ncdhw=True, out_split=out_split)
     return _conv_tc(layer, ops.to_ndhwc(volume), act)
 
 
@@ -196,7 +201,8 @@
     head0, cls = classif3
     width = out.shape[3]
     if _tc_ok(cls, width):
-        return _conv_tc(cls, _conv_tc(head0, out, ACT_RELU), ACT_NONE, out_ndhwc=False, res_ndhwc=False)
+        mid = _conv_tc(head0, out, ACT_RELU, out_split=_split_chain_ok(width, head0, cls))
+        return _conv_tc(cls, mid, ACT_NONE, out_ndhwc=False, res_ndhwc=False)
     if cls.cin == 32 and cls.cout == 1 and cls._w5 is not None and cls.stride == 1:
         if "c1" not in cls._tc:
             cls._tc["c1"] = ops.pack_c1_weight(cls._w5)
@@ -222,8 +228,9 @@
         stem_tc = all(_tc_ok(l, width) for l in (self.dres0[0], self.dres0[1], self.dres1[0], self.dres1[1]))
         b, _, dd, hh, ww = volume.shape
         if stem_tc and _tc_ok(self.classif3[0], width) and all(_hg_channels_last_ok(hg, (b, dd, hh, ww, 32)) for hg in self.hg):
-            c = _conv_tc(self.dres0[1], _stem_in(self.dres0[0], volume, ACT_RELU), ACT_RELU)
-            out = _conv_tc(self.dres1[1], _conv_tc(self.dres1[0], c, ACT_RELU), ACT_NONE, residual=c)
+            split = _split_chain_ok(width, self.dres0[0], self.dres0[1], self.dres1[0], self.dres1[1])
+            c = _conv_tc(self.dres0[1], _stem_in(self.dres0[0], volume, ACT_RELU, out_split=split), ACT_RELU, out_split=split)
+            out = _conv_tc(self.dres1[1], _conv_tc(self.dres1[0], c, ACT_RELU, out_split=split), ACT_NONE, residual=c)
             for hg in self.hg:
                 out = _gwc_hourglass_channels_last(hg, out)
             return _classif3_channels_last(self.classif3, out)
diff --git a/openstereo_b200/csrc/api.cu b/openstereo_b200/csrc/api.cu
--- a/openstereo_b200/csrc/api.cu
+++ b/openstereo_b200/csrc/api.cu
@@ -124,6 +124,27 @@
   return true;
 }
 
+bool make_tensor_map_split(CUtensorMap* out, const void* base, int C, int W, int H, int BD, int kc) {
+  EncodeTiledFn fn = encode_fn();
+  if (!fn) {
+    set_error("cuTensorMapEncodeTiled not available from the driver");
+    return false;
+  }
+  const uint64_t vox = 2ull * C * sizeof(uint16_t);
+  const cuuint64_t dims[4] = {2ull * C, (cuuint64_t)W, (cuuint64_t)H, (cuuint64_t)BD};
+  const cuuint64_t strides[3] = {vox, vox * W, vox * W * H};
+  const cuuint32_t box[4] = {2u * kc, (cuuint32_t)W, 1, 1};
+  const cuuint32_t elem[4] = {1, 1, 1, 1};
+  CUresult r = fn(out, CU_TENSOR_MAP_DATA_TYPE_FLOAT16, 4, const_cast<void*>(base), dims, strides, box, elem,
+                  CU_TENSOR_MAP_INTERLEAVE_NONE, kc == 32 ? CU_TENSOR_MAP_SWIZZLE_128B : CU_TENSOR_MAP_SWIZZLE_64B,
+                  CU_TENSOR_MAP_L2_PROMOTION_L2_128B, CU_TENSOR_MAP_FLOAT_OOB_FILL_NONE);
+  if (r != CUDA_SUCCESS) {
+    set_error("cuTensorMapEncodeTiled (split activations) failed with CUresult %d", (int)r);
+    return false;
+  }
+  return true;
+}
+
 }
 
 extern "C" {
diff --git a/openstereo_b200/csrc/common.cuh b/openstereo_b200/csrc/common.cuh
--- a/openstereo_b200/csrc/common.cuh
+++ b/openstereo_b200/csrc/common.cuh
@@ -69,6 +69,13 @@
       "l"(reinterpret_cast<uint64_t>(map)), "r"(smem_u32(bar)), "r"(c0), "r"(c1), "r"(c2)
       : "memory");
 }
+__device__ __forceinline__ void tma_load_4d(void* smem_dst, const CUtensorMap* map, uint64_t* bar, int c0, int c1, int c2, int c3) {
+  asm volatile(
+      "cp.async.bulk.tensor.4d.shared::cluster.global.mbarrier::complete_tx::bytes [%0], [%1, {%3, %4, %5, %6}], [%2];"
+      ::"r"(smem_u32(smem_dst)),
+      "l"(reinterpret_cast<uint64_t>(map)), "r"(smem_u32(bar)), "r"(c0), "r"(c1), "r"(c2), "r"(c3)
+      : "memory");
+}
 __device__ __forceinline__ void tma_prefetch_desc(const CUtensorMap* map) {
   asm volatile("prefetch.tensormap [%0];" ::"l"(reinterpret_cast<uint64_t>(map)) : "memory");
 }
@@ -77,5 +84,6 @@
 
 bool make_tensor_map_3d(CUtensorMap* out, const void* base, uint64_t d0, uint64_t d1, uint64_t d2, uint64_t stride1_bytes,
                         uint64_t stride2_bytes, uint32_t box0, uint32_t box1, uint32_t box2);
+bool make_tensor_map_split(CUtensorMap* out, const void* base, int C, int W, int H, int BD, int kc);
 
 }
diff --git a/openstereo_b200/csrc/conv3d_tc.cu b/openstereo_b200/csrc/conv3d_tc.cu
--- a/openstereo_b200/csrc/conv3d_tc.cu
+++ b/openstereo_b200/csrc/conv3d_tc.cu
@@ -13,6 +13,7 @@
 constexpr int TC_ROW_BYTES = TC_W * TC_KC * 4;
 
 struct TcParams {
+  CUtensorMap xmap;
   const float* x;
   const void* w;
   const float* scale;
@@ -26,6 +27,7 @@
   int out_ndhwc, res_ndhwc;
   int bulk_rows;
   int in_ncdhw;
+  int in_split, out_split, res_split;
   int items, hblocks;
 };
 
@@ -44,7 +46,7 @@
 };
 
 template <int COUT>
-__global__ void __launch_bounds__(TC_WG_THREADS, 1) conv3d_tc_kernel(const TcParams p) {
+__global__ void __launch_bounds__(TC_WG_THREADS, 1) conv3d_tc_kernel(const __grid_constant__ TcParams p) {
   using C = TcCfg<COUT>;
   constexpr int N3 = C::N3;
   constexpr int B_SLICE = C::B_SLICE;
@@ -70,7 +72,7 @@
 
   if (threadIdx.x == 0) {
     for (int s = 0; s < TC_STAGES; ++s) {
-      mbar_init(&a_ready[s], 128);
+      mbar_init(&a_ready[s], p.in_split ? 1 : 128);
       mbar_init(&a_empty[s], 4 * TC_WGS);
     }
     for (int k = 0; k < TC_BSLOTS * 3; ++k) {
@@ -115,7 +117,6 @@
     const int wg = warp >> 2;
     xchg += wg * C::XCHG_FLOATS;
     const int bar_xchg = 1 + wg;
-    constexpr uint32_t LO = TcK<TC_KC>::LO_OFF;
     constexpr uint32_t A_HALF = 64 * TC_KC * 4 / 16;
     const uint64_t dbase = desc_sw128_base();
     const uint32_t b16 = (smem_u32(b_buf) & 0x3FFFF) >> 4;
@@ -146,7 +147,8 @@
               wg_fence();
 #pragma unroll
               for (int ks = 0; ks < TcK<TC_KC>::KSTEPS; ++ks)
-                wg_mma_split<N3>(acc, da0 + 2 * ks, A_HALF, db0 + 2 * ks, LO, ks > 0 ? 1u : accum);
+                wg_mma_split<N3>(acc, da0 + TcK<TC_KC>::A_KSTEP * ks, A_HALF, TcK<TC_KC>::A_LO, db0 + 2 * ks, TcK<TC_KC>::B_LO,
+                                 ks > 0 ? 1u : accum);
               wg_commit();
               wg_wait_all();
               accum = 1;
@@ -171,14 +173,33 @@
         return true;
       };
       frag_epilogue<COUT>(acc, lane, q, tiles + warp * FRAG_TP_FLOATS, s_scale, s_shift, p.act, p.y, p.out_ndhwc ? 1 : plane, p.residual, p.res_ndhwc ? 1 : plane,
-                          nullptr, rows, COUT == 32 ? 32 : p.Cout);
+                          nullptr, rows, COUT == 32 ? 32 : p.Cout, p.out_split, p.res_split, p.overflow);
     }
   }
   else if (warp < 4 * TC_WGS + 4) {
     setmaxnreg_dec<TC_LOADER_REGS>();
+    if (p.in_split) {
+      if (warp == 4 * TC_WGS && elect_one()) {
+        RowIter ld{(int)blockIdx.x, 0, 0, -1};
+        if (ld.it < p.items) ld.kd = (((ld.it / p.hblocks) % p.D) == 0) ? 1 : 0;
+        uint32_t rowc = 0;
+        while (advance(ld)) {
+          const int hb = ld.it % p.hblocks;
+          const int d = (ld.it / p.hblocks) % p.D;
+          const int b = ld.it / (p.hblocks * p.D);
+          const uint32_t s = rowc % TC_STAGES, par = (rowc / TC_STAGES) & 1;
+          mbar_wait_relaxed(&a_empty[s], par ^ 1);
+          mbar_arrive_expect_tx(&a_ready[s], TC_ROW_BYTES);
+          tma_load_4d(a_buf + s * TC_ROW_BYTES, &p.xmap, &a_ready[s], 2 * TC_KC * ld.ch, 0, hb * TC_TILES - 1 + ld.r, b * p.D + d + ld.kd - 1);
+          ++rowc;
+        }
+      }
+      __syncwarp();
+      return;
+    }
     const int lt = threadIdx.x - 4 * TC_WGS * 32;
     const int vsel = lt >> 3, c16 = lt & 7;
-    const int vcol = ((vsel & 1) << 2) | ((vsel >> 1) & 3) | (vsel & 8);
+    const int vcol = ((vsel & 1) << 1) | ((vsel >> 1) & 1) | (vsel & 12);
     float amax = 0.f;
     auto run = [&](auto in_ncdhw) {
       constexpr bool NCDHW = decltype(in_ncdhw)::value;
@@ -331,12 +352,13 @@
 }
 
 __global__ void __launch_bounds__(256) ncdhw_to_ndhwc_kernel(const float* __restrict__ x, float* __restrict__ y, int C, int Cp,
-                                                             size_t vol) {
+                                                             size_t vol, uint16_t* __restrict__ ys, unsigned int* overflow) {
   __shared__ float tile[32][33];
   const int b = blockIdx.z;
   const size_t v0 = (size_t)blockIdx.x * 32;
   const int c0 = blockIdx.y * 32;
   const int tx = threadIdx.x & 31, ty = threadIdx.x >> 5;
+  float amax = 0.f;
   for (int i = ty; i < 32; i += 8) {
     const int c = c0 + i;
     const size_t v = v0 + tx;
@@ -346,15 +368,28 @@
   for (int i = ty; i < 32; i += 8) {
     const size_t v = v0 + i;
     const int c = c0 + tx;
-    if (c < Cp && v < vol) y[((size_t)b * vol + v) * Cp + c] = tile[tx][i];
-  }
+    if (c >= Cp || v >= vol) continue;
+    if (!ys) {
+      y[((size_t)b * vol + v) * Cp + c] = tile[tx][i];
+      continue;
+    }
+    const float s = tile[tx][i] * TC_ACT_SCALE;
+    const uint32_t hl = cvt_f16x2_sat(s, s - f16x2_to_float2(cvt_f16x2_sat(s, 0.f)).x);
+    uint16_t* vox = ys + ((size_t)b * vol + v) * 2 * Cp;
+    vox[split_index(c)] = (uint16_t)(hl & 0xFFFFu);
+    vox[split_index(c) + SPLIT_GRANULE] = (uint16_t)(hl >> 16);
+    amax = fmaxf(amax, fabsf(s));
+  }
+  if (ys) tc_report_overflow(overflow, amax);
 }
 
 template <int COUT>
 int launch_tc(const TcArgs& a, cudaStream_t stream) {
   TcParams p{};
   p.Cout = a.Cout, p.in_ncdhw = a.in_ncdhw;
-  p.bulk_rows = a.in_ncdhw || a.Cin == TC_KC;
+  p.in_split = a.in_split, p.out_split = a.out_split, p.res_split = a.res_split;
+  p.bulk_rows = !a.in_split && (a.in_ncdhw || a.Cin == TC_KC);
+  if (a.in_split && !make_tensor_map_split(&p.xmap, a.x, a.Cin, TC_W, a.H, a.B * a.D, TC_KC)) return OSB_ECUDA;
   p.hblocks = (a.H + TC_TILES - 1) / TC_TILES;
   static const std::string variant = tc_variant_name("tc<%d>", COUT);
   return launch_persistent<conv3d_tc_kernel<COUT>>(a, p, (long long)a.B * a.D * p.hblocks, TcCfg<COUT>::SMEM, variant.c_str(), stream);
@@ -380,7 +415,21 @@
   OSB_REQUIRE(B > 0 && C > 0 && Cpad >= C && D > 0 && H > 0 && W > 0 && B <= 65535, "ncdhw_to_ndhwc: bad shape");
   const size_t vol = (size_t)D * H * W;
   dim3 grid((unsigned)((vol + 31) / 32), (Cpad + 31) / 32, B);
-  ncdhw_to_ndhwc_kernel<<<grid, 256, 0, (cudaStream_t)stream>>>(x, y, C, Cpad, vol);
+  ncdhw_to_ndhwc_kernel<<<grid, 256, 0, (cudaStream_t)stream>>>(x, y, C, Cpad, vol, nullptr, nullptr);
+  count_launch();
+  return check_launch("ncdhw_to_ndhwc_kernel");
+}
+
+int osb_ncdhw_to_split(const float* x, float* y_split, int B, int C, int D, int H, int W, osb_stream_t stream) {
+  using namespace osb;
+  OSB_REQUIRE(x && y_split, "ncdhw_to_split: null pointer");
+  OSB_REQUIRE(B > 0 && C > 0 && C % SPLIT_GRANULE == 0 && D > 0 && H > 0 && W > 0 && B <= 65535,
+              "ncdhw_to_split: bad shape (C must be a multiple of %d)", SPLIT_GRANULE);
+  unsigned int* flag = tc_overflow_flag();
+  if (!flag) return OSB_ECUDA;
+  const size_t vol = (size_t)D * H * W;
+  dim3 grid((unsigned)((vol + 31) / 32), (C + 31) / 32, B);
+  ncdhw_to_ndhwc_kernel<<<grid, 256, 0, (cudaStream_t)stream>>>(x, nullptr, C, C, vol, reinterpret_cast<uint16_t*>(y_split), flag);
   count_launch();
   return check_launch("ncdhw_to_ndhwc_kernel");
 }
@@ -396,6 +445,12 @@
   OSB_REQUIRE(!a.in_ncdhw || kc == 32, "conv3d_k3_tc: NCDHW input is served by the W = 128 kernel only");
   OSB_REQUIRE((!a.ystride && !a.gate) || kc == 16, "conv3d_k3_tc: a channel slice or gate needs the 16-channel-chunk kernels");
   OSB_REQUIRE(a.Cout > 16 || (!a.out_ndhwc && (!a.residual || !a.res_ndhwc)), "conv3d_k3_tc: Cout <= 16 writes (and adds) NCDHW tensors only");
+  OSB_REQUIRE(!(a.in_split || a.out_split || a.res_split) || (kc == 32 && !a.ystride && !a.gate),
+              "conv3d_k3_tc: split activations are served by the W = 128 kernel only");
+  OSB_REQUIRE(!a.in_split || !a.in_ncdhw, "conv3d_k3_tc: an input is either NCDHW or split");
+  OSB_REQUIRE((!a.out_split || a.out_ndhwc) && (!a.res_split || a.res_ndhwc), "conv3d_k3_tc: split tensors are channels-last");
+  OSB_REQUIRE(!(a.out_split || a.res_split) || (a.out_ndhwc && (!a.residual || a.res_ndhwc)),
+              "conv3d_k3_tc: a split output or residual needs a channels-last output and residual");
   const TcLaunch launch = select_conv3d_tc(a.Cin, a.Cout, a.W, dilation, a.gate != nullptr, a.slice()).launch;
   const int rc = check_tc_args("conv3d_k3_tc", a, launch);
   return rc != OSB_OK ? rc : launch(a, (cudaStream_t)stream);
@@ -430,6 +485,17 @@
                             Cout}, 1, stream);
 }
 
+int osb_conv3d_k3_tc_split_fwd(const float* x, const void* w_split, const float* scale, const float* shift, const float* residual,
+                               float* y, int B, int Cin, int Cout, int D, int H, int W, int act, int in_layout, int out_layout,
+                               int res_layout, osb_stream_t stream) {
+  auto known = [](int l) { return l == OSB_LAYOUT_NCDHW || l == OSB_LAYOUT_NDHWC || l == OSB_LAYOUT_SPLIT; };
+  OSB_REQUIRE(known(in_layout) && known(out_layout) && known(res_layout), "conv3d_k3_tc_split: unknown layout");
+  osb::TcArgs a{x, w_split, scale, shift, residual, nullptr, y, B, Cin, Cout, D, H, W, act, out_layout != OSB_LAYOUT_NCDHW, res_layout != OSB_LAYOUT_NCDHW,
+                in_layout == OSB_LAYOUT_NCDHW, 0, Cout};
+  a.in_split = in_layout == OSB_LAYOUT_SPLIT, a.out_split = out_layout == OSB_LAYOUT_SPLIT, a.res_split = res_layout == OSB_LAYOUT_SPLIT;
+  return conv3d_k3_tc_impl(a, 1, stream);
+}
+
 int osb_conv2d_tc_kc(int Cin, int Cout, int W, int dilation) { return osb::select_conv3d_tc(Cin, Cout, W, dilation, false, false).kc; }
 
 int osb_conv2d_k3_tc_fwd(const float* x_nhwc, const void* w_split, const float* scale, const float* shift, const float* residual,
diff --git a/openstereo_b200/csrc/conv3d_tcdc.cu b/openstereo_b200/csrc/conv3d_tcdc.cu
--- a/openstereo_b200/csrc/conv3d_tcdc.cu
+++ b/openstereo_b200/csrc/conv3d_tcdc.cu
@@ -46,7 +46,6 @@
   static_assert(STAGES >= NLW, "the ring must hold at least one unit per loader warp");
   static constexpr int HBLK = TILES * R;
   static constexpr int KSTEPS = KC / 16;
-  static constexpr int LO = KC / 8;
   static constexpr int A_OFF = 0;
   static constexpr int B_OFF = A_OFF + STAGES * UNIT_BYTES;
   static constexpr int STAGE_OFF = B_OFF + TC_BSLOTS * KS_ * B_SUB;
@@ -198,7 +197,7 @@
               wg_fence();
 #pragma unroll
               for (int ks = 0; ks < C::KSTEPS; ++ks)
-                wg_mma_split<C::NGK>(acc, da0 + 2 * ks, A_HALF, db0 + 2 * ks, C::LO, ks > 0 ? 1u : accum);
+                wg_mma_split<C::NGK>(acc, da0 + TcK<KC>::A_KSTEP * ks, A_HALF, TcK<KC>::A_LO, db0 + 2 * ks, TcK<KC>::B_LO, ks > 0 ? 1u : accum);
               wg_commit();
               wg_wait_all();
               accum = 1;
diff --git a/openstereo_b200/csrc/conv3d_tcg.cu b/openstereo_b200/csrc/conv3d_tcg.cu
--- a/openstereo_b200/csrc/conv3d_tcg.cu
+++ b/openstereo_b200/csrc/conv3d_tcg.cu
@@ -49,7 +49,6 @@
   static constexpr int S_FIRST = -DIL;
   static constexpr int S_LAST = (NT - 1) * TS + DIL;
   static constexpr int KSTEPS = KC / 16;
-  static constexpr int LO = KC / 8;
   static constexpr int A_OFF = 0;
   static constexpr int B_OFF = A_OFF + STAGES * UNIT_BYTES;
   static constexpr int BAR_OFF = B_OFF + TC_BSLOTS * 3 * B_SUB;
@@ -173,7 +172,7 @@
               wg_fence();
 #pragma unroll
               for (int ks = 0; ks < C::KSTEPS; ++ks)
-                wg_mma_split<C::NG3>(acc, da0 + 2 * ks, A_HALF, db0 + 2 * ks, C::LO, ks > 0 ? 1u : accum);
+                wg_mma_split<C::NG3>(acc, da0 + TcK<KC>::A_KSTEP * ks, A_HALF, TcK<KC>::A_LO, db0 + 2 * ks, TcK<KC>::B_LO, ks > 0 ? 1u : accum);
               wg_commit();
               wg_wait_all();
               accum = 1;
diff --git a/openstereo_b200/csrc/conv3d_tcs2.cu b/openstereo_b200/csrc/conv3d_tcs2.cu
--- a/openstereo_b200/csrc/conv3d_tcs2.cu
+++ b/openstereo_b200/csrc/conv3d_tcs2.cu
@@ -45,7 +45,6 @@
   static constexpr int NU = TILES * 3 * 2;
   static constexpr int HBLK = TILES * R;
   static constexpr int KSTEPS = KC / 16;
-  static constexpr int LO = KC / 8;
   static constexpr int A_OFF = 0;
   static constexpr int B_OFF = A_OFF + STAGES * UNIT_BYTES;
   static constexpr int STAGE_OFF = B_OFF + TC_BSLOTS * 3 * B_SLOT;
@@ -159,8 +158,8 @@
                 wg_fence();
 #pragma unroll
                 for (int ks = 0; ks < C::KSTEPS; ++ks) {
-                  if (par == 0) wg_mma_split<C::G>(acc_e, da0 + 2 * ks, A_HALF, db0 + 2 * ks, C::LO, ks > 0 ? 1u : accum_e);
-                  else wg_mma_split<2 * C::G>(acc_o, da0 + 2 * ks, A_HALF, db0 + 2 * ks, C::LO, ks > 0 ? 1u : accum_o);
+                  if (par == 0) wg_mma_split<C::G>(acc_e, da0 + TcK<KC>::A_KSTEP * ks, A_HALF, TcK<KC>::A_LO, db0 + 2 * ks, TcK<KC>::B_LO, ks > 0 ? 1u : accum_e);
+                  else wg_mma_split<2 * C::G>(acc_o, da0 + TcK<KC>::A_KSTEP * ks, A_HALF, TcK<KC>::A_LO, db0 + 2 * ks, TcK<KC>::B_LO, ks > 0 ? 1u : accum_o);
                 }
                 wg_commit();
                 wg_wait_all();
diff --git a/openstereo_b200/csrc/tc_common.cuh b/openstereo_b200/csrc/tc_common.cuh
--- a/openstereo_b200/csrc/tc_common.cuh
+++ b/openstereo_b200/csrc/tc_common.cuh
@@ -90,12 +90,12 @@
 __device__ __forceinline__ void wg_wait_all() { asm volatile("wgmma.wait_group.sync.aligned 0;" ::: "memory"); }
 
 template <int N>
-__device__ __forceinline__ void wg_mma_split(float (&acc)[2][N / 2], uint64_t da, uint32_t a_half, uint64_t db, uint32_t lo,
-                                             uint32_t accumulate) {
+__device__ __forceinline__ void wg_mma_split(float (&acc)[2][N / 2], uint64_t da, uint32_t a_half, uint32_t a_lo, uint64_t db,
+                                             uint32_t b_lo, uint32_t accumulate) {
 #pragma unroll
   for (int h = 0; h < 2; ++h) {
-    wgmma_f16<N>(acc[h], da + h * a_half + lo, db, accumulate);
-    wgmma_f16<N>(acc[h], da + h * a_half, db + lo, 1);
+    wgmma_f16<N>(acc[h], da + h * a_half + a_lo, db, accumulate);
+    wgmma_f16<N>(acc[h], da + h * a_half, db + b_lo, 1);
     wgmma_f16<N>(acc[h], da + h * a_half, db, 1);
   }
 }
@@ -197,23 +197,41 @@
 }
 
 
+constexpr int SPLIT_GRANULE = 16;
+__device__ __forceinline__ int split_index(int c) { return (c / SPLIT_GRANULE) * 2 * SPLIT_GRANULE + c % SPLIT_GRANULE; }
+__device__ __forceinline__ void split_store4(uint16_t* vox, int c, const float4 v, float& amax) {
+  uint2 hi, lo;
+  f16_split4(v, hi, lo, amax);
+  *reinterpret_cast<uint2*>(vox + split_index(c)) = hi;
+  *reinterpret_cast<uint2*>(vox + split_index(c) + SPLIT_GRANULE) = lo;
+}
+__device__ __forceinline__ float4 split_load4(const uint16_t* vox, int c) {
+  const uint2 hi = __ldg(reinterpret_cast<const uint2*>(vox + split_index(c)));
+  const uint2 lo = __ldg(reinterpret_cast<const uint2*>(vox + split_index(c) + SPLIT_GRANULE));
+  const float2 h01 = f16x2_to_float2(hi.x), h23 = f16x2_to_float2(hi.y), l01 = f16x2_to_float2(lo.x), l23 = f16x2_to_float2(lo.y);
+  constexpr float inv = 1.f / TC_ACT_SCALE;
+  return make_float4((h01.x + l01.x) * inv, (h01.y + l01.y) * inv, (h23.x + l23.x) * inv, (h23.y + l23.y) * inv);
+}
+
 template <int KC>
 __device__ __forceinline__ void stage_f16_split(uint8_t* tile, int row, int q, const float4 v, float& amax) {
   uint2 hi, lo;
   f16_split4(v, hi, lo, amax);
-  const int sub = (q & 1) << 3;
-  *reinterpret_cast<uint2*>(tile + swz_offset<KC>(row, q >> 1) + sub) = hi;
-  *reinterpret_cast<uint2*>(tile + swz_offset<KC>(row, KC / 8 + (q >> 1)) + sub) = lo;
+  const int sub = (q & 1) << 3, chunk = 4 * (q >> 2) + ((q >> 1) & 1);
+  *reinterpret_cast<uint2*>(tile + swz_offset<KC>(row, chunk) + sub) = hi;
+  *reinterpret_cast<uint2*>(tile + swz_offset<KC>(row, chunk + 2) + sub) = lo;
 }
 template <int KC>
 __device__ __forceinline__ int lane_voxel(int lane) {
-  if constexpr (KC == 32) return (((lane >> 3) & 1) << 2) | (lane >> 4);
+  if constexpr (KC == 32) return (((lane >> 3) & 1) << 1) | (lane >> 4);
   else return ((lane >> 2) & 1) | (((lane >> 3) & 1) << 2) | ((lane >> 4) << 1);
 }
 template <int KC>
 struct TcK {
   static constexpr int KSTEPS = KC / 16;
-  static constexpr int LO_OFF = KC / 8;
+  static constexpr int A_KSTEP = 4;
+  static constexpr int A_LO = 2;
+  static constexpr int B_LO = KC / 8;
 };
 
 template <int G, int DIL>
@@ -277,13 +295,15 @@
 template <int G, class Rows>
 __device__ __forceinline__ void frag_epilogue(const float (&acc)[2][3 * G / 2], int lane, int wq, float* tbuf, const float* sc,
                                               const float* sh, int act, float* y, size_t ycs, const float* res, size_t rcs,
-                                              const float* gate, Rows rows, int nch) {
+                                              const float* gate, Rows rows, int nch, bool y_split = false, bool res_split = false,
+                                              unsigned int* overflow = nullptr) {
   const int c0 = 2 * (lane & 3), l4 = lane >> 2;
   if constexpr (G == 32) {
     if (ycs == 1 && (!res || rcs == 1)) {
       const int c4 = 4 * (lane & 7), sub = lane >> 3;
       const float4 a = *reinterpret_cast<const float4*>(sc + c4);
       const float4 b = *reinterpret_cast<const float4*>(sh + c4);
+      float amax = 0.f;
 #pragma unroll
       for (int h = 0; h < 2; ++h) {
         __syncwarp();
@@ -306,7 +326,10 @@
         if (res) {
           float4 r[4];
 #pragma unroll
-          for (int i = 0; i < 4; ++i) r[i] = ok[i] ? __ldg(reinterpret_cast<const float4*>(res + ro[i] + c4)) : make_float4(0.f, 0.f, 0.f, 0.f);
+          for (int i = 0; i < 4; ++i)
+            r[i] = !ok[i] ? make_float4(0.f, 0.f, 0.f, 0.f)
+                 : res_split ? split_load4(reinterpret_cast<const uint16_t*>(res + ro[i]), c4)
+                             : __ldg(reinterpret_cast<const float4*>(res + ro[i] + c4));
 #pragma unroll
           for (int i = 0; i < 4; ++i) o[i].x += r[i].x, o[i].y += r[i].y, o[i].z += r[i].z, o[i].w += r[i].w;
         }
@@ -328,9 +351,13 @@
           for (int i = 0; i < 4; ++i) o[i].x *= g[i].x, o[i].y *= g[i].y, o[i].z *= g[i].z, o[i].w *= g[i].w;
         }
 #pragma unroll
-        for (int i = 0; i < 4; ++i)
-          if (ok[i]) *reinterpret_cast<float4*>(y + yo[i] + c4) = o[i];
+        for (int i = 0; i < 4; ++i) {
+          if (!ok[i]) continue;
+          if (y_split) split_store4(reinterpret_cast<uint16_t*>(y + yo[i]), c4, o[i], amax);
+          else *reinterpret_cast<float4*>(y + yo[i] + c4) = o[i];
+        }
       }
+      if (y_split) tc_report_overflow(overflow, amax);
       return;
     }
   }
@@ -453,6 +480,7 @@
   int cout_real;
   float kappa;
   unsigned int* overflow;
+  int in_split = 0, out_split = 0, res_split = 0;
   bool slice() const { return ystride != 0 && ystride != Cout; }
 };
 using TcLaunch = int (*)(const TcArgs&, cudaStream_t);
diff --git a/openstereo_b200/ops.py b/openstereo_b200/ops.py
--- a/openstereo_b200/ops.py
+++ b/openstereo_b200/ops.py
@@ -37,22 +37,22 @@
     return out or {}
 
 
-def _call(name, *args):
+def _call(name, *args, profile_as=None):
     dev = _LAUNCH_DEVICE[0]
     if dev is not None and dev != torch.cuda.current_device():
         with torch.cuda.device(dev):
-            return _call_on_current(name, *args)
-    return _call_on_current(name, *args)
-
-
-def _call_on_current(name, *args):
+            return _call_on_current(name, args, profile_as or name)
+    return _call_on_current(name, args, profile_as or name)
+
+
+def _call_on_current(name, args, key):
     if _PROFILE is None:
         return _lib.call(name, *args)
     start, stop = torch.cuda.Event(enable_timing=True), torch.cuda.Event(enable_timing=True)
     start.record()
     _lib.call(name, *args)
     stop.record()
-    _PROFILE.setdefault(name, []).append((start, stop))
+    _PROFILE.setdefault(key, []).append((start, stop))
 
 
 def _prep(t, name):
@@ -631,24 +631,65 @@
     return y
 
 
+SPLIT_GRANULE = 16
+LAYOUT_NCDHW, LAYOUT_NDHWC, LAYOUT_SPLIT = 0, 1, 2
+
+
+def is_split(t):
+    return t.dtype == torch.float16 and t.dim() == 5
+
+
+def to_split(x):
+    assert x.is_cuda and x.dtype == torch.float32 and x.is_contiguous() and x.dim() == 5
+    b, c, d, h, w = x.shape
+    assert c % SPLIT_GRANULE == 0, "split activations need a multiple of %d channels" % SPLIT_GRANULE
+    y = torch.empty((b, d, h, w, 2 * c), dtype=torch.float16, device=x.device)
+    _call("osb_ncdhw_to_split", x.data_ptr(), y.data_ptr(), b, c, d, h, w, _stream(y))
+    return y
+
+
+def from_split(x_split):
+    assert is_split(x_split) and x_split.shape[4] % (2 * SPLIT_GRANULE) == 0
+    g = x_split.shape[4] // (2 * SPLIT_GRANULE)
+    v = x_split.view(*x_split.shape[:4], g, 2, SPLIT_GRANULE).float()
+    return ((v[..., 0, :] + v[..., 1, :]) * (1.0 / 16)).reshape(*x_split.shape[:4], g * SPLIT_GRANULE).contiguous()
+
+
 def conv3d_k3_tc(x_ndhwc, w_split, scale=None, shift=None, residual=None, act=ACT_NONE, out_ndhwc=True, res_ndhwc=True,
-                 in_ncdhw=False, gate=None):
-    assert x_ndhwc.is_cuda and x_ndhwc.dtype == torch.float32 and x_ndhwc.is_contiguous() and x_ndhwc.dim() == 5
+                 in_ncdhw=False, gate=None, out_split=False):
+    assert x_ndhwc.is_cuda and x_ndhwc.dtype in (torch.float32, torch.float16) and x_ndhwc.is_contiguous() and x_ndhwc.dim() == 5
+    in_split = is_split(x_ndhwc)
+    assert not (in_split and in_ncdhw)
     if in_ncdhw:
         b, cin, d, h, w = x_ndhwc.shape
     else:
         b, d, h, w, cin = x_ndhwc.shape
+        if in_split:
+            cin = w_split.data.shape[1] * w_split.kc
+            if x_ndhwc.shape[4] != 2 * cin:
+                raise ValueError("conv3d_k3_tc: an fp16 input is read as split activations (ops.to_split), 2 * Cin = %d entries per "
+                                 "voxel for this weight; got %d" % (2 * cin, x_ndhwc.shape[4]))
     cout = w_split.cout_real
     kc = conv3d_tc_kc(cin, cout, w)
     assert kc
     wptr, scale = _tc_args(w_split, cin, kc, scale)
     if shift is not None and shift.numel() < w_split.cout:
         shift = torch.cat((shift.float(), shift.new_zeros(w_split.cout - shift.numel()).float()))
+    res_split = residual is not None and is_split(residual)
+    if residual is not None:
+        want = (b, d, h, w, 2 * cout if res_split else cout) if res_ndhwc else (b, cout, d, h, w)
+        assert tuple(residual.shape) == want and residual.is_contiguous() and (res_split or residual.dtype == torch.float32)
+    if in_split or out_split or res_split:
+        assert gate is None and (out_ndhwc or not out_split)
+        shape = (b, d, h, w, 2 * cout if out_split else cout) if out_ndhwc else (b, cout, d, h, w)
+        y = torch.empty(shape, dtype=torch.float16 if out_split else torch.float32, device=x_ndhwc.device)
+        layout = lambda split, ndhwc: LAYOUT_SPLIT if split else (LAYOUT_NDHWC if ndhwc else LAYOUT_NCDHW)
+        _call("osb_conv3d_k3_tc_split_fwd", x_ndhwc.data_ptr(), wptr, _ptr(scale), _ptr(shift), _ptr(residual), y.data_ptr(),
+              b, cin, cout, d, h, w, act, layout(in_split, not in_ncdhw), layout(out_split, out_ndhwc), layout(res_split, res_ndhwc),
+              _stream(y), profile_as="osb_conv3d_k3_tc_ncdhw_fwd" if in_ncdhw else "osb_conv3d_k3_tc_fwd")
+        return y
     shape = (b, d, h, w, cout) if out_ndhwc else (b, cout, d, h, w)
     y = torch.empty(shape, dtype=torch.float32, device=x_ndhwc.device)
-    if residual is not None:
-        want = (b, d, h, w, cout) if res_ndhwc else (b, cout, d, h, w)
-        assert tuple(residual.shape) == want and residual.is_contiguous()
     assert not in_ncdhw or kc == 32
     if gate is not None:
         assert kc == 16 and out_ndhwc and res_ndhwc and not in_ncdhw
```

New measurement: 296.5 (median of 6 runs). 1.04x the previous value.
